# MrTornado24/IDE-3D

Measured on AMD Instinct MI355X. Metric: 512x512 RGB+seg frames/s @96 depth samples (whole job), higher is better.
Workload: dtype f32 (3x3 convs + MLPs: fp32 operands as 3 bf16 pieces, 6 products, f32 accumulate)

## Files before the change

### ide-3d_amd/csrc/modconv.hip

```cpp
#include "common.h"
#include "knobs.h"
#include <stdlib.h>
#include <string.h>
#include <type_traits>

namespace ide3d {

typedef float f32x16 __attribute__((ext_vector_type(16)));

#ifdef IDE3D_MC_TRACE
__device__ unsigned long long g_mc_dbg[256];
#define IDE3D_MC_TS(k) { const unsigned long long now_ = __builtin_readcyclecounter(); mc_acc[k] += now_ - mc_last; mc_last = now_; }
#else
#define IDE3D_MC_TS(k)
#endif

enum { MODE_CONV3 = 0, MODE_CONV1 = 1, MODE_TCONV3 = 2, MODE_TCONV3A = 3, MODE_CONV3S2 = 4 };

template <int MODE> struct ModeCfg;
template <> struct ModeCfg<MODE_CONV3>  { static constexpr int KC = 4, WTAPS = 9, MAXT = 9; };
template <> struct ModeCfg<MODE_CONV1>  { static constexpr int KC = 16, WTAPS = 1, MAXT = 1; };
template <> struct ModeCfg<MODE_CONV3S2> { static constexpr int KC = 4, WTAPS = 9, MAXT = 9; };
template <> struct ModeCfg<MODE_TCONV3> { static constexpr int KC = 4, WTAPS = 9, MAXT = 4; };
template <> struct ModeCfg<MODE_TCONV3A> { static constexpr int KC = 4, WTAPS = 9, MAXT = 9; };
// ... 426 lines not shown
        IDE3D_MC_TS(4)
    }

#ifdef IDE3D_MC_TRACE
    const unsigned long long mc_t1 = __builtin_readcyclecounter();
#endif
    modconv_finish<MODE, TI, PH, PW, NWV, K::NCLS, K::MTW, K::NTW, K::BM, 2 * K::LDS_W>(p, partial, g, acc, s_w, mb, n0, y0, x0, split, cls, wm, wn, l32);
#ifdef IDE3D_MC_TRACE
    if (blockIdx.x == 100 && threadIdx.x == 0) {
        for (int k = 0; k < 6; ++k) g_mc_dbg[k] = mc_acc[k];
        g_mc_dbg[7] = (unsigned long long)(c_end - c_begin);
        g_mc_dbg[8] = mc_prologue;
        g_mc_dbg[9] = __builtin_readcyclecounter() - mc_t1;
    }
#endif
}


typedef unsigned u32x4 __attribute__((ext_vector_type(4)));
typedef unsigned u32x2 __attribute__((ext_vector_type(2)));
typedef __bf16 bf16x8 __attribute__((ext_vector_type(8)));
typedef __bf16 bf16x2 __attribute__((ext_vector_type(2)));
typedef float f32x2 __attribute__((ext_vector_type(2)));

template <int MODE, int BIG, int PH, int PARTS, int WBUF = 2, int NWV_ = 4, int PAIR = 0>
struct SpCfg {
    static_assert(MODE == MODE_CONV3 || MODE == MODE_TCONV3A, "split-bf16 loop: 3x3 and all-class transposed 3x3 only");
    static_assert(BIG == 1 || BIG == 2, "64- or 128-row blocks");
    static_assert(NWV_ == 4 || NWV_ == 8, "4 or 8 waves");
    static constexpr int PW = 16, NWV = NWV_, NT = 64 * NWV;
    static constexpr int BN = PH * PW;
    static_assert(!PAIR || MODE == MODE_TCONV3A, "row-parity pairs exist in the transposed form only");
    static constexpr int NCLS = (MODE == MODE_TCONV3A) ? (PAIR ? 2 : 4) : 1;
    static constexpr int BM = (BIG == 1) ? 128 : 64;
    static constexpr int WM = (BIG == 2 && PH == 32) ? 1 : 2, WN = NWV / WM;
    static constexpr int MTW = BM / 32 / WM, NTW = BN / 32 / WN;
    static_assert(MTW >= 1 && MTW * 32 * WM == BM, "row block must split into 32-row MFMA tiles per wave");
    static_assert(NTW >= 1 && NTW * 32 * WN == BN, "pixel tile must split into 32-pixel MFMA tiles per wave");
    static constexpr int NLOAD = 4;
    static constexpr int KC = 16;
    static constexpr int HALO = (MODE == MODE_TCONV3A) ? 1 : 2;
    static constexpr int HP = PH + HALO, HW = PW + HALO, NSLOT = HP * HW;
    static constexpr int NS = PARTS * (PARTS + 1) / 2;
    static constexpr int W_UNITS = 3 * PARTS * 2 * BM;
    static constexpr int X_UNITS = PARTS * 2 * NSLOT;
    static constexpr int NXR = (NSLOT + 63) / 64;
    static constexpr int LDS_BYTES = 16 * (WBUF * W_UNITS + 2 * X_UNITS);
    static_assert(LDS_BYTES <= 160 * 1024, "LDS of one CU");
};

__host__ __device__ inline int64_t sp_packed_units(int mblocks, int cchunks, int bm, int parts) { return (int64_t)mblocks * cchunks * 9 * parts * 2 * bm; }

__device__ __forceinline__ unsigned pk_bf16(float a, float b) {
    f32x2 v = {a, b};
    return __builtin_bit_cast(unsigned, __builtin_convertvector(v, bf16x2));
}
typedef _Float16 f16x2 __attribute__((ext_vector_type(2)));
typedef _Float16 f16x8 __attribute__((ext_vector_type(8)));
template <int PARTS, int F16 = 0>
__device__ __forceinline__ void split_pair(float a, float b, unsigned (&out)[PARTS]) {
    if constexpr (F16) {
        static_assert(PARTS == 2, "the fp16 split has two pieces");
        const f32x2 v = {a, b};
        const unsigned hi = __builtin_bit_cast(unsigned, __builtin_convertvector(v, f16x2));
        f32x2 r;
        asm("v_fma_mix_f32 %0, %1, -1.0, %2 op_sel_hi:[1,0,0]" : "=v"(r.x) : "v"(hi), "v"(a));
        asm("v_fma_mix_f32 %0, %1, -1.0, %2 op_sel:[1,0,0] op_sel_hi:[1,0,0]" : "=v"(r.y) : "v"(hi), "v"(b));
        out[0] = hi; out[1] = __builtin_bit_cast(unsigned, __builtin_convertvector(r, f16x2));
    } else {
#pragma unroll
    for (int q = 0; q < PARTS; ++q) {
        const unsigned pk = pk_bf16(a, b);
        out[q] = pk;
        if (q + 1 < PARTS) { a -= __uint_as_float(pk << 16); b -= __uint_as_float(pk & 0xffff0000u); }
    }
    }
}
template <int F16>
__device__ __forceinline__ f32x16 sp_mfma(const u32x4& a, const u32x4& b, const f32x16& c) {
    if constexpr (F16) return __builtin_amdgcn_mfma_f32_32x32x16_f16(__builtin_bit_cast(f16x8, a), __builtin_bit_cast(f16x8, b), c, 0, 0, 0);
    else return __builtin_amdgcn_mfma_f32_32x32x16_bf16(__builtin_bit_cast(bf16x8, a), __builtin_bit_cast(bf16x8, b), c, 0, 0, 0);
}
__device__ __forceinline__ void f16_scale(float bound, float& scale, float& unscale) {
    scale = 1.f; unscale = 1.f;
    if (bound > 0.f && bound < __builtin_inff()) {
        int e;
        frexpf(bound, &e);
        e = min(max(15 - e, -126), 126);
        scale = ldexpf(1.f, e); unscale = ldexpf(1.f, -e);
    }
}

__global__ void __launch_bounds__(256)
modconv_row_scale_kernel(const float* __restrict__ w, int cout, int rowlen, int rows_padded, float* __restrict__ scale, float* __restrict__ unscale) {
    const int row = blockIdx.x * 4 + (threadIdx.x >> 6), lane = threadIdx.x & 63;
    if (row >= rows_padded) return;
    float m = 0.f;
    if (row < cout) for (int i = lane; i < rowlen; i += 64) m = fmaxf(m, fabsf(w[(int64_t)row * rowlen + i]));
#pragma unroll
    for (int off = 32; off > 0; off >>= 1) m = fmaxf(m, __shfl_xor(m, off));
    if (lane == 0) { float sc, us; f16_scale(m, sc, us); scale[row] = sc; unscale[row] = us; }
}

template <int PARTS, int F16 = 0>
__global__ void __launch_bounds__(256)
modconv_pack_split_kernel(const float* __restrict__ w, int cout, int cin, int bm, int mblocks, int cchunks, u32x4* __restrict__ out,
                          const float* __restrict__ row_scale = nullptr) {
    const int64_t total = (int64_t)mblocks * cchunks * 9 * 2 * bm;
    const int64_t stride = (int64_t)gridDim.x * blockDim.x;
    for (int64_t i = (int64_t)blockIdx.x * blockDim.x + threadIdx.x; i < total; i += stride) {
        int64_t r = i;
        const int co_l = (int)(r % bm); r /= bm;
        const int kg = (int)(r % 2); r /= 2;
        const int tap = (int)(r % 9); r /= 9;
        const int cc = (int)(r % cchunks); r /= cchunks;
        const int mb = (int)r;
        const int co = mb * bm + co_l;
        const float rs = F16 ? row_scale[co] : 1.f;
        unsigned pk[4][PARTS];
#pragma unroll
        for (int e = 0; e < 4; ++e) {
            const int ci = cc * 16 + kg * 8 + e * 2;
            const float a = (co < cout && ci < cin) ? w[((int64_t)co * cin + ci) * 9 + tap] * rs : 0.f;
            const float b = (co < cout && ci + 1 < cin) ? w[((int64_t)co * cin + ci + 1) * 9 + tap] * rs : 0.f;
            split_pair<PARTS, F16>(a, b, pk[e]);
        }
        const int64_t base = (((int64_t)(mb * cchunks + cc) * 9 + tap) * PARTS * 2 + kg) * bm + co_l;
#pragma unroll
        for (int q = 0; q < PARTS; ++q) {
            const u32x4 v = {pk[0][q], pk[1][q], pk[2][q], pk[3][q]};
            out[base + (int64_t)q * 2 * bm] = v;
        }
    }
}

template <int OFF_BYTES>
__device__ __forceinline__ u32x4 lds_read128_async(unsigned addr) {
    u32x4 v;
    asm volatile("ds_read_b128 %0, %1 offset:%2" : "=v"(v) : "v"(addr), "n"(OFF_BYTES));
    return v;
}
template <int PENDING>
__device__ __forceinline__ void lds_wait128(u32x4& first) { asm volatile("s_waitcnt lgkmcnt(%1)" : "+v"(first) : "n"(PENDING)); }
__device__ __forceinline__ void lds_pin128(u32x4& v) { asm volatile("" : "+v"(v)); }

struct HeadEpi {
    const u32x4* w;
    const float* bias;
    float* y;
    int rows;
    float clamp;
    int store_x;
    int bias_first;
};
template <int PH, int PW, int NWV, int MTW, int NTW, int BM, int MT, int PARTS, int SCRATCH>
__device__ __forceinline__ void split_heads_finish(const ide3d_modconv_params& p, const HeadEpi& he, f32x16 (&acc)[1][MTW][NTW], float* smem,
                                                   int n0, int y0, int x0, int wm, int wn, int lp) {
    constexpr int NT = 64 * NWV, BN = PH * PW, TP = BN + 4, ROWS = MT * 32, CCH = BM / 16, A_UNITS = PARTS * 2 * ROWS;
    static_assert(BM * TP + 2 * BM + ROWS <= SCRATCH, "activation tile + coefficients must fit the loop's LDS");
    const int tid = threadIdx.x, lane = tid & 63, half = lane >> 5, l32 = lane & 31;
    const int wid = __builtin_amdgcn_readfirstlane(tid >> 6);
    const int hw = p.h * p.w_;
    float* const s_t = smem;
    float* const s_dm = smem + BM * TP;
    float* const s_bi = s_dm + BM;
    float* const s_hb = s_bi + BM;
    for (int e = tid; e < BM; e += NT) {
        s_dm[e] = (p.dcoefs && e < p.cout) ? p.dcoefs[(int64_t)n0 * p.cout + e] : 1.f;
        s_bi[e] = (p.bias && e < p.cout) ? p.bias[e] : 0.f;
    }
    for (int e = tid; e < ROWS; e += NT) s_hb[e] = (he.bias && e < he.rows) ? he.bias[e] : 0.f;
    __syncthreads();
    const float e_alpha = (p.act == 3) ? p.alpha : 1.f, e_gain = p.gain;
    const float e_clamp = (p.clamp >= 0.f) ? p.clamp : __builtin_inff();
    const float e_nstr = p.noise ? p.noise_strength : 0.f;
    auto finish = [&](float v, float d, float nz, float bb) {
        v *= d; v += nz; v += bb;
        v = (v > 0.f) ? v : v * e_alpha;
        v *= e_gain;
        return fminf(fmaxf(v, -e_clamp), e_clamp);
    };
#pragma unroll
    for (int j = 0; j < NTW; ++j) {
        const int pix = (wn * NTW + j) * 32 + lp;
        const int gy = y0 + pix / PW, gx = x0 + pix % PW;
        const float nz = (e_nstr != 0.f) ? p.noise[gy * p.w_ + gx] * e_nstr : 0.f;
#pragma unroll
        for (int i = 0; i < MTW; ++i)
#pragma unroll
            for (int r = 0; r < 16; ++r) {
                const int rl = (wm * MTW + i) * 32 + (r & 3) + 8 * (r >> 2) + 4 * half;
                s_t[rl * TP + pix] = finish(acc[0][i][j][r], s_dm[rl], nz, s_bi[rl]);
            }
    }
    __syncthreads();
    typedef float f32x4a __attribute__((ext_vector_type(4)));
    typedef float f32x4u __attribute__((ext_vector_type(4), aligned(4)));
    if (he.store_x) {
        float* const yimg = p.y + (int64_t)n0 * p.cout * hw;
#pragma unroll 4
        for (int e = tid; e < BM * BN / 4; e += NT) {
            const int rl = e / (BN / 4), pix = (e % (BN / 4)) * 4;
            const int gy = y0 + pix / PW, gx = x0 + pix % PW;
            *reinterpret_cast<f32x4u*>(yimg + (int64_t)rl * hw + gy * p.w_ + gx) = *reinterpret_cast<const f32x4a*>(s_t + rl * TP + pix);
        }
    }
    constexpr int NPT = BN / 32;
    constexpr int RG = (MT % 2 == 0 && NPT / NWV < 2) ? 2 : 1, MTH = MT / RG, PG = NWV / RG, NTH = NPT / PG;
    static_assert(MTH * RG == MT && NTH * PG == NPT && NTH >= 1, "head work must split evenly over the waves");
    const int rg = wid / PG, pg = wid % PG;
    const u32x4* __restrict__ wsrc = he.w + (int64_t)n0 * CCH * A_UNITS + half * ROWS + rg * MTH * 32 + l32;
    f32x16 hacc[MTH][NTH];
#pragma unroll
    for (int m = 0; m < MTH; ++m)
#pragma unroll
        for (int g = 0; g < 4; ++g) {
            const f32x4a b4 = *reinterpret_cast<const f32x4a*>(s_hb + (rg * MTH + m) * 32 + 8 * g + 4 * half);
#pragma unroll
            for (int t = 0; t < NTH; ++t)
#pragma unroll
                for (int k = 0; k < 4; ++k) hacc[m][t][4 * g + k] = he.bias_first ? b4[k] : 0.f;
        }
    u32x4 af[2][MTH][PARTS];
    auto fetch_a = [&](int c, int buf) {
#pragma unroll
        for (int m = 0; m < MTH; ++m)
#pragma unroll
            for (int q = 0; q < PARTS; ++q) af[buf][m][q] = wsrc[(int64_t)c * A_UNITS + q * 2 * ROWS + m * 32];
    };
    fetch_a(0, 0);
#pragma unroll
    for (int c = 0; c < CCH; ++c) {
        const int ab = c & 1;
        if (c + 1 < CCH) fetch_a(c + 1, ab ^ 1);
#pragma unroll
        for (int t = 0; t < NTH; ++t) {
            const float* xs = s_t + (c * 16 + 8 * half) * TP + (pg * NTH + t) * 32 + l32;
            u32x4 bfrag[PARTS];
            {
                unsigned pk[4][PARTS];
#pragma unroll
                for (int e = 0; e < 4; ++e) split_pair<PARTS>(xs[(2 * e) * TP], xs[(2 * e + 1) * TP], pk[e]);
#pragma unroll
                for (int q = 0; q < PARTS; ++q) bfrag[q] = u32x4{pk[0][q], pk[1][q], pk[2][q], pk[3][q]};
            }
#pragma unroll
            for (int m = 0; m < MTH; ++m)
#pragma unroll
                for (int qa = 0; qa < PARTS; ++qa)
#pragma unroll
                    for (int qb = 0; qa + qb < PARTS; ++qb)
                        hacc[m][t] = __builtin_amdgcn_mfma_f32_32x32x16_bf16(__builtin_bit_cast(bf16x8, af[ab][m][qa]), __builtin_bit_cast(bf16x8, bfrag[qb]), hacc[m][t], 0, 0, 0);
        }
    }
    const float h_clamp = (he.clamp >= 0.f) ? he.clamp : __builtin_inff();
#pragma unroll
    for (int t = 0; t < NTH; ++t) {
        const int pix = (pg * NTH + t) * 32 + l32;
        const int gy = y0 + pix / PW, gx = x0 + pix % PW;
        float* const o = he.y + (int64_t)n0 * he.rows * hw + gy * p.w_ + gx;
#pragma unroll
        for (int m = 0; m < MTH; ++m)
#pragma unroll
            for (int r = 0; r < 16; ++r) {
                const int row = (rg * MTH + m) * 32 + 8 * (r >> 2) + 4 * half + (r & 3);
                if (row >= he.rows) continue;
                float v = hacc[m][t][r];
                if (he.bias_first) {
                    v = __builtin_amdgcn_fmed3f(v, -h_clamp, h_clamp);
                } else {
                    v *= 1.f; v += 0.f; v += s_hb[row];
                    v = (v > 0.f) ? v : v * 1.f;
                    v = fminf(fmaxf(v, -h_clamp), h_clamp);
                }
                o[(int64_t)row * hw] = v;
            }
    }
    __syncthreads();
}

template <int MODE, int BIG, int PH, int PARTS, int WBUF, int NWV, int F16, int TEAMS = 1, int PAR = -1, int HEAD_MT = 0>
__device__ __forceinline__ void modconv_split_tile(const ide3d_modconv_params& p, const u32x4* __restrict__ wp, float* __restrict__ partial,
                                                   const ConvGeom& g, unsigned char* smem, int mb, int tl, int grp, int split, int tiles_x,
                                                   const float* __restrict__ row_unscale, float* wg_scratch = nullptr, const HeadEpi* he = nullptr) {
    using K = SpCfg<MODE, BIG, PH, PARTS, WBUF, NWV, (PAR >= 0)>;
    static_assert(!F16 || PARTS == 2, "f16x3 = two fp16 pieces per operand");
    static_assert(PAR < 0 || (MODE == MODE_TCONV3A && WBUF == 2 && TEAMS == 1), "row-parity pairs: transposed form, two weight buffers, one team");
    constexpr int NST = (PAR < 0) ? 3 : (PAR == 0 ? 2 : 1);
    auto kys = [](int i) constexpr { return (PAR < 0) ? i : (PAR == 0 ? 2 * i : 1); };
    static_assert(TEAMS == 1 || (TEAMS == 2 && NWV == 4), "two teams of four waves, or one team");
    constexpr int PW = K::PW;
    const int tid = (TEAMS == 2) ? (int)(threadIdx.x & 255u) : (int)threadIdx.x, lane = tid & 63;
    const int wid = __builtin_amdgcn_readfirstlane(tid >> 6);
    const int wm = wid / K::WN, wn = wid % K::WN;
    const int half = lane >> 5, l32 = lane & 31;
    const int lp = ((((l32 >> 2) ^ (l32 >> 3) ^ (l32 >> 4)) & 1) << 4) | (l32 & 15);
    const int txi = tl % tiles_x, tyi = tl / tiles_x;
    const int y0 = tyi * PH, x0 = txi * PW;
    const int n0 = grp;
    u32x4* const s_w = reinterpret_cast<u32x4*>(smem);
    u32x4* const s_x = s_w + WBUF * K::W_UNITS;

    f32x16 acc[K::NCLS][K::MTW][K::NTW];
#pragma unroll
    for (int q = 0; q < K::NCLS; ++q)
#pragma unroll
        for (int i = 0; i < K::MTW; ++i)
#pragma unroll
            for (int j = 0; j < K::NTW; ++j)
#pragma unroll
                for (int r = 0; r < 16; ++r) acc[q][i][j][r] = 0.f;

    const int hw = p.h * p.w_;
    int x_src[K::NXR];
#pragma unroll
    for (int r = 0; r < K::NXR; ++r) {
        const int sidx = lane + 64 * r;
        const int ry = sidx / K::HW, rx = sidx % K::HW;
        const int yy = y0 - 1 + ry, xx = x0 - 1 + rx;
        x_src[r] = (sidx < K::NSLOT && yy >= 0 && yy < p.h && xx >= 0 && xx < p.w_) ? yy * p.w_ + xx : -1;
    }
    const float* __restrict__ ximg = p.x + (int64_t)n0 * p.cin * hw;
    float xreg[K::NXR][4];
    float sty[4];
    float xs = 1.f, xus = 1.f;
    if constexpr (F16) {
        float mm = p.styles ? 0.f : 1.f;
        if (p.styles) for (int ci = lane; ci < p.cin; ci += 64) mm = fmaxf(mm, fabsf(p.styles[(int64_t)n0 * p.cin + ci]));
        float xm = (lane < IDE3D_AMAX_SLOTS) ? p.x_amax[(int64_t)n0 * IDE3D_AMAX_FLOATS + lane * IDE3D_AMAX_STRIDE] : 0.f;
#pragma unroll
        for (int off = 32; off > 0; off >>= 1) { mm = fmaxf(mm, __shfl_xor(mm, off)); xm = fmaxf(xm, __shfl_xor(xm, off)); }
        f16_scale(mm * xm, xs, xus);
    }
    const bool stages_patch = (NWV == 4) || wid < 4;
    auto fetch_patch = [&](int c) {
        if (!stages_patch) return;
        const int ci0 = c * K::KC + wid * 4;
#pragma unroll
        for (int k = 0; k < 4; ++k) {
            const int ci = min(ci0 + k, p.cin - 1);
            sty[k] = (ci0 + k < p.cin) ? (p.styles ? p.styles[(int64_t)n0 * p.cin + ci] : 1.f) : 0.f;
#pragma unroll
            for (int r = 0; r < K::NXR; ++r) xreg[r][k] = ximg[(int64_t)ci * hw + max(x_src[r], 0)];
        }
    };
    auto commit_patch = [&](int buf) {
        if (!stages_patch) return;
        unsigned char* const dst = reinterpret_cast<unsigned char*>(s_x + buf * K::X_UNITS) + ((wid >> 1) * K::NSLOT) * 16 + (wid & 1) * 8;
        const float sc[4] = {F16 ? sty[0] * xs : sty[0], F16 ? sty[1] * xs : sty[1], F16 ? sty[2] * xs : sty[2], F16 ? sty[3] * xs : sty[3]};
#pragma unroll
        for (int r = 0; r < K::NXR; ++r) {
            const int sidx = lane + 64 * r;
            const bool live = x_src[r] >= 0;
            unsigned lo[PARTS], hi[PARTS];
            split_pair<PARTS, F16>(live ? xreg[r][0] * sc[0] : 0.f, live ? xreg[r][1] * sc[1] : 0.f, lo);
            split_pair<PARTS, F16>(live ? xreg[r][2] * sc[2] : 0.f, live ? xreg[r][3] * sc[3] : 0.f, hi);
            if (sidx < K::NSLOT) {
#pragma unroll
                for (int q = 0; q < PARTS; ++q) {
                    const u32x2 v = {lo[q], hi[q]};
                    *reinterpret_cast<u32x2*>(dst + (q * 2 * K::NSLOT + sidx) * 16) = v;
                }
            }
        }
    };
    const u32x4* __restrict__ wsrc = wp + (int64_t)mb * g.cchunks * 3 * K::W_UNITS;
    constexpr int W_PIECES = K::W_UNITS / 64;
    static_assert(K::W_UNITS % 64 == 0, "weight stage is a whole number of 1 KB pieces");
    constexpr int W_COL = (W_PIECES + 3) / 4;
    constexpr int W_EARLY = (NWV == 8) ? (W_COL * 5 + 8) / 9 : W_COL;
    auto fetch_weights = [&](int stage, int buf, bool late = false) {
        const u32x4* src = wsrc + (int64_t)stage * K::W_UNITS;
        if (NWV == 4 && late) return;
        if (NWV == 8 && (late != (wid < 4))) return;
        const int m0 = late ? W_EARLY : 0, m1 = late ? W_COL : W_EARLY;
        for (int m = m0; m < m1; ++m) {
            const int i = (wid & 3) + 4 * m;
            if (i < W_PIECES)
                __builtin_amdgcn_global_load_lds((const __attribute__((address_space(1))) void*)(src + i * 64 + lane),
                                                 (__attribute__((address_space(3))) void*)(s_w + buf * K::W_UNITS + i * 64), 16, 0, 0);
        }
    };

    const unsigned a_base0 = (unsigned)(size_t)(s_w + half * K::BM + wm * K::MTW * 32 + l32);
    unsigned b_base0[K::NTW];
#pragma unroll
    for (int j = 0; j < K::NTW; ++j) {
        const int pix = (wn * K::NTW + j) * 32 + lp;
        b_base0[j] = (unsigned)(size_t)(s_x + half * K::NSLOT + (pix / PW) * K::HW + (pix % PW));
    }

    const int c_begin = split * g.chunks_per_split;
    const int c_end = min(c_begin + g.chunks_per_split, g.cchunks);
#ifdef IDE3D_MC_TRACE
    unsigned long long mc_acc[6] = {0, 0, 0, 0, 0, 0}, mc_last = 0;
    const unsigned long long mc_t0 = __builtin_readcyclecounter();
#endif
    if (c_begin < c_end) {
        if (WBUF == 2) { fetch_weights(c_begin * 3 + kys(0), 0); if (NWV == 8) fetch_weights(c_begin * 3 + kys(0), 0, true); }
        fetch_patch(c_begin);
        commit_patch(0);
    }
    asm volatile("s_waitcnt vmcnt(0)" ::: "memory");
    __syncthreads();
    int wbuf = 0;
#ifdef IDE3D_MC_TRACE
    mc_last = __builtin_readcyclecounter();
    const unsigned long long mc_prologue = mc_last - mc_t0;
#endif
    for (int c = c_begin; c < c_end; ++c) {
        const int xbuf = (c - c_begin) & 1;
        const bool more = c + 1 < c_end;
        static_for<NST>([&](auto sii) {
            constexpr int SI = decltype(sii)::value, KY = kys(SI);
            constexpr bool LAST = (SI == NST - 1), MID = (SI == (NST == 3 ? 1 : 0));
            const int next_stage = LAST ? (c + 1) * 3 + kys(0) : c * 3 + kys(LAST ? 0 : SI + 1);
            IDE3D_MC_TS(0)
            if constexpr (WBUF == 2) {
                if (!LAST || more) fetch_weights(next_stage, wbuf ^ 1);
                if (MID && more) fetch_patch(c + 1);
            } else {
                fetch_weights(c * 3 + KY, 0);
                if (MID && more) fetch_patch(c + 1);
                asm volatile("s_waitcnt vmcnt(0)" ::: "memory");
                __syncthreads();
            }
            IDE3D_MC_TS(1)
            const unsigned a_base = a_base0 + ((WBUF == 2) ? wbuf * (K::W_UNITS * 16) : 0);
            unsigned b_base[K::NTW];
#pragma unroll
            for (int j = 0; j < K::NTW; ++j) b_base[j] = b_base0[j] + xbuf * (K::X_UNITS * 16);
            constexpr int GRP = K::MTW + K::NTW, NGRP = 3 * PARTS;
            constexpr int SP_AHEAD = 1;
            constexpr int NBUF = (PARTS == 2 && SP_AHEAD > 1) ? 3 : 2;
            constexpr int AHEAD_CAP = 15 / GRP - 1, AHEAD_SAFE = (NBUF - 1) * PARTS - 1;
            constexpr int AHEAD = (SP_AHEAD < AHEAD_CAP ? SP_AHEAD : AHEAD_CAP) < AHEAD_SAFE ? (SP_AHEAD < AHEAD_CAP ? SP_AHEAD : AHEAD_CAP) : AHEAD_SAFE;
            static_assert(AHEAD >= 1 && (AHEAD + 1) * GRP <= 15, "lgkmcnt is a 4-bit counter");
            constexpr bool B_REUSE = (MODE == MODE_TCONV3A) && NBUF == 2;
            u32x4 av[NBUF][K::MTW][PARTS], bv[NBUF][K::NTW][PARTS];
            auto issue = [&](auto ss) {
                constexpr int S = decltype(ss)::value, KX = S / PARTS, Q = S % PARTS, B = KX % NBUF, T = KY * 3 + KX;
                constexpr int BS = B_REUSE ? (KX == 2 ? 1 : 0) : B;
                static_for<K::MTW>([&](auto ii) {
                    constexpr int I = decltype(ii)::value;
                    av[B][I][Q] = lds_read128_async<(((KX * PARTS + Q) * 2) * K::BM + I * 32) * 16>(a_base);
                });
                if constexpr (!(B_REUSE && KX == 1))
                static_for<K::NTW>([&](auto jj) {
                    constexpr int J = decltype(jj)::value;
                    bv[BS][J][Q] = lds_read128_async<(Q * 2 * K::NSLOT + tap_patch_offset<MODE, K::HW>(T)) * 16>(b_base[J]);
                });
            };
            static_for<AHEAD>([&](auto ss) { issue(ss); });
            static_for<NGRP>([&](auto ss) {
                constexpr int S = decltype(ss)::value, KX = S / PARTS, Q = S % PARTS, B = KX % NBUF, QC = (PAR >= 0) ? (KX & 1) : tap_class<MODE>(KY * 3 + KX);
                constexpr int BS = B_REUSE ? (KX == 2 ? 1 : 0) : B;
                if constexpr (S + AHEAD < NGRP) issue(std::integral_constant<int, S + AHEAD>{});
                constexpr int PENDING = [] { int n = 0; for (int s2 = S + 1; s2 <= S + AHEAD && s2 < NGRP; ++s2) n += K::MTW + ((B_REUSE && s2 / PARTS == 1) ? 0 : K::NTW); return n; }();
                lds_wait128<PENDING>(av[B][0][Q]);
#pragma unroll
                for (int i = 0; i < K::MTW; ++i) lds_pin128(av[B][i][Q]);
                if constexpr (!(B_REUSE && KX == 1)) {
#pragma unroll
                for (int j = 0; j < K::NTW; ++j) lds_pin128(bv[BS][j][Q]);
                }
#pragma unroll
                for (int qa = 0; qa <= Q; ++qa)
#pragma unroll
                    for (int qb = 0; qb <= Q; ++qb) {
                        if ((qa == Q || qb == Q) && qa + qb < PARTS) {
#pragma unroll
                            for (int i = 0; i < K::MTW; ++i)
#pragma unroll
                                for (int j = 0; j < K::NTW; ++j)
                                    acc[QC][i][j] = sp_mfma<F16>(av[B][i][qa], bv[BS][j][qb], acc[QC][i][j]);
                        }
                    }
            });
            IDE3D_MC_TS(2)
            if (LAST && more) commit_patch(xbuf ^ 1);
            if constexpr (WBUF == 2 && NWV == 8) { if (!LAST || more) fetch_weights(next_stage, wbuf ^ 1, true); }
            IDE3D_MC_TS(3)
            if (WBUF == 2) asm volatile("s_waitcnt vmcnt(0)" ::: "memory");
            IDE3D_MC_TS(4)
            __syncthreads();
            IDE3D_MC_TS(5)
            wbuf ^= 1;
        });
    }
#ifdef IDE3D_MC_TRACE
    const unsigned long long mc_t1 = __builtin_readcyclecounter();
#endif
    if constexpr (HEAD_MT > 0) {
        static_assert(MODE == MODE_CONV3 && TEAMS == 1 && !F16 && K::NCLS == 1, "fused heads: 3x3 split-bf16 layers");
        split_heads_finish<PH, PW, K::NWV, K::MTW, K::NTW, K::BM, HEAD_MT, PARTS, K::LDS_BYTES / 4>(p, *he, acc, reinterpret_cast<float*>(smem), n0, y0, x0, wm, wn, lp);
    } else
    modconv_finish<MODE, 1, PH, PW, K::NWV, K::NCLS, K::MTW, K::NTW, K::BM, K::LDS_BYTES / 4, PAR>(p, partial, g, acc, reinterpret_cast<float*>(smem), mb, n0, y0, x0, split, 0, wm, wn, lp,
                                                                                                F16 ? row_unscale : nullptr, xus, (TEAMS == 2) ? tid : -1, wg_scratch);
#ifdef IDE3D_MC_TRACE
    if (blockIdx.x == 100 && (threadIdx.x == 0 || threadIdx.x == 256)) {
        const int o = threadIdx.x ? 16 : 0;
        for (int k = 0; k < 6; ++k) g_mc_dbg[o + k] = mc_acc[k];
        g_mc_dbg[o + 7] = (unsigned long long)(c_end - c_begin) * 3;
        g_mc_dbg[o + 8] = mc_prologue;
        g_mc_dbg[o + 9] = __builtin_readcyclecounter() - mc_t1;
    }
#endif
}



constexpr int head_waves(int mt) { return mt == 1 ? 16 : 8; }
template <int PARTS, int MT>
struct HeadCfg {
    static constexpr int ROWS = MT * 32;
    static constexpr int A_UNITS = PARTS * 2 * ROWS;
    static constexpr int NWV = head_waves(MT);
    static constexpr int BN = 32 * NWV;
};
__host__ __device__ inline int64_t head_packed_units(int n, int cchunks, int parts, int mt) { return (int64_t)n * cchunks * parts * 2 * mt * 32; }

template <int PARTS>
__global__ void __launch_bounds__(256)
head_pack_split_kernel(const float* __restrict__ w, int64_t w_batch_stride, int n, int cout, int cin, int rows, int cchunks, u32x4* __restrict__ out) {
    const int64_t total = (int64_t)n * cchunks * 2 * rows;
    const int64_t stride = (int64_t)gridDim.x * blockDim.x;
    for (int64_t i = (int64_t)blockIdx.x * blockDim.x + threadIdx.x; i < total; i += stride) {
        int64_t r = i;
        const int row = (int)(r % rows); r /= rows;
        const int kg = (int)(r % 2); r /= 2;
        const int cc = (int)(r % cchunks); r /= cchunks;
        const int nb = (int)r;
        unsigned pk[4][PARTS];
#pragma unroll
        for (int e = 0; e < 4; ++e) {
            const int ci = cc * 16 + kg * 8 + e * 2;
            const float a = (row < cout && ci < cin) ? w[nb * w_batch_stride + (int64_t)row * cin + ci] : 0.f;
            const float b = (row < cout && ci + 1 < cin) ? w[nb * w_batch_stride + (int64_t)row * cin + ci + 1] : 0.f;
            split_pair<PARTS>(a, b, pk[e]);
        }
        const int64_t base = (((int64_t)nb * cchunks + cc) * PARTS * 2 + kg) * rows + row;
#pragma unroll
        for (int q = 0; q < PARTS; ++q) {
            const u32x4 v = {pk[0][q], pk[1][q], pk[2][q], pk[3][q]};
            out[base + (int64_t)q * 2 * rows] = v;
        }
    }
}

template <int PARTS, int MT>
__global__ void __launch_bounds__(64 * head_waves(MT), head_waves(MT) / 4)
head_split_kernel(ide3d_modconv_params p, const u32x4* __restrict__ wp, int cchunks, int tiles_per_image) {
    using K = HeadCfg<PARTS, MT>;
    if constexpr (K::NWV == 16) asm volatile("" ::: "v127"); else asm volatile("" ::: "v255");
    constexpr int S_MIN = K::NWV * 32 * 40 / 4 + 2 * K::ROWS / 4 + 16;
    constexpr int S_UNITS = (2 * K::A_UNITS > S_MIN) ? 2 * K::A_UNITS : S_MIN;
    __shared__ __attribute__((aligned(16))) u32x4 s_a[S_UNITS];
    const int tid = threadIdx.x, lane = tid & 63, half = lane >> 5, l32 = lane & 31;
    const int wid = __builtin_amdgcn_readfirstlane(tid >> 6);
    const int bid = xcd_remap(blockIdx.x, gridDim.x);
    const int n0 = bid / tiles_per_image, tile = bid % tiles_per_image;
    const int hw = p.h * p.w_;
    const int pix = tile * K::BN + wid * 32 + l32;
    const int pix_c = min(pix, hw - 1);
    const float* __restrict__ xl = p.x + (int64_t)n0 * p.cin * hw + (int64_t)(8 * half) * hw + pix_c;
    const u32x4* __restrict__ wsrc = wp + (int64_t)n0 * cchunks * K::A_UNITS;

    f32x16 acc[1][MT][1];
#pragma unroll
    for (int m = 0; m < MT; ++m)
#pragma unroll
        for (int r = 0; r < 16; ++r) acc[0][m][0][r] = 0.f;

    constexpr int A_PIECES = K::A_UNITS / 64;
    static_assert(K::A_UNITS % 64 == 0, "whole 1 KB pieces");
    auto fetch_a = [&](int c, int buf) {
        for (int i = wid; i < A_PIECES; i += K::NWV)
            __builtin_amdgcn_global_load_lds((const __attribute__((address_space(1))) void*)(wsrc + (int64_t)c * K::A_UNITS + i * 64 + lane),
                                             (__attribute__((address_space(3))) void*)(s_a + buf * K::A_UNITS + i * 64), 16, 0, 0);
    };
    float xr[3][8];
    auto fetch_b = [&](int c, auto slot_tag) {
        constexpr int SLOT = decltype(slot_tag)::value;
#pragma unroll
        for (int e = 0; e < 8; ++e) {
            const int ch = c * 16 + 8 * half + e;
            const float v = xl[(int64_t)(min(ch, p.cin - 1) - 8 * half) * hw];
            xr[SLOT][e] = (ch < p.cin) ? v : 0.f;
        }
    };
    using S0 = std::integral_constant<int, 0>; using S1 = std::integral_constant<int, 1>; using S2 = std::integral_constant<int, 2>;
    fetch_a(0, 0); fetch_b(0, S0{});
    if (cchunks > 1) fetch_b(1, S1{});
    auto chunk = [&](int c, auto slot_tag) {
        constexpr int SLOT = decltype(slot_tag)::value, NSLOT = (SLOT + 2) % 3;
        if (c + 1 < cchunks) asm volatile("s_waitcnt vmcnt(8)" ::: "memory"); else asm volatile("s_waitcnt vmcnt(0)" ::: "memory");
        __syncthreads();
        if (c + 1 < cchunks) fetch_a(c + 1, (c + 1) & 1);
        if (c + 2 < cchunks) fetch_b(c + 2, std::integral_constant<int, NSLOT>{});
        u32x4 bfrag[PARTS];
        {
            unsigned pk[4][PARTS];
#pragma unroll
            for (int e = 0; e < 4; ++e) split_pair<PARTS>(xr[SLOT][2 * e], xr[SLOT][2 * e + 1], pk[e]);
#pragma unroll
            for (int q = 0; q < PARTS; ++q) bfrag[q] = u32x4{pk[0][q], pk[1][q], pk[2][q], pk[3][q]};
        }
        const u32x4* sa = s_a + (c & 1) * K::A_UNITS + half * K::ROWS + l32;
#pragma unroll
        for (int m = 0; m < MT; ++m) {
            u32x4 af[PARTS];
#pragma unroll
            for (int q = 0; q < PARTS; ++q) af[q] = sa[q * 2 * K::ROWS + m * 32];
#pragma unroll
            for (int qa = 0; qa < PARTS; ++qa)
#pragma unroll
                for (int qb = 0; qa + qb < PARTS; ++qb)
                    acc[0][m][0] = __builtin_amdgcn_mfma_f32_32x32x16_bf16(__builtin_bit_cast(bf16x8, af[qa]), __builtin_bit_cast(bf16x8, bfrag[qb]), acc[0][m][0], 0, 0, 0);
        }
    };
    for (int c = 0; c < cchunks; c += 3) {
        chunk(c, S0{});
        if (c + 1 < cchunks) chunk(c + 1, S1{});
        if (c + 2 < cchunks) chunk(c + 2, S2{});
    }
    __syncthreads();
    ide3d_modconv_params pf = p;
    pf.h = 1; pf.w_ = hw;
    ConvGeom g{};
    g.oh = 1; g.ow = hw; g.split_k = 1;
    modconv_finish<MODE_CONV1, 1, 1, K::BN, K::NWV, 1, MT, 1, K::ROWS, S_UNITS * 4>(pf, nullptr, g, acc, reinterpret_cast<float*>(s_a), 0, n0, 0, tile * K::BN, 0, 0, 0, wid, l32);
}


template <class T>
__device__ __forceinline__ T* uniform_ptr(T* ptr) {
    const uint64_t v = reinterpret_cast<uint64_t>(ptr);
    const unsigned lo = __builtin_amdgcn_readfirstlane((unsigned)v), hi = __builtin_amdgcn_readfirstlane((unsigned)(v >> 32));
    return reinterpret_cast<T*>(((uint64_t)hi << 32) | lo);
}
template <int PARTS, int MT, int NCH>
__global__ void __launch_bounds__(512, 2)
head_resident_kernel(ide3d_modconv_params p, const u32x4* __restrict__ wp, int wgs_per_image, int tiles32) {
    using K = HeadCfg<PARTS, MT>;
    asm volatile("" ::: "v255");
    constexpr int NWV = 8, NBUF = (MT == 1) ? 2 : 1;
    __shared__ __attribute__((aligned(16))) u32x4 s_a[NCH * K::A_UNITS + K::ROWS / 4 + 4];
    float* const s_bi = reinterpret_cast<float*>(s_a + NCH * K::A_UNITS);
// ... 174 lines not shown

constexpr int STRIP_CO = 8, STRIP_WAVES = 16;
__global__ void __launch_bounds__(256)
tconv_strip_pack_kernel(const float* __restrict__ w, int cout, int cin, int cout_pad, float* __restrict__ ws) {
    const int64_t total = (int64_t)cin * 6 * cout_pad;
    for (int64_t i = (int64_t)blockIdx.x * 256 + threadIdx.x; i < total; i += (int64_t)gridDim.x * 256) {
        const int co = (int)(i % cout_pad); const int64_t r = i / cout_pad;
        const int t = (int)(r % 6), ci = (int)(r / 6);
        const int tap = t < 3 ? 6 + t : (t - 3) * 3 + 2;
        ws[i] = co < cout ? w[((int64_t)co * cin + ci) * 9 + tap] : 0.f;
    }
}
__global__ void __launch_bounds__(256)
tconv_strip_gather_kernel(const float* __restrict__ x, int rows, int h, int w_, float* __restrict__ xs) {
    const int len = w_ + h;
    for (int64_t i = (int64_t)blockIdx.x * 256 + threadIdx.x; i < (int64_t)rows * len; i += (int64_t)gridDim.x * 256) {
        const int64_t r = i / len; const int e = (int)(i - r * len);
        xs[i] = e < w_ ? x[r * h * w_ + (int64_t)(h - 1) * w_ + e] : x[r * h * w_ + (int64_t)(e - w_) * w_ + (w_ - 1)];
    }
}
__global__ void __launch_bounds__(64 * STRIP_WAVES, 4)
tconv_strip_kernel(ide3d_modconv_params p, const float* __restrict__ ws, const float* __restrict__ xs, int cout_pad, int oh, int ow, int64_t pitch,
                   int nb_re, int nb_ro, int nb_ce) {
    __shared__ float s_red[STRIP_WAVES][STRIP_CO][64];
    __shared__ float s_am[STRIP_WAVES];
    const int h = p.h, w_ = p.w_;
    const int lane = threadIdx.x & 63, q = __builtin_amdgcn_readfirstlane((int)(threadIdx.x >> 6));
    int b = (int)blockIdx.x, kind = 0;
    if (b >= nb_re) { b -= nb_re; kind = 1; if (b >= nb_ro) { b -= nb_ro; kind = 2; if (b >= nb_ce) { b -= nb_ce; kind = 3; } } }
    const bool is_row = kind < 2, odd = kind & 1;
    const int a = b * 64 + lane;
    const int t = 2 * a + (odd ? 1 : 0);
    const bool live = t < (is_row ? ow : oh - 1);
    const int co0 = (int)blockIdx.y * STRIP_CO, n = (int)blockIdx.z;
    const int len = is_row ? w_ : h;
    const bool ok_a = live && a < len, ok_b = live && !odd && a >= 1;
    const int64_t xs_pitch = (int64_t)w_ + h;
    const float* __restrict__ xn = xs + (int64_t)n * p.cin * xs_pitch;
    const int64_t off_a = (is_row ? 0 : w_) + min(a, len - 1), off_b = (is_row ? 0 : w_) + min(max(a - 1, 0), len - 1);
    const float* __restrict__ wt = ws + (is_row ? 0 : 3) * (int64_t)cout_pad + co0;
    constexpr int STRIP_CH = 8 * STRIP_WAVES, PER_WAVE = STRIP_CH / STRIP_WAVES, WPC = 3 * STRIP_CO;
    static_assert(PER_WAVE * WPC == 3 * 64, "three weight loads per lane and chunk");
    __shared__ __attribute__((aligned(16))) float s_wt[STRIP_WAVES][PER_WAVE * WPC];
    float acc[STRIP_CO];
#pragma unroll
    for (int j = 0; j < STRIP_CO; ++j) acc[j] = 0.f;
    for (int c0 = 0; c0 < p.cin; c0 += STRIP_CH) {
        float xa[PER_WAVE], xb[PER_WAVE], scv[PER_WAVE], wreg[3];
#pragma unroll
        for (int k = 0; k < PER_WAVE; ++k) {
            const int ci = min(c0 + q + k * STRIP_WAVES, p.cin - 1);
            xa[k] = xn[(int64_t)ci * xs_pitch + off_a];
            xb[k] = odd ? 0.f : xn[(int64_t)ci * xs_pitch + off_b];
            scv[k] = p.styles ? p.styles[(int64_t)n * p.cin + ci] : 1.f;
        }
#pragma unroll
        for (int r = 0; r < 3; ++r) {
            const int e = lane + 64 * r, k = e / WPC, rem = e - k * WPC, tp = rem / STRIP_CO, jj = rem - tp * STRIP_CO;
            const int ci = c0 + q + k * STRIP_WAVES;
            wreg[r] = (ci < p.cin) ? wt[((int64_t)ci * 6 + tp) * cout_pad + jj] : 0.f;
        }
        __builtin_amdgcn_wave_barrier();
#pragma unroll
        for (int r = 0; r < 3; ++r) s_wt[q][lane + 64 * r] = wreg[r];
        __builtin_amdgcn_fence(__ATOMIC_RELEASE, "wavefront");
        __builtin_amdgcn_wave_barrier();
        __builtin_amdgcn_fence(__ATOMIC_ACQUIRE, "wavefront");
#pragma unroll
        for (int k = 0; k < PER_WAVE; ++k) {
            const float va = ok_a ? xa[k] * scv[k] : 0.f;
            const float4* wv = reinterpret_cast<const float4*>(&s_wt[q][k * WPC]);
            if (odd) {
                const float4 b0 = wv[2], b1 = wv[3];
                const float w1[STRIP_CO] = {b0.x, b0.y, b0.z, b0.w, b1.x, b1.y, b1.z, b1.w};
#pragma unroll
                for (int j = 0; j < STRIP_CO; ++j) acc[j] = fmaf(va, w1[j], acc[j]);
            } else {
                const float vb = ok_b ? xb[k] * scv[k] : 0.f;
                const float4 a0 = wv[0], a1 = wv[1], c0v = wv[4], c1v = wv[5];
                const float w0[STRIP_CO] = {a0.x, a0.y, a0.z, a0.w, a1.x, a1.y, a1.z, a1.w};
                const float w2[STRIP_CO] = {c0v.x, c0v.y, c0v.z, c0v.w, c1v.x, c1v.y, c1v.z, c1v.w};
#pragma unroll
                for (int j = 0; j < STRIP_CO; ++j) { acc[j] = fmaf(va, w0[j], acc[j]); acc[j] = fmaf(vb, w2[j], acc[j]); }
            }
        }
    }
#pragma unroll
    for (int j = 0; j < STRIP_CO; ++j) s_red[q][j][lane] = acc[j];
    __syncthreads();
    float am = 0.f;
    {
        static_assert(STRIP_CO <= STRIP_WAVES, "wave q < STRIP_CO finishes output channel co0 + q");
        float v = 0.f;
        const int qc = min(q, STRIP_CO - 1);
#pragma unroll
        for (int k = 0; k < STRIP_WAVES; ++k) v += s_red[k][qc][lane];
        const int co = co0 + q;
        if (live && q < STRIP_CO && co < p.cout) {
            v *= p.dcoefs ? p.dcoefs[(int64_t)n * p.cout + co] : 1.f;
            const int oy = is_row ? oh - 1 : t, ox = is_row ? t : ow - 1;
            p.y[((int64_t)n * p.cout + co) * ((int64_t)oh * pitch) + (int64_t)oy * pitch + ox] = v;
            amax_acc(am, v);
        }
    }
    if (p.y_amax) amax_raise_block(p.y_amax, n, am, s_am);
}

struct BlockId { int mb, tile, grp, split; };
__device__ __forceinline__ BlockId decode_block(const ConvGeom& g) {
    int bid = xcd_remap(blockIdx.x, gridDim.x);
    BlockId b;
    b.mb = bid % g.mblocks; bid /= g.mblocks;
    b.tile = bid % g.tile_base[4]; bid /= g.tile_base[4];
    b.grp = bid % g.img_groups; bid /= g.img_groups;
    b.split = bid;
    return b;
}

template <int MODE, int BIG, int TI, int PH, int PW, int NWV = 4, int KCO = 0>
__global__ void __launch_bounds__(64 * NWV, NWV == 8 ? 2
                                  : (McCfg<MODE, BIG, TI, PH, PW, NWV, KCO>::NCLS * McCfg<MODE, BIG, TI, PH, PW, NWV, KCO>::MTW * McCfg<MODE, BIG, TI, PH, PW, NWV, KCO>::NTW > 8) ? 1
                                  : (TI * PH * PW <= 128 && MODE != MODE_CONV3S2 && KCO == 0) ? 3 : 2)
modconv_kernel(ide3d_modconv_params p, const float* __restrict__ wp, float* __restrict__ partial, ConvGeom g) {
    using K = McCfg<MODE, BIG, TI, PH, PW, NWV, KCO>;
    __shared__ __attribute__((aligned(16))) float s_w[2 * K::LDS_W];
    __shared__ __attribute__((aligned(16))) float s_x[2 * K::LDS_X];
    const BlockId b = decode_block(g);
    int cls = 0;
    if (MODE == MODE_TCONV3) { cls = (b.tile >= g.tile_base[1]) + (b.tile >= g.tile_base[2]) + (b.tile >= g.tile_base[3]); }
    modconv_tile<MODE, BIG, TI, PH, PW, NWV, KCO>(p, wp, partial, g, s_w, s_x, b.mb, b.tile - g.tile_base[cls], b.grp, b.split, cls, g.tiles_x[cls]);
}


#ifdef IDE3D_SP_SHARED_SIMD
constexpr bool kSpExclusive = false;
#else
constexpr bool kSpExclusive = true;
#endif
template <int MODE, int BIG, int PH, int PARTS, int WBUF, int NWV>
constexpr int sp_waves_per_simd() {
    using K = SpCfg<MODE, BIG, PH, PARTS, WBUF, NWV>;
    return (NWV == 8) ? 2 : (!kSpExclusive && K::LDS_BYTES <= 80 * 1024 && (WBUF == 1 || K::NCLS * K::MTW * K::NTW <= 8)) ? 2 : 1;
}
template <int MODE, int BIG, int PH, int PARTS, int WBUF = 2, int NWV = 4, int F16 = 0>
__global__ void __launch_bounds__(64 * NWV, (sp_waves_per_simd<MODE, BIG, PH, PARTS, WBUF, NWV>()))
modconv_split_kernel(ide3d_modconv_params p, const u32x4* __restrict__ wp, float* __restrict__ partial, ConvGeom g, const float* __restrict__ row_unscale) {
    using K = SpCfg<MODE, BIG, PH, PARTS, WBUF, NWV>;
    if constexpr (kSpExclusive) { if constexpr (NWV == 8) asm volatile("" ::: "v255"); else asm volatile("" ::: "v255", "a255"); }
    __shared__ __attribute__((aligned(16))) unsigned char sp_smem[K::LDS_BYTES];
    const BlockId b = decode_block(g);
    modconv_split_tile<MODE, BIG, PH, PARTS, WBUF, NWV, F16>(p, wp, partial, g, sp_smem, b.mb, b.tile, b.grp, b.split, g.tiles_x[0], row_unscale);
}

template <int BIG, int PH, int HEAD_MT>
__global__ void __launch_bounds__(512, 2)
modconv_split_heads_kernel(ide3d_modconv_params p, const u32x4* __restrict__ wp, ConvGeom g, HeadEpi he) {
    using K = SpCfg<MODE_CONV3, BIG, PH, 3, 2, 8>;
    if constexpr (kSpExclusive) asm volatile("" ::: "v255");
    __shared__ __attribute__((aligned(16))) unsigned char sp_smem[K::LDS_BYTES];
    const BlockId b = decode_block(g);
    modconv_split_tile<MODE_CONV3, BIG, PH, 3, 2, 8, 0, 1, -1, HEAD_MT>(p, wp, nullptr, g, sp_smem, b.mb, b.tile, b.grp, b.split, g.tiles_x[0], nullptr, nullptr, &he);
}

template <int BIG, int PH, int PARTS, int F16 = 0>
__global__ void __launch_bounds__(512, 2)
modconv_split_pair_kernel(ide3d_modconv_params p, const u32x4* __restrict__ wp, float* __restrict__ partial, ConvGeom g, const float* __restrict__ row_unscale) {
    using K = SpCfg<MODE_TCONV3A, BIG, PH, PARTS, 2, 8, 1>;
    if constexpr (kSpExclusive) asm volatile("" ::: "v255");
    __shared__ __attribute__((aligned(16))) unsigned char sp_smem[K::LDS_BYTES];
    const int half_grid = (int)(gridDim.x >> 1);
    const int par = __builtin_amdgcn_readfirstlane((int)blockIdx.x >= half_grid ? 1 : 0);
    int bid = xcd_remap((int)blockIdx.x - par * half_grid, half_grid);
    BlockId b;
    b.mb = bid % g.mblocks; bid /= g.mblocks;
    b.tile = bid % g.tile_base[4]; bid /= g.tile_base[4];
    b.grp = bid % g.img_groups; bid /= g.img_groups;
    b.split = bid;
    if (par == 0) modconv_split_tile<MODE_TCONV3A, BIG, PH, PARTS, 2, 8, F16, 1, 0>(p, wp, partial, g, sp_smem, b.mb, b.tile, b.grp, b.split, g.tiles_x[0], row_unscale);
    else          modconv_split_tile<MODE_TCONV3A, BIG, PH, PARTS, 2, 8, F16, 1, 1>(p, wp, partial, g, sp_smem, b.mb, b.tile, b.grp, b.split, g.tiles_x[0], row_unscale);
}

template <int MODE, int BIG, int PH, int PARTS, int WBUF, int F16>
__global__ void __launch_bounds__(512, 2)
modconv_split_teams_kernel(ide3d_modconv_params p, const u32x4* __restrict__ wp, float* __restrict__ partial, ConvGeom g, const float* __restrict__ row_unscale) {
    using K = SpCfg<MODE, BIG, PH, PARTS, WBUF, 4>;
    static_assert(2 * K::LDS_BYTES <= 160 * 1024, "both teams' LDS must fit");
    asm volatile("" ::: "v255");
    __shared__ __attribute__((aligned(16))) unsigned char sp_smem[2 * K::LDS_BYTES];
    const int team = (int)(threadIdx.x >> 8);
    int bid = xcd_remap(blockIdx.x, gridDim.x);
    const int mpairs = g.mblocks >> 1;
    BlockId b;
    b.mb = 2 * (bid % mpairs) + team; bid /= mpairs;
    b.tile = bid % g.tile_base[4]; bid /= g.tile_base[4];
    b.grp = bid % g.img_groups; bid /= g.img_groups;
    b.split = bid;
    modconv_split_tile<MODE, BIG, PH, PARTS, WBUF, 4, F16, 2>(p, wp, partial, g, sp_smem + team * K::LDS_BYTES, b.mb, b.tile, b.grp, b.split, g.tiles_x[0], row_unscale,
                                                              reinterpret_cast<float*>(sp_smem));
}

__global__ void __launch_bounds__(256)
modconv_epilogue_kernel(ide3d_modconv_params p, const float* __restrict__ partial, int split_k, int oh, int ow) {
    const int64_t per = (int64_t)p.n * p.cout * oh * ow;
    const int64_t stride = (int64_t)gridDim.x * blockDim.x;
    int am_n = -1; float am = 0.f;
    __shared__ unsigned s_am[64];
    const bool am_lds = p.y_amax && p.n <= 64;
    if (p.y_amax) { if (threadIdx.x < 64) s_am[threadIdx.x] = 0u; __syncthreads(); }
    const int hw = oh * ow;
    if (p.y_pitch <= 0 && (hw & 3) == 0) {
        typedef float f32x4v __attribute__((ext_vector_type(4)));
        const int64_t per4 = per >> 2;
        for (int64_t q = (int64_t)blockIdx.x * blockDim.x + threadIdx.x; q < per4; q += stride) {
            const int64_t i = q << 2;
            f32x4v v = {0.f, 0.f, 0.f, 0.f};
            int s = 0;
            for (; s + 4 <= split_k; s += 4) {
                f32x4v t[4];
#pragma unroll
                for (int k = 0; k < 4; ++k) t[k] = *reinterpret_cast<const f32x4v*>(partial + (int64_t)(s + k) * per + i);
#pragma unroll
                for (int k = 0; k < 4; ++k) v += t[k];
            }
            for (; s < split_k; ++s) v += *reinterpret_cast<const f32x4v*>(partial + (int64_t)s * per + i);
            const int pix = (int)(i % hw);
            const int co = (int)((i / hw) % p.cout);
            const int n = (int)(i / ((int64_t)hw * p.cout));
            const float d = p.dcoefs ? p.dcoefs[(int64_t)n * p.cout + co] : 1.f, bb = p.bias ? p.bias[co] : 0.f;
#pragma unroll
            for (int e = 0; e < 4; ++e) {
                float x = v[e];
                if (p.dcoefs) x *= d;
                if (p.noise) x += p.noise[pix + e] * p.noise_strength;
                if (p.bias) x += bb;
                if (p.act == 3) x = (x > 0.f) ? x : x * p.alpha;
                x *= p.gain;
                if (p.clamp >= 0.f) x = fminf(fmaxf(x, -p.clamp), p.clamp);
                v[e] = x;
            }
            *reinterpret_cast<f32x4v*>(p.y + i) = v;
            if (p.y_amax) {
                if (n != am_n) { if (am_n >= 0) { if (am_lds) amax_lds_flush(s_am, am_n, am); else amax_commit(p.y_amax, am_n, am, false); } am_n = n; am = 0.f; }
                amax_acc(am, v[0]); amax_acc(am, v[1]); amax_acc(am, v[2]); amax_acc(am, v[3]);
            }
        }
    } else
    for (int64_t i = (int64_t)blockIdx.x * blockDim.x + threadIdx.x; i < per; i += stride) {
        float v = 0.f;
        int s = 0;
        for (; s + 8 <= split_k; s += 8) {
            float t[8];
#pragma unroll
            for (int k = 0; k < 8; ++k) t[k] = partial[(int64_t)(s + k) * per + i];
#pragma unroll
            for (int k = 0; k < 8; ++k) v += t[k];
        }
        if (s + 4 <= split_k) {
            float t[4];
#pragma unroll
            for (int k = 0; k < 4; ++k) t[k] = partial[(int64_t)(s + k) * per + i];
#pragma unroll
            for (int k = 0; k < 4; ++k) v += t[k];
            s += 4;
        }
        for (; s < split_k; ++s) v += partial[(int64_t)s * per + i];
        const int pix = (int)(i % ((int64_t)oh * ow));
        const int co = (int)((i / ((int64_t)oh * ow)) % p.cout);
        const int n = (int)(i / ((int64_t)oh * ow * p.cout));
        if (p.dcoefs) v *= p.dcoefs[(int64_t)n * p.cout + co];
        if (p.noise) v += p.noise[pix] * p.noise_strength;
        if (p.bias) v += p.bias[co];
        if (p.act == 3) v = (v > 0.f) ? v : v * p.alpha;
        v *= p.gain;
        if (p.clamp >= 0.f) v = fminf(fmaxf(v, -p.clamp), p.clamp);
        if (p.y_pitch > 0) p.y[(i / ow) * p.y_pitch + (i % ow)] = v; else p.y[i] = v;
        if (p.y_amax) {
            if (n != am_n) { if (am_n >= 0) { if (am_lds) amax_lds_flush(s_am, am_n, am); else amax_commit(p.y_amax, am_n, am, false); } am_n = n; am = 0.f; }
            amax_acc(am, v);
        }
    }
    if (p.y_amax) {
        if (am_n >= 0) { if (am_lds) amax_lds_flush(s_am, am_n, am); else amax_commit(p.y_amax, am_n, am, false); }
        if (am_lds) amax_lds_commit(p.y_amax, s_am, p.n);
    }
}


struct ConvPlan {
    int mode, big, tile;
    int bm, kc, taps, mblocks, cchunks, oh, ow;
    int parts;
    int f16;
    int pair;
    int strip;
    int64_t strip_off, strip_floats;
    int64_t packed_floats, aux_floats, partial_floats;
    ConvGeom g;
};

struct McEnv { bool no_flat, no_allcls; int tile, debug, ta_rows; };
static const McEnv& mc_env() {
    static const McEnv e = {knobs().mc_no_flat, knobs().mc_no_allcls, knobs().mc_tile, knobs().mc_debug, knobs().mc_ta_rows};
    return e;
}

struct PlanKnobs { bool ta_bm64, head_bm128, ta_kc8, no_smallmap, ta_old, sp_oldplan, no_ph32, no_w8split, no_one_round; int sp_modes; };
static const PlanKnobs& plan_knobs() {
    const Knobs& e = knobs();
    static const PlanKnobs k = {e.ta_bm64, e.head_bm128, e.ta_kc8, e.no_smallmap, e.ta_old, e.sp_oldplan, e.no_ph32, e.no_w8split, e.no_one_round, e.sp_modes};
    return k;
}

static ide3d_modconv_params flatten_pointwise(const ide3d_modconv_params& in) {
    ide3d_modconv_params p = in;
// ... 268 lines not shown
}
static bool head_resident_applies(const ide3d_modconv_params& p) {
    const bool no_resident = ide3d::knobs().head_no_resident;
    const int mt = p.cout <= 32 ? 1 : 6, cchunks = ide3d::cdiv(p.cin, 16);
    const int hw = p.h * p.w_, wgs_img = ide3d::kNumCU / p.n, tiles32 = hw / 32;
    return !no_resident && ide3d::kSpExclusive && p.cin % 16 == 0 && hw % 32 == 0 && wgs_img >= 1 && p.y_pitch == 0 &&
           ((mt == 1 && (cchunks == 4 || cchunks == 8)) || (mt == 6 && cchunks == 8)) && tiles32 >= 2 * wgs_img * 8;
}

static int check_modconv(const ide3d_modconv_params& p) {
    using namespace ide3d;
    IDE3D_CHECK_ARG(p.n > 0 && p.cin > 0 && p.cout > 0 && p.h > 0 && p.w_ > 0, "modconv2d: bad shape");
    IDE3D_CHECK_ARG(p.k == 1 || p.k == 3, "modconv2d: kernel size must be 1 or 3 (got %d)", p.k);
    IDE3D_CHECK_ARG(p.mode == 0 || ((p.mode == 1 || p.mode == 2) && p.k == 3),
                    "modconv2d: mode must be 0 (conv), 1 (3x3 stride-2 conv, no padding) or 2 (3x3 transposed, stride 2)");
    IDE3D_CHECK_ARG(p.mode != 1 || (p.h >= 3 && p.w_ >= 3), "modconv2d: stride-2 convolution needs an input of at least 3x3");
    IDE3D_CHECK_ARG((int64_t)p.n * p.cin * p.h * p.w_ < 0x7fffffffLL, "modconv2d: input too large for 32-bit indexing");
    return IDE3D_OK;
}

extern "C" int64_t ide3d_modconv_workspace_bytes(int32_t n, int32_t cin, int32_t cout, int32_t h, int32_t w, int32_t k, int32_t mode,
                                                 int32_t per_image_weights) {
    using namespace ide3d;
    ide3d_modconv_params p{};
    p.n = n; p.cin = cin; p.cout = cout; p.h = h; p.w_ = w; p.k = k; p.mode = mode; p.w_batch_stride = per_image_weights ? 1 : 0;
    if (check_modconv(p) != IDE3D_OK) return -1;
    p.x = nullptr;
    int64_t packed = 0, part = 0;
    static const float dummy = 0.f;
    for (int epi = 0; epi < 2; ++epi) {
        ide3d_modconv_params q0 = p;
        q0.act = 1; q0.gain = 1.f; q0.clamp = -1.f;
        if (epi == 1) { q0.noise = &dummy; q0.bias = &dummy; q0.noise_strength = 1.f; q0.act = 3; q0.alpha = 0.2f; q0.gain = 1.41421356f; }
        for (int arith : {1, 3, 6, 16}) {
            ConvPlan pl; plan_conv(q0, pl, arith);
            ConvPlan pf; plan_conv(flatten_pointwise(q0), pf, arith);
            for (const ConvPlan* q : {&pl, &pf}) {
                if (q->packed_floats + q->aux_floats > packed) packed = q->packed_floats + q->aux_floats;
                if (q->partial_floats > part) part = q->partial_floats;
            }
        }
    }
    int64_t bytes = (packed + part) * (int64_t)sizeof(float);
    if (per_image_weights && k == 1) {
        const int64_t hb = head_packed_units(n, cdiv(cin, 16), 3, cout <= 32 ? 1 : 6) * 16;
        if (hb > bytes) bytes = hb;
    }
    return bytes;
}

static void pack_split_weights(const ide3d_modconv_params& p, const ide3d::ConvPlan& pl, float* wp, hipStream_t st) {
    using namespace ide3d;
    const int64_t items = (int64_t)pl.mblocks * pl.cchunks * 9 * 2 * pl.bm;
    if (pl.f16) {
        float* const rs = wp + pl.packed_floats;
        const int rows = pl.mblocks * pl.bm;
        hipLaunchKernelGGL(modconv_row_scale_kernel, dim3(cdiv(rows, 4)), dim3(256), 0, st, p.w, p.cout, p.cin * 9, rows, rs, rs + rows);
        hipLaunchKernelGGL((modconv_pack_split_kernel<2, 1>), dim3(stream_grid(items, 256)), dim3(256), 0, st, p.w, p.cout, p.cin, pl.bm, pl.mblocks, pl.cchunks, reinterpret_cast<u32x4*>(wp), rs);
    }
    else if (pl.parts == 2) hipLaunchKernelGGL(modconv_pack_split_kernel<2>, dim3(stream_grid(items, 256)), dim3(256), 0, st, p.w, p.cout, p.cin, pl.bm, pl.mblocks, pl.cchunks, reinterpret_cast<u32x4*>(wp), nullptr);
    else               hipLaunchKernelGGL(modconv_pack_split_kernel<3>, dim3(stream_grid(items, 256)), dim3(256), 0, st, p.w, p.cout, p.cin, pl.bm, pl.mblocks, pl.cchunks, reinterpret_cast<u32x4*>(wp), nullptr);
}

extern "C" int ide3d_modconv2d(const ide3d_modconv_params* pp, void* stream) {
    using namespace ide3d;
    IDE3D_CHECK_ARG(pp != nullptr, "modconv2d: null params");
    const ide3d_modconv_params p = flatten_pointwise(*pp);
    IDE3D_CHECK_ARG(p.x && p.w && p.y && p.workspace, "modconv2d: null tensor / workspace pointer");
    int rc = check_modconv(p);
    if (rc) return rc;
    IDE3D_CHECK_ARG(p.act == 1 || p.act == 3, "modconv2d: act must be linear (1) or lrelu (3)");
    IDE3D_CHECK_ARG(p.y_pitch == 0 || (p.mode == 2 && p.y_pitch >= 2 * p.w_ + 1), "modconv2d: y_pitch is the row pitch of a transposed convolution's output (>= 2 w + 1), or 0");
    hipStream_t st_head = (hipStream_t)stream;
    {
        const int64_t hw = (int64_t)p.h * p.w_;
        if (head_small_applies(p)) {
            if (hw <= 64) hipLaunchKernelGGL((head_small_kernel<64, 32>), dim3(cdiv(p.cout, HS_RB), 1, p.n), dim3(HS_THREADS), 0, st_head, p, (int)hw);
            else          hipLaunchKernelGGL((head_small_kernel<256, 8>), dim3(cdiv(p.cout, HS_RB), cdiv((int)hw, 256), p.n), dim3(HS_THREADS), 0, st_head, p, (int)hw);
            IDE3D_CHECK_LAUNCH("modconv2d (small-map heads)");
            return IDE3D_OK;
        }
    }
    if (head_split_applies(p, resolve_arith(p.arith))) {
        const int parts = resolve_arith(p.arith) == 3 ? 2 : 3, mt = p.cout <= 32 ? 1 : 6, cchunks = cdiv(p.cin, 16);
        IDE3D_CHECK_ARG(p.workspace_bytes >= head_packed_units(p.n, cchunks, parts, mt) * 16, "modconv2d: workspace too small for the packed head weights");
        u32x4* wu = reinterpret_cast<u32x4*>(p.workspace);
        const int64_t items = (int64_t)p.n * cchunks * 2 * mt * 32;
        const int tiles = cdiv(p.h * p.w_, 32 * head_waves(mt));
        const int hw_h = p.h * p.w_, wgs_img = kNumCU / p.n, tiles32 = hw_h / 32;
        const bool resident = head_resident_applies(p);
#define IDE3D_HEAD_RES(P, M, C) IDE3D_EXCL_LAUNCH((head_resident_kernel<P, M, C>), dim3(p.n * wgs_img), 512, 0, st_head, p, wu, wgs_img, tiles32)
#define IDE3D_HEAD(P, M) do { \
            hipLaunchKernelGGL(head_pack_split_kernel<P>, dim3(stream_grid(items, 256)), dim3(256), 0, st_head, p.w, p.w_batch_stride, p.n, p.cout, p.cin, M * 32, cchunks, wu); \
            if (resident) { if (M == 6) IDE3D_HEAD_RES(P, 6, 8); else if (cchunks == 4) IDE3D_HEAD_RES(P, 1, 4); else IDE3D_HEAD_RES(P, 1, 8); } \
            else IDE3D_EXCL_LAUNCH((head_split_kernel<P, M>), dim3(p.n * tiles), 64 * head_waves(M), 0, st_head, p, wu, cchunks, tiles); } while (0)
        if (parts == 2) { if (mt == 1) IDE3D_HEAD(2, 1); else IDE3D_HEAD(2, 6); }
        else            { if (mt == 1) IDE3D_HEAD(3, 1); else IDE3D_HEAD(3, 6); }
#undef IDE3D_HEAD
#undef IDE3D_HEAD_RES
        IDE3D_CHECK_LAUNCH("modconv2d (split-bf16 heads)");
        return IDE3D_OK;
    }
    int arith_eff = resolve_arith(p.arith);
    if (arith_eff == 16 && !p.x_amax) arith_eff = 6;
    ConvPlan pl; plan_conv(p, pl, arith_eff);
    IDE3D_CHECK_ARG(p.workspace_bytes >= (pl.packed_floats + pl.aux_floats + pl.partial_floats) * (int64_t)sizeof(float),
                    "modconv2d: workspace too small (need %lld bytes)", (long long)((pl.packed_floats + pl.aux_floats + pl.partial_floats) * sizeof(float)));
    hipStream_t st = (hipStream_t)stream;
    float* wp = p.workspace;
    float* partial = p.workspace + pl.packed_floats + pl.aux_floats;
    if (pl.parts) {
        if (!p.weights_packed) pack_split_weights(p, pl, wp, st);
#define IDE3D_SP_DISPATCH(M) \
        do { if (pl.big == 1) { if (pl.f16) launch_split<M, 1, 2, 1>(p, pl, wp, partial, st); else if (pl.parts == 2) launch_split<M, 1, 2>(p, pl, wp, partial, st); else launch_split<M, 1, 3>(p, pl, wp, partial, st); } \
             else             { if (pl.f16) launch_split<M, 2, 2, 1>(p, pl, wp, partial, st); else if (pl.parts == 2) launch_split<M, 2, 2>(p, pl, wp, partial, st); else launch_split<M, 2, 3>(p, pl, wp, partial, st); } } while (0)
        if (pl.mode == MODE_CONV3) IDE3D_SP_DISPATCH(MODE_CONV3); else IDE3D_SP_DISPATCH(MODE_TCONV3A);
#undef IDE3D_SP_DISPATCH
    } else {
    if (!p.weights_packed) {
        hipLaunchKernelGGL(modconv_pack_kernel, dim3(stream_grid(pl.packed_floats, 256)), dim3(256), 0, st,
                           p.w, p.w_batch_stride, p.w_batch_stride ? p.n : 1, p.cout, p.cin, pl.taps, pl.bm, pl.kc, pl.mblocks, pl.cchunks, wp);
    }
#define IDE3D_MC_DISPATCH(M) \
    do { if (pl.big == 1) launch_tiles<M, 1>(p, pl, wp, partial, st); else if (pl.big == 2) launch_tiles<M, 2>(p, pl, wp, partial, st); \
         else launch_tiles<M, 0>(p, pl, wp, partial, st); } while (0)
    if (pl.mode == MODE_CONV3)       IDE3D_MC_DISPATCH(MODE_CONV3);
    else if (pl.mode == MODE_CONV1)  IDE3D_MC_DISPATCH(MODE_CONV1);
    else if (pl.mode == MODE_CONV3S2) IDE3D_MC_DISPATCH(MODE_CONV3S2);
    else if (pl.mode == MODE_TCONV3A) IDE3D_MC_DISPATCH(MODE_TCONV3A);
    else                             IDE3D_MC_DISPATCH(MODE_TCONV3);
#undef IDE3D_MC_DISPATCH
    }
    if (pl.g.split_k > 1) {
        const int64_t per = (int64_t)p.n * p.cout * pl.oh * pl.ow;
        hipLaunchKernelGGL(modconv_epilogue_kernel, dim3(stream_grid((p.y_pitch <= 0 && ((pl.oh * pl.ow) & 3) == 0) ? per / 4 : per, 256)), dim3(256), 0, st, p, partial, pl.g.split_k, pl.oh, pl.ow);
    }
    if (pl.mode == MODE_TCONV3A && !p.weights_packed) {
        hipLaunchKernelGGL(tconv_strip_pack_kernel, dim3(stream_grid(pl.strip_floats, 256)), dim3(256), 0, st, p.w, p.cout, p.cin, cdiv(p.cout, STRIP_CO) * STRIP_CO,
                           wp + pl.packed_floats + pl.strip_off);
    }
    if (pl.strip) {
        const int cout_pad = cdiv(p.cout, STRIP_CO) * STRIP_CO;
        float* const wstrip = wp + pl.packed_floats + pl.strip_off;
        const int nb_re = cdiv(p.w_ + 1, 64), nb_ro = cdiv(p.w_, 64), nb_ce = cdiv(p.h, 64), nb_co = cdiv(p.h, 64);
        float* const xs = wstrip + pl.strip_floats;
        hipLaunchKernelGGL(tconv_strip_gather_kernel, dim3(stream_grid((int64_t)p.n * p.cin * (p.h + p.w_), 256)), dim3(256), 0, st, p.x, p.n * p.cin, p.h, p.w_, xs);
        hipLaunchKernelGGL(tconv_strip_kernel, dim3(nb_re + nb_ro + nb_ce + nb_co, cout_pad / STRIP_CO, p.n), dim3(64 * STRIP_WAVES), 0, st, p, wstrip, xs, cout_pad,
                           pl.oh, pl.ow, (int64_t)(p.y_pitch > 0 ? p.y_pitch : pl.ow), nb_re, nb_ro, nb_ce);
    }
    IDE3D_CHECK_LAUNCH("modconv2d");
    return IDE3D_OK;
}

extern "C" int ide3d_modconv2d_heads(const ide3d_modconv_params* pp, const ide3d_modconv_head_epilogue* hp, void* stream) {
    using namespace ide3d;
    IDE3D_CHECK_ARG(pp != nullptr && hp != nullptr, "modconv2d_heads: null params");
    const ide3d_modconv_params& p = *pp;
    const ide3d_modconv_head_epilogue& h = *hp;
    IDE3D_CHECK_ARG(p.x && p.w && p.workspace && (p.y || h.no_activation_output) && h.w && h.y && h.workspace, "modconv2d_heads: null tensor / workspace pointer");
    int rc = check_modconv(p);
    if (rc) return rc;
    IDE3D_CHECK_ARG(p.act == 1 || p.act == 3, "modconv2d_heads: act must be linear (1) or lrelu (3)");
    IDE3D_CHECK_ARG(h.rows > 0, "modconv2d_heads: bad head rows");
    auto no_kernel = [](const char* why) { set_error("modconv2d_heads: %s", why); return IDE3D_ENOKERNEL; };
    if (knob_live("IDE3D_MODCONV_NO_HEAD_FUSION")) return no_kernel("IDE3D_MODCONV_NO_HEAD_FUSION is set");
    if (p.k != 3 || p.mode != 0 || p.w_batch_stride != 0 || p.y_amax || p.y_pitch != 0) return no_kernel("not a shared-weight 3x3 layer without side outputs");
    int arith = resolve_arith(p.arith);
    if (arith == 16 && !p.x_amax) arith = 6;
    if (arith != 6) return no_kernel("the fused form exists for bf16x6 only");
    ConvPlan pl; plan_conv(p, pl, arith);
    if (pl.parts != 3 || pl.f16 || pl.mode != MODE_CONV3 || pl.pair || pl.g.split_k != 1 || pl.g.mblocks != 1 || pl.bm != p.cout || TIv[pl.tile] != 1)
        return no_kernel("the layer's plan does not hold all channels of a tile in one workgroup");
    const bool tile16 = pl.big == 1 && p.cout == 128 && pl.tile != 0 && pl.tile != 4 && pl.tile != 6 && pl.tile != 12 && sp_form(pl).waves == 8;
    const bool tile32 = pl.big == 2 && p.cout == 64 && pl.tile == 12;
    const int ph = tile32 ? 32 : 16;
    if (!(tile16 || tile32) || p.h % ph != 0 || p.w_ % 16 != 0) return no_kernel("no fused instance for this tile");
    ide3d_modconv_params q{};
    q.x = p.y; q.w = h.w; q.bias = h.bias; q.y = h.y;
    q.n = p.n; q.cin = p.cout; q.cout = h.rows; q.h = p.h; q.w_ = p.w_; q.k = 1; q.mode = 0;
    q.act = 1; q.alpha = 0.f; q.gain = 1.f; q.clamp = h.clamp; q.w_batch_stride = (int64_t)h.rows * p.cout; q.arith = p.arith;
    const int mt = h.rows <= 32 ? 1 : 6, hcc = p.cout / 16;
    if (head_small_applies(q) || !head_split_applies(q, resolve_arith(q.arith)) || resolve_arith(q.arith) == 3 || (mt == 6 && !tile16))
        return no_kernel("the heads do not take the split-bf16 path");
    IDE3D_CHECK_ARG(p.workspace_bytes >= (pl.packed_floats + pl.aux_floats) * (int64_t)sizeof(float), "modconv2d_heads: workspace too small");
    IDE3D_CHECK_ARG(h.workspace_bytes >= head_packed_units(p.n, hcc, 3, mt) * 16, "modconv2d_heads: head workspace too small");
    hipStream_t st = (hipStream_t)stream;
    if (!p.weights_packed) pack_split_weights(p, pl, p.workspace, st);
    u32x4* const hw_packed = reinterpret_cast<u32x4*>(h.workspace);
    const int64_t items = (int64_t)p.n * hcc * 2 * mt * 32;
    hipLaunchKernelGGL(head_pack_split_kernel<3>, dim3(stream_grid(items, 256)), dim3(256), 0, st, h.w, q.w_batch_stride, p.n, h.rows, p.cout, mt * 32, hcc, hw_packed);
    HeadEpi e;
    e.w = hw_packed; e.bias = h.bias; e.y = h.y; e.rows = h.rows; e.clamp = h.clamp; e.store_x = !h.no_activation_output;
    e.bias_first = head_resident_applies(q) ? 1 : 0;
    const ConvGeom& g = pl.g;
    const unsigned nblocks = (unsigned)((int64_t)g.mblocks * g.tile_base[4] * g.img_groups * g.split_k);
    const u32x4* wu = reinterpret_cast<const u32x4*>(p.workspace);
    if (tile32) IDE3D_EXCL_LAUNCH((modconv_split_heads_kernel<2, 32, 1>), dim3(nblocks), 512, 0, st, p, wu, g, e);
    else if (mt == 1) IDE3D_EXCL_LAUNCH((modconv_split_heads_kernel<1, 16, 1>), dim3(nblocks), 512, 0, st, p, wu, g, e);
    else IDE3D_EXCL_LAUNCH((modconv_split_heads_kernel<1, 16, 6>), dim3(nblocks), 512, 0, st, p, wu, g, e);
    IDE3D_CHECK_LAUNCH("modconv2d_heads");
    return IDE3D_OK;
}

extern "C" int ide3d_modconv_plan(const ide3d_modconv_params* pp, ide3d_modconv_plan_info* out) {
    using namespace ide3d;
    IDE3D_CHECK_ARG(pp != nullptr && out != nullptr, "modconv_plan: null argument");
    const ide3d_modconv_params p = flatten_pointwise(*pp);
    int rc = check_modconv(p);
    if (rc) return rc;
    *out = ide3d_modconv_plan_info{};
    const int arith = resolve_arith(p.arith);
    if (head_small_applies(p)) {
        const int hw = p.h * p.w_;
        out->kind = IDE3D_PLAN_HEAD_SMALL; out->tile_h = 1; out->tile_w = hw <= 64 ? 64 : 256; out->rows = HS_RB; out->waves = HS_THREADS / 64; out->split_k = 1;
        out->workgroups = (int64_t)cdiv(p.cout, HS_RB) * (hw <= 64 ? 1 : cdiv(hw, 256)) * p.n;
        return IDE3D_OK;
    }
    if (head_split_applies(p, arith)) {
        const int mt = p.cout <= 32 ? 1 : 6;
        out->rows = mt * 32; out->parts = arith == 3 ? 2 : 3; out->split_k = 1; out->tile_h = 1;
        if (head_resident_applies(p)) { out->kind = IDE3D_PLAN_HEAD_RESIDENT; out->tile_w = 32; out->waves = 8; out->workgroups = (int64_t)p.n * (kNumCU / p.n); }
        else { out->kind = IDE3D_PLAN_HEAD_SPLIT; out->waves = head_waves(mt); out->tile_w = 32 * out->waves; out->workgroups = (int64_t)p.n * cdiv(p.h * p.w_, out->tile_w); }
        return IDE3D_OK;
    }
    int arith_eff = arith;
    if (arith_eff == 16 && !p.x_amax) arith_eff = 6;
    ConvPlan pl; plan_conv(p, pl, arith_eff);
    const int64_t blocks = (int64_t)pl.g.mblocks * pl.g.tile_base[4] * pl.g.img_groups * pl.g.split_k * (pl.pair ? 2 : 1);
    out->tile_h = PHv[pl.tile]; out->tile_w = PWv[pl.tile]; out->images_per_tile = TIv[pl.tile];
    out->rows = pl.bm; out->parts = pl.parts; out->f16 = pl.f16; out->split_k = pl.g.split_k; out->strip = pl.strip;
    out->transposed_all_class = (pl.mode == MODE_TCONV3A);
    if (pl.parts) {
        const SpForm f = sp_form(pl);
        out->kind = f.teams ? IDE3D_PLAN_SPLIT_TEAMS : IDE3D_PLAN_SPLIT; out->waves = f.teams ? 8 : f.waves; out->workgroups = f.teams ? blocks / 2 : blocks;
    } else {
        out->kind = IDE3D_PLAN_FP32; out->waves = (pl.tile == 8 || pl.tile == 9) ? 8 : 4; out->workgroups = blocks;
    }
    return IDE3D_OK;
}

extern "C" int ide3d_set_conv_arithmetic(int32_t arith) {
    IDE3D_CHECK_ARG(arith == 0 || arith == 1 || arith == 3 || arith == 6 || arith == 16,
                    "set_conv_arithmetic: 0 (environment default), 1 (fp32), 3 (bf16x3), 6 (bf16x6) or 16 (f16x3)");
    ide3d::g_conv_arith = arith;
    return IDE3D_OK;
}
extern "C" int32_t ide3d_get_conv_arithmetic(void) { return ide3d::conv_arith_default(); }

#ifdef IDE3D_MC_TRACE
extern "C" int ide3d_debug_mc(unsigned long long* host) {
    return (int)hipMemcpyFromSymbol(host, HIP_SYMBOL(ide3d::g_mc_dbg), sizeof(unsigned long long) * 256);
}
#endif

namespace ide3d {
const char* modconv_build_flags() {
    return ""
#ifdef IDE3D_SP_SHARED_SIMD
        "!IDE3D_SP_SHARED_SIMD "
#endif
#ifdef IDE3D_MC_TRACE
        "IDE3D_MC_TRACE "
#endif
        ;
}
}
```

### ide-3d_amd/torch_utils/hip_plugin.py

```python

import ctypes
import math
import os
import threading
import weakref

import torch

_LIB_ENV = 'IDE3D_HIP_LIB'
_ABI_VERSION = 8
AMAX_SLOTS, AMAX_STRIDE = 32, 64
AMAX_FLOATS = AMAX_SLOTS * AMAX_STRIDE

_DTYPE_CODE = {torch.float32: 0, torch.float16: 1, torch.bfloat16: 2, torch.float64: 3}

_lock = threading.Lock()
_lib = None

CALLS = {}


def lib_path():
    env = os.environ.get(_LIB_ENV)
    if env:
        return env
    here = os.path.dirname(os.path.abspath(__file__))
    return os.path.join(os.path.dirname(here), 'lib', 'libide3d_hip.so')


class _UpfirdnParams(ctypes.Structure):
    _fields_ = [
        ('x', ctypes.c_void_p), ('f', ctypes.c_void_p), ('y', ctypes.c_void_p),
        ('dtype', ctypes.c_int32),
        ('n', ctypes.c_int32), ('c', ctypes.c_int32), ('in_h', ctypes.c_int32), ('in_w', ctypes.c_int32),
        ('out_h', ctypes.c_int32), ('out_w', ctypes.c_int32),
        ('x_stride', ctypes.c_int64 * 4), ('y_stride', ctypes.c_int64 * 4),
        ('f_h', ctypes.c_int32), ('f_w', ctypes.c_int32),
        ('f_stride', ctypes.c_int64 * 2),
        ('up_x', ctypes.c_int32), ('up_y', ctypes.c_int32), ('down_x', ctypes.c_int32), ('down_y', ctypes.c_int32),
        ('pad_x0', ctypes.c_int32), ('pad_y0', ctypes.c_int32),
        ('flip', ctypes.c_int32), ('gain', ctypes.c_float), ('x_row_floats', ctypes.c_int32),
    ]


def _row_floats_readable(x):
    if x.ndim != 4 or any(st <= 0 for st in x.stride()):
        return 0
    last_row = x.storage_offset() + sum((x.shape[i] - 1) * x.stride(i) for i in range(3))
    total = x.untyped_storage().nbytes() // x.element_size()
    return int(max(0, min(total - last_row, 2 ** 31 - 1)))


class _UpfirdnEpilogue(ctypes.Structure):
    _fields_ = [
        ('add', ctypes.c_void_p), ('add_stride', ctypes.c_int64 * 4),
        ('noise', ctypes.c_void_p), ('noise_strength', ctypes.c_float),
        ('bias', ctypes.c_void_p),
        ('fused_act', ctypes.c_int32), ('act', ctypes.c_int32),
        ('alpha', ctypes.c_float), ('act_gain', ctypes.c_float), ('clamp', ctypes.c_float),
        ('y_amax', ctypes.c_void_p),
    ]


class _FlreluParams(ctypes.Structure):
    _fields_ = [
        ('x', ctypes.c_void_p), ('y', ctypes.c_void_p), ('b', ctypes.c_void_p), ('s', ctypes.c_void_p),
        ('fu', ctypes.c_void_p), ('fd', ctypes.c_void_p),
        ('dtype', ctypes.c_int32),
        ('n', ctypes.c_int32), ('c', ctypes.c_int32), ('in_h', ctypes.c_int32), ('in_w', ctypes.c_int32),
        ('out_h', ctypes.c_int32), ('out_w', ctypes.c_int32),
        ('x_stride', ctypes.c_int64 * 4), ('y_stride', ctypes.c_int64 * 4),
        ('fu_w', ctypes.c_int32), ('fu_h', ctypes.c_int32), ('fd_w', ctypes.c_int32), ('fd_h', ctypes.c_int32),
        ('fu_stride', ctypes.c_int64 * 2), ('fd_stride', ctypes.c_int64 * 2),
        ('up', ctypes.c_int32), ('down', ctypes.c_int32),
        ('pad_x0', ctypes.c_int32), ('pad_y0', ctypes.c_int32),
        ('s_w_bytes', ctypes.c_int32), ('s_h', ctypes.c_int32),
        ('s_ofs_x', ctypes.c_int32), ('s_ofs_y', ctypes.c_int32),
        ('sw_limit', ctypes.c_int32), ('sign_mode', ctypes.c_int32),
        ('flip', ctypes.c_int32),
        ('gain', ctypes.c_float), ('slope', ctypes.c_float), ('clamp', ctypes.c_float),
    ]


class _Lattice(ctypes.Structure):
    _fields_ = [('n', ctypes.c_int32), ('voxel_size', ctypes.c_float), ('corner', ctypes.c_float * 3), ('scale', ctypes.c_float)]


class _RenderParams(ctypes.Structure):
    _fields_ = [
        ('rays_d_cam', ctypes.c_void_p), ('z_lin', ctypes.c_void_p), ('cam2world', ctypes.c_void_p),
        ('jitter', ctypes.c_void_p), ('sigma_noise', ctypes.c_void_p),
        ('tex_planes', ctypes.c_void_p), ('geo_planes', ctypes.c_void_p),
        ('tex_stride', ctypes.c_int64 * 4), ('geo_stride', ctypes.c_int64 * 4),
        ('geo_w0', ctypes.c_void_p), ('geo_b0', ctypes.c_void_p), ('geo_w1', ctypes.c_void_p), ('geo_b1', ctypes.c_void_p),
        ('tex_w0', ctypes.c_void_p), ('tex_b0', ctypes.c_void_p), ('tex_w1', ctypes.c_void_p), ('tex_b1', ctypes.c_void_p),
        ('n', ctypes.c_int32), ('rays_per_img', ctypes.c_int32), ('steps', ctypes.c_int32),
        ('C', ctypes.c_int32), ('H', ctypes.c_int32), ('W', ctypes.c_int32),
        ('hidden', ctypes.c_int32), ('feat_ch', ctypes.c_int32), ('seg_ch', ctypes.c_int32),
        ('clamp_mode', ctypes.c_int32), ('last_back', ctypes.c_int32), ('white_back', ctypes.c_int32),
        ('max_depth', ctypes.c_float),
        ('out_feat', ctypes.c_void_p), ('out_depth', ctypes.c_void_p), ('out_wsum', ctypes.c_void_p),
    ]


class _ModconvParams(ctypes.Structure):
    _fields_ = [
        ('x', ctypes.c_void_p), ('w', ctypes.c_void_p), ('styles', ctypes.c_void_p), ('dcoefs', ctypes.c_void_p),
        ('noise', ctypes.c_void_p), ('bias', ctypes.c_void_p), ('y', ctypes.c_void_p),
        ('n', ctypes.c_int32), ('cin', ctypes.c_int32), ('cout', ctypes.c_int32),
        ('h', ctypes.c_int32), ('w_', ctypes.c_int32), ('k', ctypes.c_int32),
        ('noise_strength', ctypes.c_float),
        ('act', ctypes.c_int32), ('alpha', ctypes.c_float), ('gain', ctypes.c_float), ('clamp', ctypes.c_float),
        ('mode', ctypes.c_int32), ('weights_packed', ctypes.c_int32),
        ('workspace', ctypes.c_void_p), ('workspace_bytes', ctypes.c_int64),
        ('w_batch_stride', ctypes.c_int64), ('arith', ctypes.c_int32),
        ('x_amax', ctypes.c_void_p), ('y_amax', ctypes.c_void_p), ('y_pitch', ctypes.c_int32),
    ]


class _ModconvHeadEpilogue(ctypes.Structure):
    _fields_ = [
        ('w', ctypes.c_void_p), ('bias', ctypes.c_void_p), ('y', ctypes.c_void_p),
        ('rows', ctypes.c_int32), ('clamp', ctypes.c_float), ('no_activation_output', ctypes.c_int32),
        ('workspace', ctypes.c_void_p), ('workspace_bytes', ctypes.c_int64),
    ]


class _ModconvPlanInfo(ctypes.Structure):
    _fields_ = [
        ('kind', ctypes.c_int32), ('tile_h', ctypes.c_int32), ('tile_w', ctypes.c_int32), ('images_per_tile', ctypes.c_int32),
        ('rows', ctypes.c_int32), ('waves', ctypes.c_int32), ('parts', ctypes.c_int32), ('f16', ctypes.c_int32),
        ('split_k', ctypes.c_int32), ('strip', ctypes.c_int32), ('transposed_all_class', ctypes.c_int32), ('reserved', ctypes.c_int32),
        ('workgroups', ctypes.c_int64),
    ]


PLAN_KINDS = ('fp32', 'split', 'split_teams', 'head_split', 'head_resident', 'head_small')

STYLE_BATCH_MAX = 24


class _StyleJob(ctypes.Structure):
    _fields_ = [
        ('w', ctypes.c_void_p), ('w_stride', ctypes.c_int64),
        ('affine_w', ctypes.c_void_p), ('affine_b', ctypes.c_void_p),
        ('wsq_t', ctypes.c_void_p),
        ('cin', ctypes.c_int32), ('cout', ctypes.c_int32),
        ('affine_gain', ctypes.c_float), ('bias_gain', ctypes.c_float),
        ('styles', ctypes.c_void_p), ('dcoefs', ctypes.c_void_p),
    ]


class _FoldJob(ctypes.Structure):
    _fields_ = [
        ('w', ctypes.c_void_p), ('w_stride', ctypes.c_int64),
        ('cin', ctypes.c_int32), ('affine_gain', ctypes.c_float),
        ('a0', ctypes.c_void_p), ('b0', ctypes.c_void_p), ('w0', ctypes.c_void_p), ('cout0', ctypes.c_int32), ('gain0', ctypes.c_float),
        ('a1', ctypes.c_void_p), ('b1', ctypes.c_void_p), ('w1', ctypes.c_void_p), ('cout1', ctypes.c_int32), ('gain1', ctypes.c_float),
        ('out', ctypes.c_void_p),
    ]


LOWRES_MAX_LAYERS, LOWRES_MAX_HEADS = 8, 4


class _LowresLayer(ctypes.Structure):
    _fields_ = [('weight', ctypes.c_void_p), ('styles', ctypes.c_void_p), ('dcoefs', ctypes.c_void_p), ('noise', ctypes.c_void_p), ('bias', ctypes.c_void_p),
                ('act_gain', ctypes.c_float), ('clamp', ctypes.c_float), ('up', ctypes.c_int32), ('head', ctypes.c_int32),
                ('weights_packed', ctypes.c_int32), ('reserved', ctypes.c_int32)]


class _LowresHead(ctypes.Structure):
    _fields_ = [('w', ctypes.c_void_p), ('bias', ctypes.c_void_p), ('skip', ctypes.c_void_p), ('clamp', ctypes.c_float), ('O', ctypes.c_int32)]


class _LowresParams(ctypes.Structure):
    _fields_ = [('x0', ctypes.c_void_p), ('x0_batch_stride', ctypes.c_int64), ('fir', ctypes.c_void_p), ('x_out', ctypes.c_void_p),
                ('workspace', ctypes.c_void_p), ('workspace_bytes', ctypes.c_int64),
                ('n', ctypes.c_int32), ('C', ctypes.c_int32), ('res0', ctypes.c_int32), ('nlayers', ctypes.c_int32), ('nheads', ctypes.c_int32),
                ('arith', ctypes.c_int32), ('persistent', ctypes.c_int32), ('reserved', ctypes.c_int32),
                ('layers', _LowresLayer * LOWRES_MAX_LAYERS), ('heads', _LowresHead * LOWRES_MAX_HEADS)]


class _MappingParams(ctypes.Structure):
    _fields_ = [
        ('z', ctypes.c_void_p), ('c', ctypes.c_void_p), ('embed_w', ctypes.c_void_p), ('embed_b', ctypes.c_void_p),
        ('fc_w', ctypes.c_void_p * 16), ('fc_b', ctypes.c_void_p * 16), ('fc_out', ctypes.c_int32 * 16),
        ('w_avg', ctypes.c_void_p), ('ws', ctypes.c_void_p),
        ('workspace', ctypes.c_void_p), ('workspace_bytes', ctypes.c_int64),
        ('n', ctypes.c_int32), ('z_dim', ctypes.c_int32), ('c_dim', ctypes.c_int32), ('embed', ctypes.c_int32),
        ('layers', ctypes.c_int32), ('num_ws', ctypes.c_int32),
        ('embed_weight_gain', ctypes.c_float), ('embed_bias_gain', ctypes.c_float), ('lr_multiplier', ctypes.c_float),
        ('alpha', ctypes.c_float), ('act_gain', ctypes.c_float), ('truncation_psi', ctypes.c_float),
        ('truncation_cutoff', ctypes.c_int32),
    ]


def _hip_runtimes_mapped():
    paths = set()
    try:
        with open('/proc/self/maps') as f:
            for line in f:
                if 'libamdhip64' in line:
                    paths.add(line.split()[-1])
    except OSError:
        pass
    return paths


def load():
    global _lib
    if _lib is not None:
        return _lib
    with _lock:
        if _lib is not None:
            return _lib
        path = lib_path()
        if not os.path.isfile(path):
            raise RuntimeError(
                f'libide3d_hip.so not found at {path}. Build it with `python -c "import __graft_entry__ as g; g.build()"` '
                f'or `make -C ide-3d_amd/csrc`, or point ${_LIB_ENV} at it. There is no CPU/eager fallback for CUDA tensors.')
        torch.cuda.is_available()
        try:
            lib = ctypes.CDLL(path, mode=ctypes.RTLD_LOCAL)
        except OSError as e:
            raise RuntimeError(f'failed to load {path}: {e}') from e
        rts = _hip_runtimes_mapped()
        if len(rts) > 1:
            raise RuntimeError(f'two HIP runtimes mapped in one process ({sorted(rts)}); import torch before loading the plugin')
        vp, i32, i64, f32 = ctypes.c_void_p, ctypes.c_int32, ctypes.c_int64, ctypes.c_float
        lib.ide3d_last_error.restype = ctypes.c_char_p
        lib.ide3d_last_error.argtypes = []
        lib.ide3d_abi_version.restype = ctypes.c_int
        lib.ide3d_build_arch.restype = ctypes.c_char_p
        if lib.ide3d_abi_version() != _ABI_VERSION:
            raise RuntimeError(f'{path}: ABI version {lib.ide3d_abi_version()} != expected {_ABI_VERSION}; rebuild')
        lib.ide3d_build_flags.restype = ctypes.c_char_p
        lib.ide3d_build_flags.argtypes = []
        flags = lib.ide3d_build_flags().decode('ascii', 'replace').split()
        unsafe = [f for f in flags if f.startswith('!')]
        if unsafe and os.environ.get('IDE3D_ALLOW_EXPERIMENT_BUILD') != '1':
            raise RuntimeError(f'{path} was built with experiment knobs that change results or drop a safety property ({" ".join(unsafe)}); '
                               'rebuild without EXTRA=..., or set IDE3D_ALLOW_EXPERIMENT_BUILD=1 for timing experiments')
        protos = {
            'ide3d_bias_act': [vp, vp, vp, vp, vp, vp, ctypes.c_int, ctypes.c_int, ctypes.c_int, f32, f32, f32, i64, i64, i64, vp],
            'ide3d_upfirdn2d': [ctypes.POINTER(_UpfirdnParams), vp],
            'ide3d_upfirdn2d_ex': [ctypes.POINTER(_UpfirdnParams), ctypes.POINTER(_UpfirdnEpilogue), vp],
            'ide3d_filtered_lrelu': [ctypes.POINTER(_FlreluParams), vp],
            'ide3d_filtered_lrelu_act': [vp, vp, ctypes.c_int, i32, i32, i32, i32, ctypes.POINTER(i64 * 4),
                                         i32, i32, i32, i32, f32, f32, f32, ctypes.c_int, vp],
            'ide3d_triplane_sample': [vp, ctypes.POINTER(i64 * 4), i32, i32, i32, i32, vp, i64, vp, vp],
            'ide3d_triplane_sample_rays': [vp, ctypes.POINTER(i64 * 4), i32, i32, i32, i32, vp, i64, vp, i32, i32, i32, vp],
            'ide3d_triplane_taps': [i32, i32, vp, i64, vp, vp],
            'ide3d_triplane_sample_backward': [vp, vp, ctypes.POINTER(i64 * 4), i32, i32, i32, i32, vp, i64,
                                               vp, ctypes.POINTER(i64 * 4), vp, vp],
            'ide3d_composite': [vp, vp, vp, vp, i64, i32, i32, ctypes.c_int, ctypes.c_int, ctypes.c_int, f32,
                                ctypes.c_int, vp, vp, vp, vp],
            'ide3d_sample_pdf': [vp, vp, vp, i64, i64, i32, i32, f32, vp, vp],
            'ide3d_render_rays': [ctypes.POINTER(_RenderParams), vp],
            'ide3d_sample_voxel': [ctypes.POINTER(_RenderParams), vp, i64, vp, vp, ctypes.c_int, vp],
            'ide3d_lattice_points': [ctypes.POINTER(_Lattice), i64, i64, vp, vp],
            'ide3d_density_lattice': [ctypes.POINTER(_RenderParams), ctypes.POINTER(_Lattice), i64, i64, vp, vp],
            'ide3d_modconv2d': [ctypes.POINTER(_ModconvParams), vp],
            'ide3d_modconv2d_heads': [ctypes.POINTER(_ModconvParams), ctypes.POINTER(_ModconvHeadEpilogue), vp],
            'ide3d_modconv_plan': [ctypes.POINTER(_ModconvParams), ctypes.POINTER(_ModconvPlanInfo)],
            'ide3d_modconv_workspace_bytes': [i32, i32, i32, i32, i32, i32, i32, i32],
            'ide3d_set_conv_arithmetic': [i32],
            'ide3d_get_conv_arithmetic': [],
            'ide3d_frame_u8': [vp, vp, vp, i32, i32, i32, i32, vp, vp],
            'ide3d_sphere_points': [vp, vp, i32, ctypes.c_float, i32, vp, vp, vp],
            'ide3d_cam2world': [vp, vp, vp, i32, i32, vp, vp],
            'ide3d_style_demod': [vp, i64, vp, vp, vp, i32, i32, i32, i32, f32, f32, vp, vp, vp],
            'ide3d_fold_heads': [vp, i64, i32, i32, i32, f32, vp, vp, vp, i32, f32, vp, vp, vp, i32, f32, vp, vp],
            'ide3d_style_demod_batch': [ctypes.POINTER(_StyleJob), i32, i32, i32, vp],
            'ide3d_fold_heads_batch': [ctypes.POINTER(_FoldJob), i32, i32, i32, vp],
            'ide3d_mapping': [ctypes.POINTER(_MappingParams), vp],
            'ide3d_mapping_workspace_bytes': [],
            'ide3d_mapping_supported': [],
            'ide3d_skip_upsample_add_cl': [vp, ctypes.POINTER(i64 * 4), vp, ctypes.POINTER(i64 * 4), i32, i32, i32, i32, vp, vp],
            'ide3d_bilinear_up2_split': [vp, i32, i32, i32, i32, ctypes.POINTER(vp * 3), ctypes.POINTER(i32 * 3), ctypes.POINTER(i32 * 3), ctypes.POINTER(ctypes.c_int64 * 3), vp],
            'ide3d_lowres_layers_supported': [i32, i32, i32, ctypes.POINTER(i32), i32, i32],
            'ide3d_lowres_workspace_bytes': [ctypes.POINTER(_LowresParams)],
            'ide3d_lowres_group': [ctypes.POINTER(_LowresParams), vp],
        }
        for name, argtypes in protos.items():
            fn = getattr(lib, name)
            fn.restype = ctypes.c_int64 if name.endswith('_bytes') else ctypes.c_int
            fn.argtypes = argtypes
        _lib = lib
        return _lib


EXPORTED_SYMBOLS = (
    'ide3d_last_error', 'ide3d_abi_version', 'ide3d_build_arch', 'ide3d_build_flags', 'ide3d_exclusive_violations', 'ide3d_exclusive_violation_text', 'ide3d_bias_act', 'ide3d_upfirdn2d', 'ide3d_upfirdn2d_ex',
    'ide3d_filtered_lrelu', 'ide3d_filtered_lrelu_act', 'ide3d_triplane_sample', 'ide3d_triplane_sample_rays', 'ide3d_triplane_taps',
    'ide3d_triplane_sample_backward', 'ide3d_composite', 'ide3d_sample_pdf', 'ide3d_render_rays', 'ide3d_sample_voxel',
    'ide3d_lattice_points', 'ide3d_density_lattice',
    'ide3d_modconv2d', 'ide3d_modconv2d_heads', 'ide3d_modconv_workspace_bytes', 'ide3d_modconv_plan', 'ide3d_set_conv_arithmetic', 'ide3d_get_conv_arithmetic', 'ide3d_frame_u8', 'ide3d_sphere_points', 'ide3d_cam2world', 'ide3d_style_demod', 'ide3d_fold_heads',
    'ide3d_style_demod_batch', 'ide3d_fold_heads_batch',
    'ide3d_skip_upsample_add_cl', 'ide3d_bilinear_up2_split', 'ide3d_mapping', 'ide3d_mapping_workspace_bytes', 'ide3d_mapping_supported',
    'ide3d_lowres_layers_supported', 'ide3d_lowres_workspace_bytes', 'ide3d_lowres_group',
)


def exclusive_violations():
    lib = load()
    lib.ide3d_exclusive_violations.restype = ctypes.c_int
    lib.ide3d_exclusive_violation_text.restype = ctypes.c_char_p
    return int(lib.ide3d_exclusive_violations()), lib.ide3d_exclusive_violation_text().decode('utf-8', 'replace')


def _check(rc, what):
    if rc == 0:
        CALLS[what] = CALLS.get(what, 0) + 1
    if rc != 0:
        msg = load().ide3d_last_error().decode('utf-8', 'replace')
        raise RuntimeError(f'{what} failed (code {rc}): {msg}')


_raw_stream = getattr(torch._C, '_cuda_getCurrentRawStream', None)


def _stream_handle(device):
    if _raw_stream is not None:
        return _raw_stream(device.index if device.index is not None else torch.cuda.current_device())
    return torch.cuda.current_stream(device).cuda_stream


def _stream(t):
    return ctypes.c_void_p(_stream_handle(t.device))


_private_streams = {}


def _hip_runtime():
    paths = _hip_runtimes_mapped()
    if len(paths) != 1:
        raise RuntimeError(f'expected exactly one HIP runtime mapped in this process, found {sorted(paths)}')
    rt = ctypes.CDLL(next(iter(paths)))
    rt.hipStreamCreateWithFlags.argtypes = [ctypes.POINTER(ctypes.c_void_p), ctypes.c_uint]
    rt.hipStreamCreateWithFlags.restype = ctypes.c_int
    return rt


def private_stream(device, purpose):
    device = torch.device(device)
    idx = device.index if device.index is not None else torch.cuda.current_device()
    key = (idx, purpose)
    st = _private_streams.get(key)
    if st is None:
        with _lock:
            st = _private_streams.get(key)
            if st is None:
                torch.cuda.init()
                h = ctypes.c_void_p()
                with torch.cuda.device(idx):
                    rc = _hip_runtime().hipStreamCreateWithFlags(ctypes.byref(h), 1)
                if rc != 0 or not h.value:
                    raise RuntimeError(f'hipStreamCreateWithFlags failed ({rc})')
                st = _private_streams[key] = torch.cuda.ExternalStream(h.value, device=torch.device('cuda', idx))
    return st


capture_lock = threading.RLock()


class _NoGuard:
    def __enter__(self):
        return self

    def __exit__(self, *exc):
        return False


_NO_GUARD = _NoGuard()


def _dev_guard(device):
    if device is None:
        return _NO_GUARD
    idx = device.index if isinstance(device, torch.device) else device
    if idx is None or idx == torch.cuda.current_device():
        return _NO_GUARD
    return torch.cuda.device(idx)


_scope = threading.local()
_scope_finalizers = {}


def _drop_owner(domain):
    _scope_finalizers.pop(domain, None)
    for cache in (ModconvPlugin._ws, MappingPlugin._ws, LowresPlugin._ws):
        for k in [k for k in cache if domain in k]:
            del cache[k]


class workspace_scope:

    def __init__(self, owner):
        self.domain = ('owner', id(owner))
        if self.domain not in _scope_finalizers:
            _scope_finalizers[self.domain] = weakref.finalize(owner, _drop_owner, self.domain)

    def __enter__(self):
        self.prev = getattr(_scope, 'domain', None)
        _scope.domain = self.domain
        return self

    def __exit__(self, *exc):
        _scope.domain = self.prev
        return False


def _ws_domain(device):
    dom = getattr(_scope, 'domain', None)
    return dom if dom is not None else ('stream', _stream_handle(device))


def _ptr(t):
    return ctypes.c_void_p(t.data_ptr()) if (t is not None and t.numel() > 0) else ctypes.c_void_p(0)


def _i64x4(vals):
    return (ctypes.c_int64 * 4)(*[int(v) for v in vals])


def _require(cond, msg):
    if not cond:
        raise RuntimeError(msg)


def _dense(t):
    return t.is_contiguous() or (t.ndim == 4 and t.is_contiguous(memory_format=torch.channels_last))



class BiasActPlugin:

    @staticmethod
    def bias_act(x, b, xref, yref, dy, grad, dim, act, alpha, gain, clamp):
        _require(x.is_cuda, 'x must reside on CUDA device')
        for name, t in (('b', b), ('xref', xref), ('yref', yref), ('dy', dy)):
            if t.numel():
                _require(t.device == x.device, f'{name} must reside on the same device as x')
                _require(t.dtype == x.dtype, f'{name} must have the same dtype as x')
        _require(x.dtype in _DTYPE_CODE, 'x must be float16, bfloat16, float32 or float64')
        _require(b.numel() == 0 or (b.ndim == 1 and 0 <= dim < x.ndim and b.shape[0] == x.shape[dim]),
                 'b must be a vector matching dimension `dim` of x')
        _require(b.numel() == 0 or b.is_contiguous(), 'b must be contiguous')
# ... 341 lines not shown
        p.rays_per_img, p.steps = rays_d_cam.shape[0], z_lin.shape[0]
        keep = [rays_d_cam, z_lin, cam2world]
        if jitter is not None:
            jitter = jitter.contiguous(); keep.append(jitter); p.jitter = jitter.data_ptr()
        if sigma_noise is not None:
            sigma_noise = sigma_noise.contiguous(); keep.append(sigma_noise); p.sigma_noise = sigma_noise.data_ptr()
        p.clamp_mode, p.last_back, p.white_back = int(clamp_mode), int(bool(last_back)), int(bool(white_back))
        p.max_depth = float(max_depth or 0.0)
        n, R = p.n, p.rays_per_img
        feat = torch.empty([n, p.feat_ch + p.seg_ch, R], dtype=torch.float32, device=dev)
        depth = torch.empty([n, R], dtype=torch.float32, device=dev)
        wsum = torch.empty([n, R], dtype=torch.float32, device=dev)
        p.out_feat, p.out_depth, p.out_wsum = feat.data_ptr(), depth.data_ptr(), wsum.data_ptr()
        with _dev_guard(dev):
            rc = load().ide3d_render_rays(ctypes.byref(p), _stream(tex_planes))
        if rc == -2:
            return None
        _check(rc, 'render_rays')
        return feat, depth, wsum

    @staticmethod
    def sample_voxel(tex_planes, geo_planes, mlp, pts, sigma_only=False):
        dev = tex_planes.device
        pts = pts.contiguous()
        _require(pts.is_cuda and pts.dtype == torch.float32 and pts.ndim == 3 and pts.shape[2] == 3, 'pts must be [n, m, 3] float32')
        p = _RenderParams()
        VolumeRenderPlugin._fill_render_params(p, tex_planes, geo_planes, mlp)
        n, m = pts.shape[0], pts.shape[1]
        _require(n == p.n, 'pts batch must match the tri-plane batch')
        width = p.feat_ch + p.seg_ch + 1
        out = None if sigma_only else torch.empty([n * m, width], dtype=torch.float32, device=dev)
        sig = torch.empty([n * m], dtype=torch.float32, device=dev) if sigma_only else None
        if m:
            with _dev_guard(dev):
                rc = load().ide3d_sample_voxel(ctypes.byref(p), _ptr(pts), m, _ptr(out), _ptr(sig), int(sigma_only), _stream(pts))
            if rc == -2:
                return None
            _check(rc, 'sample_voxel')
        return sig if sigma_only else out


    @staticmethod
    def _lattice(n, voxel_size, corner, scale):
        lat = _Lattice()
        lat.n, lat.voxel_size, lat.scale = int(n), float(voxel_size), float(scale)
        for i in range(3):
            lat.corner[i] = float(corner[i])
        return lat

    @staticmethod
    def lattice_points(n, voxel_size, corner, scale, first, count, device):
        device = torch.device(device)
        _require(device.type == 'cuda', 'lattice_points: CUDA device required')
        pts = torch.empty([count, 3], dtype=torch.float32, device=device)
        lat = VolumeRenderPlugin._lattice(n, voxel_size, corner, scale)
        with _dev_guard(device):
            rc = load().ide3d_lattice_points(ctypes.byref(lat), int(first), int(count), _ptr(pts), _stream(pts))
        _check(rc, 'lattice_points')
        return pts

    @staticmethod
    def density_lattice(tex_planes, geo_planes, mlp, n, voxel_size, corner, scale, first, count):
        p = _RenderParams()
        VolumeRenderPlugin._fill_render_params(p, tex_planes, geo_planes, mlp)
        lat = VolumeRenderPlugin._lattice(n, voxel_size, corner, scale)
        sig = torch.empty([p.n * int(count)], dtype=torch.float32, device=tex_planes.device)
        if count:
            with _dev_guard(tex_planes.device):
                rc = load().ide3d_density_lattice(ctypes.byref(p), ctypes.byref(lat), int(first), int(count), _ptr(sig), _stream(tex_planes))
            if rc == -2:
                return None
            _check(rc, 'density_lattice')
        return sig


class ModconvPlugin:
    _ws = {}
    _heads_declined = set()

    @staticmethod
    def _workspace(lib, x, w, n, cin, cout, h, wd, k, mode, per_image, arith):
        key = (0 if per_image else w.data_ptr(), tuple(w.shape), n, h, wd, mode, x.device.index, _ws_domain(x.device), arith)
        ent = ModconvPlugin._ws.get(key)
        if ent is None:
            nbytes = lib.ide3d_modconv_workspace_bytes(n, cin, cout, h, wd, k, mode, int(per_image))
            _require(nbytes >= 0, 'modconv2d: unsupported configuration')
            if len(ModconvPlugin._ws) > 1024:
                for k_dead in [k_ for k_, e_ in ModconvPlugin._ws.items() if e_[2] is not None and e_[2]() is None]:
                    del ModconvPlugin._ws[k_dead]
            ent = [torch.empty([max(nbytes // 4, 1)], dtype=torch.float32, device=x.device), None, None]
            ModconvPlugin._ws[key] = ent
        return ent

    @staticmethod
    def _params(lib, x, w, y, styles, dcoefs, noise, noise_strength, bias, act, alpha, gain, clamp, mode, arith, x_amax, y_amax):
        n, cin, h, wd = x.shape
        per_image = (w.ndim == 5)
        cout, _, k, _ = w.shape[-4:]
        ent = ModconvPlugin._workspace(lib, x, w, n, cin, cout, h, wd, k, mode, per_image, arith)
        p = _ModconvParams()
        p.x, p.w, p.y = x.data_ptr(), w.data_ptr(), (y.data_ptr() if y is not None else None)
        keep = []
        for name, t in (('styles', styles), ('dcoefs', dcoefs), ('noise', noise), ('bias', bias)):
            if t is not None:
                t = t.contiguous(); keep.append(t)
                _require(t.is_cuda and t.dtype == torch.float32, f'modconv2d: {name} must be float32 on GPU')
                _require(t.device == x.device, f'modconv2d: {name} must reside on the same device as x')
                setattr(p, name, t.data_ptr())
        p.n, p.cin, p.cout, p.h, p.w_, p.k = n, cin, cout, h, wd, k
        p.noise_strength = float(noise_strength)
        p.act, p.alpha, p.gain, p.clamp = int(act), float(alpha), float(gain), float(clamp)
        p.mode = mode
        p.weights_packed = int((not per_image) and ent[2] is not None and ent[2]() is w and ent[1] == w._version)
        p.w_batch_stride = (cout * cin * k * k) if per_image else 0
        p.arith = arith
        for name, t in (('x_amax', x_amax), ('y_amax', y_amax)):
            if t is not None:
                _require(t.is_cuda and t.device == x.device and t.dtype == torch.float32 and tuple(t.shape) == (n, AMAX_FLOATS) and t.is_contiguous(),
                         f'modconv2d: {name} must be a contiguous float32 [n, AMAX_FLOATS] tensor on the device of x')
                setattr(p, name, t.data_ptr())
        p.workspace, p.workspace_bytes = ent[0].data_ptr(), ent[0].numel() * 4
        return p, ent, keep

    @staticmethod
    def modconv2d(x, w, styles, dcoefs, noise, noise_strength, bias, act, alpha, gain, clamp, mode=0, arith=0, x_amax=None, y_amax=None, pad_rows=False):
        for t in (x, w):
            _require(t.is_cuda and t.dtype == torch.float32 and t.is_contiguous(), 'modconv2d: contiguous float32 CUDA tensors required')
        _require(w.device == x.device, 'modconv2d: w must reside on the same device as x')
        n, cin, h, wd = x.shape
        per_image = (w.ndim == 5)
        if per_image:
            _require(w.shape[0] == n and styles is None, 'modconv2d: per-image weights need w.shape[0] == batch and styles=None')
        cout, cin2, k, k2 = w.shape[-4:]
        _require(cin == cin2 and k == k2 and k in (1, 3), 'modconv2d: weight must be [cout, cin, k, k] with k in {1, 3}')
        _require(mode in (0, 1, 2), 'modconv2d: mode must be 0, 1 or 2')
        _require(mode != 1 or (k == 3 and h >= 3 and wd >= 3), 'modconv2d: mode 1 is a 3x3 stride-2 convolution on an input of at least 3x3')
        oh, ow = (2 * h + 1, 2 * wd + 1) if mode == 2 else (((h - 3) // 2 + 1, (wd - 3) // 2 + 1) if mode == 1 else (h, wd))
        pitch = (ow + 3) // 4 * 4 if (pad_rows and mode == 2) else ow
        y = torch.empty([n, cout, oh, pitch], dtype=torch.float32, device=x.device)
        lib = load()
        arith = int(arith) or int(lib.ide3d_get_conv_arithmetic())
        if arith == 16 and x_amax is None:
            arith = 6
        p, ent, keep = ModconvPlugin._params(lib, x, w, y, styles, dcoefs, noise, noise_strength, bias, act, alpha, gain, clamp, mode, arith, x_amax, y_amax)
        p.y_pitch = pitch if pitch != ow else 0
        with _dev_guard(x.device):
            rc = lib.ide3d_modconv2d(ctypes.byref(p), _stream(x))
        _check(rc, 'modconv2d')
        ent[1], ent[2] = (None, None) if per_image else (w._version, weakref.ref(w))
        return y if pitch == ow else y[..., :ow]

    @staticmethod
    def modconv2d_heads(x, w, styles, dcoefs, noise, noise_strength, bias, act, alpha, gain, clamp, head_w, head_bias, head_clamp,
                        want_x=True, arith=0):
        for t in (x, w, head_w):
            _require(t.is_cuda and t.dtype == torch.float32 and t.is_contiguous(), 'modconv2d_heads: contiguous float32 CUDA tensors required')
        n, cin, h, wd = x.shape
        cout = w.shape[0]
        _require(w.ndim == 4 and tuple(w.shape[1:]) == (cin, 3, 3), 'modconv2d_heads: w must be [cout, cin, 3, 3]')
        _require(head_w.ndim == 5 and head_w.shape[0] == n and head_w.shape[2] == cout and tuple(head_w.shape[3:]) == (1, 1),
                 'modconv2d_heads: head_w must be [n, rows, cout, 1, 1]')
        lib = load()
        arith = int(arith) or int(lib.ide3d_get_conv_arithmetic())
        if arith == 16:
            arith = 6
        rows = head_w.shape[1]
        shape_key = (n, cin, cout, h, wd, rows, arith)
        knob_off = 'IDE3D_MODCONV_NO_HEAD_FUSION' in os.environ
        if knob_off or shape_key in ModconvPlugin._heads_declined:
            return None
        y = torch.empty([n, cout, h, wd], dtype=torch.float32, device=x.device) if want_x else None
        heads = torch.empty([n, rows, h, wd], dtype=torch.float32, device=x.device)
        p, ent, keep = ModconvPlugin._params(lib, x, w, y, styles, dcoefs, noise, noise_strength, bias, act, alpha, gain, clamp, 0, arith, None, None)
        hent = ModconvPlugin._workspace(lib, heads, head_w, n, cout, rows, h, wd, 1, 0, True, arith)
        e = _ModconvHeadEpilogue()
        e.w, e.y, e.rows, e.clamp, e.no_activation_output = head_w.data_ptr(), heads.data_ptr(), rows, float(head_clamp), int(not want_x)
        if head_bias is not None:
            head_bias = head_bias.contiguous()
            _require(head_bias.is_cuda and head_bias.dtype == torch.float32 and head_bias.numel() == rows, 'modconv2d_heads: head_bias must be float32 [rows] on GPU')
            e.bias = head_bias.data_ptr()
        e.workspace, e.workspace_bytes = hent[0].data_ptr(), hent[0].numel() * 4
        with _dev_guard(x.device):
            rc = lib.ide3d_modconv2d_heads(ctypes.byref(p), ctypes.byref(e), _stream(x))
        if rc == -2:
            ModconvPlugin._heads_declined.add(shape_key)
            return None
        _check(rc, 'modconv2d_heads')
        ent[1], ent[2] = w._version, weakref.ref(w)
        return y, heads


def modconv_plan(n, cin, cout, h, w, k=3, mode=0, per_image=False, arith=0, epilogue='conv', x_amax=False):
    p = _ModconvParams()
    p.n, p.cin, p.cout, p.h, p.w_, p.k, p.mode = n, cin, cout, h, w, k, mode
    p.arith = int(arith)
    p.w_batch_stride = cout * cin * k * k if per_image else 0
    dummy = 256
    p.x = p.w = p.y = dummy
    if not per_image:
        p.styles = p.dcoefs = dummy
    if epilogue == 'conv':
        p.noise, p.bias, p.noise_strength, p.act, p.alpha, p.gain, p.clamp = dummy, dummy, 1.0, 3, 0.2, math.sqrt(2.0), -1.0
    elif epilogue == 'plain':
        p.act, p.gain, p.clamp = 1, 1.0, -1.0
    elif epilogue == 'head':
        p.bias, p.act, p.gain, p.clamp = dummy, 1, 1.0, 256.0
    else:
        raise ValueError(epilogue)
    if x_amax:
        p.x_amax = dummy
    info = _ModconvPlanInfo()
    rc = load().ide3d_modconv_plan(ctypes.byref(p), ctypes.byref(info))
    if rc != 0:
        raise RuntimeError(f'modconv_plan failed (code {rc}): ' + load().ide3d_last_error().decode('utf-8', 'replace'))
    out = {name: getattr(info, name) for name, _ in _ModconvPlanInfo._fields_ if name != 'reserved'}
    out['kind'] = PLAN_KINDS[info.kind]
    return out


_ARITH_NAMES = {'fp32': 1, 'bf16x3': 3, 'bf16x6': 6, 'f16x3': 16, 'default': 0}


def conv_arithmetic(name=None):
    lib = load()
    if name is not None:
        _require(name in _ARITH_NAMES, f'conv_arithmetic: one of {sorted(_ARITH_NAMES)}')
        _check(lib.ide3d_set_conv_arithmetic(_ARITH_NAMES[name]), 'set_conv_arithmetic')
    code = int(lib.ide3d_get_conv_arithmetic())
    return {1: 'fp32', 3: 'bf16x3', 6: 'bf16x6', 16: 'f16x3'}[code]


class StylePlugin:
    @staticmethod
    def style_demod(w, affine_w, affine_b, affine_gain, bias_gain, wsq_t=None):
        _require(w.is_cuda and w.dtype == torch.float32 and w.ndim == 2 and w.stride(1) == 1, 'style_demod: w must be float32 [n, wdim] with unit inner stride')
        n, wdim = w.shape
        cin = affine_w.shape[0]
        _require(affine_w.is_contiguous() and affine_w.dtype == torch.float32 and affine_w.shape[1] == wdim, 'style_demod: bad affine weight')
        for name, t in (('affine_w', affine_w), ('affine_b', affine_b), ('wsq_t', wsq_t)):
            _require(t is None or t.device == w.device, f'style_demod: {name} must reside on the same device as w')
        styles = torch.empty([n, cin], dtype=torch.float32, device=w.device)
        dcoefs = None
        cout = 0
        if wsq_t is not None:
            _require(wsq_t.is_contiguous() and wsq_t.shape[0] == cin, 'style_demod: wsq_t must be contiguous [cin, cout]')
            cout = wsq_t.shape[1]
            dcoefs = torch.empty([n, cout], dtype=torch.float32, device=w.device)
        with _dev_guard(w.device):
            rc = load().ide3d_style_demod(_ptr(w), w.stride(0), _ptr(affine_w), _ptr(affine_b), _ptr(wsq_t), n, cin, cout, wdim,
                                          float(affine_gain), float(bias_gain), _ptr(styles), _ptr(dcoefs), _stream(w))
        _check(rc, 'style_demod')
        return styles, dcoefs

    @staticmethod
    def fold_heads(w, affine_gain, a0, b0, w0, gain0, a1, b1, w1, gain1):
        _require(w.is_cuda and w.dtype == torch.float32 and w.ndim == 2 and w.stride(1) == 1, 'fold_heads: w must be float32 [n, wdim]')
        n, wdim = w.shape
        cout0, cin = w0.shape[0], w0.shape[1]
        cout1 = w1.shape[0]
        for t in (a0, b0, w0, a1, b1, w1):
            _require(t.is_cuda and t.dtype == torch.float32 and t.is_contiguous(), 'fold_heads: contiguous float32 CUDA tensors required')
            _require(t.device == w.device, 'fold_heads: all tensors must reside on the same device as w')
        out = torch.empty([n, cout0 + cout1, cin, 1, 1], dtype=torch.float32, device=w.device)
        with _dev_guard(w.device):
            rc = load().ide3d_fold_heads(_ptr(w), w.stride(0), n, cin, wdim, float(affine_gain), _ptr(a0), _ptr(b0), _ptr(w0), cout0, float(gain0),
                                         _ptr(a1), _ptr(b1), _ptr(w1), cout1, float(gain1), _ptr(out), _stream(w))
        _check(rc, 'fold_heads')
        return out

    @staticmethod
    def style_demod_batch(jobs):
        if not jobs:
            return []
        w0 = jobs[0][0]
        n, wdim = w0.shape
        if n > 8:
            return None
        dev = w0.device
        tot_s = sum(j[1].shape[0] for j in jobs)
        tot_d = sum(j[5].shape[1] for j in jobs if j[5] is not None)
        sbuf = torch.empty([n * tot_s], dtype=torch.float32, device=dev)
        dbuf = torch.empty([max(n * tot_d, 1)], dtype=torch.float32, device=dev)
        arr = (_StyleJob * len(jobs))()
        outs, so, do = [], 0, 0
        for k, (w, aw, ab, again, bgain, wsq_t) in enumerate(jobs):
            _require(w.is_cuda and w.dtype == torch.float32 and w.ndim == 2 and w.stride(1) == 1 and tuple(w.shape) == (n, wdim) and w.device == dev,
                     'style_demod_batch: every w must be float32 [n, wdim] with unit inner stride on one device')
            cin = aw.shape[0]
            _require(aw.is_contiguous() and aw.shape[1] == wdim and aw.dtype == torch.float32 and aw.device == dev, 'style_demod_batch: affine weight must be contiguous float32 [cin, wdim]')
            _require(ab is None or (ab.is_contiguous() and ab.numel() == cin and ab.device == dev), 'style_demod_batch: affine bias must be contiguous [cin]')
            styles = sbuf[so:so + n * cin].view(n, cin); so += n * cin
            dco, cout = None, 0
            if wsq_t is not None:
                _require(wsq_t.is_contiguous() and wsq_t.shape[0] == cin and wsq_t.device == dev, 'style_demod_batch: wsq_t must be contiguous [cin, cout]')
                cout = wsq_t.shape[1]
                dco = dbuf[do:do + n * cout].view(n, cout); do += n * cout
            j = arr[k]
            j.w, j.w_stride = w.data_ptr(), w.stride(0)
            j.affine_w, j.affine_b = aw.data_ptr(), (ab.data_ptr() if ab is not None else None)
            j.wsq_t = wsq_t.data_ptr() if wsq_t is not None else None
            j.cin, j.cout, j.affine_gain, j.bias_gain = cin, cout, float(again), float(bgain)
            j.styles, j.dcoefs = styles.data_ptr(), (dco.data_ptr() if dco is not None else None)
            outs.append((styles, dco))
        lib = load()
        with _dev_guard(dev):
            for k0 in range(0, len(jobs), STYLE_BATCH_MAX):
                cnt = min(STYLE_BATCH_MAX, len(jobs) - k0)
                rc = lib.ide3d_style_demod_batch(ctypes.cast(ctypes.byref(arr, k0 * ctypes.sizeof(_StyleJob)), ctypes.POINTER(_StyleJob)),
                                                 cnt, n, wdim, _stream(w0))
                _check(rc, 'style_demod_batch')
        return outs

    @staticmethod
    def fold_heads_batch(jobs):
        if not jobs:
            return []
        w_0 = jobs[0][0]
        n, wdim = w_0.shape
        dev = w_0.device
        sizes = [(j[4].shape[0] + j[8].shape[0]) * j[4].shape[1] for j in jobs]
        buf = torch.empty([n * sum(sizes)], dtype=torch.float32, device=dev)
        arr = (_FoldJob * len(jobs))()
        outs, off = [], 0
        for k, (w, again, a0, b0, w0, g0, a1, b1, w1, g1) in enumerate(jobs):
            _require(w.is_cuda and w.dtype == torch.float32 and w.ndim == 2 and w.stride(1) == 1 and tuple(w.shape) == (n, wdim) and w.device == dev,
                     'fold_heads_batch: every w must be float32 [n, wdim] with unit inner stride on one device')
            for t in (a0, b0, w0, a1, b1, w1):
                _require(t.is_cuda and t.dtype == torch.float32 and t.is_contiguous() and t.device == dev, 'fold_heads_batch: contiguous float32 CUDA tensors required')
            cout0, cin = w0.shape[0], w0.shape[1]
            cout1 = w1.shape[0]
            _require(w1.shape[1] == cin and a0.shape == (cin, wdim) and a1.shape == (cin, wdim), 'fold_heads_batch: head shapes do not agree')
            out = buf[off:off + n * sizes[k]].view(n, cout0 + cout1, cin, 1, 1); off += n * sizes[k]
            j = arr[k]
            j.w, j.w_stride, j.cin, j.affine_gain = w.data_ptr(), w.stride(0), cin, float(again)
            j.a0, j.b0, j.w0, j.cout0, j.gain0 = a0.data_ptr(), b0.data_ptr(), w0.data_ptr(), cout0, float(g0)
            j.a1, j.b1, j.w1, j.cout1, j.gain1 = a1.data_ptr(), b1.data_ptr(), w1.data_ptr(), cout1, float(g1)
            j.out = out.data_ptr()
            outs.append(out)
        lib = load()
        with _dev_guard(dev):
# ... 270 lines not shown
```

### ide-3d_amd/training/graph_cache.py

```python

import collections
import contextlib
import os
import threading
import warnings
import weakref

import torch

_tls = threading.local()
_caches = weakref.WeakKeyDictionary()
_pools = {}

STATS = collections.Counter()


_PASS_ENV = ('IDE3D_NO_SKIP_MERGE', 'IDE3D_NO_STYLE_PREFETCH', 'IDE3D_NO_STYLE_BATCH', 'IDE3D_GATHER_PC', 'IDE3D_NO_LOWRES_GROUP', 'IDE3D_LOWRES_PERSISTENT')


def _env_int(name, default):
    try:
        return int(os.environ.get(name, default))
    except ValueError:
        return default


def enabled():
    return os.environ.get('IDE3D_AUTO_GRAPH', '1') != '0' and not getattr(_tls, 'off', 0)


@contextlib.contextmanager
def disabled():
    _tls.off = getattr(_tls, 'off', 0) + 1
    try:
        yield
    finally:
        _tls.off -= 1


def reset(module=None):
    if module is None:
        for c in list(_caches.values()):
            c.clear()
    elif module in _caches:
        _caches[module].clear()


def stats(module):
    c = _caches.get(module)
    return {'graphs': 0 if c is None else len(c.entries), 'seen': 0 if c is None else len(c.seen)}


def tree_stamp(root):
    acc = []
    push = acc.append
    requires_grad = False
    hooked = False
    stack = [root]
    while stack:
        m = stack.pop()
        if m._forward_hooks or m._forward_pre_hooks:
            hooked = True
        for p in m._parameters.values():
            if p is not None:
                push(p._version); push(p.data_ptr())
                if p.requires_grad:
                    requires_grad = True
        for b in m._buffers.values():
            if b is not None:
                push(b._version); push(b.data_ptr())
        for sub in m._modules.values():
            if sub is not None:
                stack.append(sub)
    return hash(tuple(acc)), requires_grad, hooked


def _global_hooks():
    mod = torch.nn.modules.module
    return bool(getattr(mod, '_global_forward_hooks', None)) or bool(getattr(mod, '_global_forward_pre_hooks', None))


class _Captured:
    __slots__ = ('graph', 'ws', 'c', 'jitter', 'jitter_given', 'out', 'planes', 'tensors', 'aliases', 'versions', '__weakref__')

    def untouched(self):
        v = 0
        for t in self.tensors:
            v += t._version
        return v == self.versions


class _ModuleGraphs:
    def __init__(self):
        self.entries = collections.OrderedDict()
        self.seen = {}
        self.stamp = None
        self.evictions = 0
        self.lock = threading.RLock()

    def clear(self):
        if self.entries:
            torch.cuda.synchronize(next(iter(self.entries.values())).ws.device)
        self.entries.clear()
        self.seen.clear()
        self.evictions = 0


def _out_tensors(out):
    if isinstance(out, dict):
        return list(out.values())
    return list(out) if isinstance(out, (tuple, list)) else [out]


def _fresh(out, caller_planes):
    memo = {}

    def cp(t):
        if not torch.is_tensor(t):
            return t
        base = t._base
        if (base is not None and base.ndim >= 2 and base.is_contiguous() and t.ndim == base.ndim and t.stride() == base.stride()
                and t.shape[0] == base.shape[0] and t.shape[2:] == base.shape[2:]):
            nb = memo.get(id(base))
            if nb is None:
                nb = memo[id(base)] = base.clone()
            off = (t.data_ptr() - base.data_ptr()) // (base.stride(1) * base.element_size())
            return nb[:, off:off + t.shape[1]]
        return t.clone()

    if isinstance(out, dict):
        res = {}
        for k, v in out.items():
            if k == 'planes':
                res[k] = caller_planes if caller_planes is not None else tuple(cp(p) for p in v)
            else:
                res[k] = cp(v)
        return res
    if isinstance(out, (tuple, list)):
        return type(out)(cp(t) for t in out)
    return cp(out)


def run(module, impl, ws, c, render_params, noise_mode, flags, force_fp32, ray_jitter, cached_planes, extra_kwargs, kind='synthesis'):
    why = _ineligible(module, ws, c, render_params, noise_mode, ray_jitter, cached_planes, extra_kwargs)
    if why is not None:
        STATS['ineligible:' + why] += 1
        return impl(ws, c, ray_jitter, cached_planes)

    from torch_utils import hip_plugin
    from training import networks
    cache = _caches.get(module)
    if cache is None:
        cache = _caches.setdefault(module, _ModuleGraphs())
    with cache.lock:
        return _run_locked(cache, module, impl, ws, c, render_params, noise_mode, flags, force_fp32, ray_jitter, cached_planes, kind)


def _run_locked(cache, module, impl, ws, c, render_params, noise_mode, flags, force_fp32, ray_jitter, cached_planes, kind):
    from torch_utils import hip_plugin
    from training import networks
    sp = module.spec
    n = ws.shape[0]
    steps = render_params.get('num_steps') or sp.num_steps
    jit_kind = 'none' if ray_jitter is False else ('draw' if ray_jitter is None else 'given')
    planes_key = None
    if cached_planes is not None:
        planes_key = tuple((p.data_ptr(), tuple(p.shape), p.stride()) for p in cached_planes)
    dev = ws.device
    sig = (kind, n, tuple(ws.shape[1:]), None if c is None else (tuple(c.shape), c.dtype), noise_mode, flags, bool(force_fp32), jit_kind, planes_key,
           render_params.get('fov'), steps, render_params.get('ray_start'), render_params.get('ray_end'),
           hip_plugin.conv_arithmetic(), networks.use_hip_modconv, torch.is_grad_enabled(), dev.index, hip_plugin._stream_handle(dev),
           bool(getattr(module, 'style_prefetch', True)),
           module.training, tuple(ch.training for ch in module.children()), tuple(os.environ.get(k) for k in _PASS_ENV))

    def current(stamp, requires_grad, hooked):
        if hooked or _global_hooks():
            return 'forward hook'
        if torch.is_grad_enabled() and (requires_grad or ws.requires_grad):
            return 'autograd'
        if cache.stamp != stamp:
            return 'parameters changed'
        return None

    ent = cache.entries.get(sig)
    replayable = not (torch.is_grad_enabled() and ws.requires_grad) and not module._forward_hooks and not module._forward_pre_hooks and not _global_hooks()
    if ent is not None and replayable and ent.untouched():
        cache.entries.move_to_end(sig)
        gen = torch.cuda.default_generators[dev.index if dev.index is not None else torch.cuda.current_device()]
        offset = gen.get_offset() if (ent.jitter is not None and not ent.jitter_given) else None
        out = _replay(ent, ws, c, ray_jitter, cached_planes)
        why = current(*tree_stamp(module))
        if why is None:
            STATS['replay'] += 1
            return out
        del out
        if offset is not None:
            gen.set_offset(offset)
        STATS['replay_discarded'] += 1

    stamp, requires_grad, hooked = tree_stamp(module)
    if cache.stamp != stamp:
        cache.clear()
        cache.stamp = stamp
    why = current(stamp, requires_grad, hooked)
    if why is not None:
        STATS['ineligible:' + why] += 1
        return impl(ws, c, ray_jitter, cached_planes)

    seen = cache.seen.get(sig, 0)
    if seen < _env_int('IDE3D_AUTO_GRAPH_AFTER', 1) << min(cache.evictions, 6):
        if len(cache.seen) > 256:
            cache.seen.clear()
        cache.seen[sig] = seen + 1
        STATS['eager'] += 1
        return impl(ws, c, ray_jitter, cached_planes)
    try:
        with hip_plugin.capture_lock:
            ent = _capture(module, impl, ws, c, ray_jitter, cached_planes, steps, sig)
    except Exception as e:
        warnings.warn(f'ide3d graph_cache: capture of G.synthesis failed ({type(e).__name__}: {e}); this call signature stays eager')
        cache.seen[sig] = -(1 << 60)
        STATS['capture_failed'] += 1
        return impl(ws, c, ray_jitter, cached_planes)
    cache.entries[sig] = ent
    cache.seen.pop(sig, None)
    while len(cache.entries) > max(1, _env_int('IDE3D_AUTO_GRAPH_MAX', 6)):
        torch.cuda.synchronize(ws.device)
        cache.entries.popitem(last=False)
        cache.evictions += 1
    STATS['capture'] += 1
    STATS['replay'] += 1
    return _replay(ent, ws, c, ray_jitter, cached_planes)


def _replay(ent, ws, c, ray_jitter, cached_planes):
    with torch.no_grad():
        ent.ws.copy_(ws, non_blocking=True)
        if ent.c is not None:
            ent.c.copy_(c, non_blocking=True)
        if ent.jitter is not None:
            if ent.jitter_given:
                ent.jitter.copy_(ray_jitter, non_blocking=True)
            else:
                ent.jitter.uniform_()
    ent.graph.replay()
    return _fresh(ent.out, cached_planes)


def _ineligible(module, ws, c, render_params, noise_mode, ray_jitter, cached_planes, extra_kwargs):
    if not enabled() or not getattr(module, 'auto_graph', True):
        return 'switched off'
    if not (torch.is_tensor(ws) and ws.is_cuda and ws.ndim == 3 and (c is None or (torch.is_tensor(c) and c.device == ws.device and c.ndim == 2))):
        return 'not device tensors'
    if ws.device.index is not None and ws.device.index != torch.cuda.current_device():
        return 'tensors on a device that is not the current one'
    if torch.cuda.is_current_stream_capturing():
        return 'capture in progress'
    if noise_mode not in ('const', 'none'):
        return 'random noise'
    if extra_kwargs:
        return 'unknown keyword arguments'
    sp = module.spec
    if render_params.get('nerf_noise') or render_params.get('importance_u') is not None:
        return 'device draws inside the pass'
    hier = render_params.get('hierarchical')
    if hier or (hier is None and sp.hierarchical):
        return 'hierarchical pass'
    for k in ('fov', 'num_steps', 'ray_start', 'ray_end'):
        v = render_params.get(k)
        if v is not None and not isinstance(v, (int, float)):
            return 'non-scalar render parameter'
    if ray_jitter is not None and ray_jitter is not False:
        steps = render_params.get('num_steps') or sp.num_steps
        if not (torch.is_tensor(ray_jitter) and ray_jitter.device == ws.device
# ... 50 lines not shown
```

### ide-3d_amd/training/networks.py

```python

import math
import weakref

import numpy as np
import torch

from dnnlib import util
from torch_utils import custom_ops
from torch_utils import misc
from torch_utils import persistence
from torch_utils.ops import bias_act
from torch_utils.ops import conv2d_resample
from torch_utils.ops import fma
from torch_utils.ops import upfirdn2d

_modconv_plugin = None

use_hip_modconv = True


def _upfirdn_plugin():
    upfirdn2d._init()
    return upfirdn2d._plugin

# ... 245 lines not shown
        _wscale_cache[id(weight)] = ent
    return ent[2]


def _scaled_const_noise(noise_const, noise_strength):
    if torch.is_grad_enabled() and (noise_strength.requires_grad or noise_const.requires_grad):
        return noise_const * noise_strength
    ent = _noise_cache.get(id(noise_const))
    if (ent is None or ent[0]() is not noise_const or ent[1]() is not noise_strength
            or ent[2] != (_stamp(noise_const), _stamp(noise_strength))):
        _evict_dead(_noise_cache)
        ent = (weakref.ref(noise_const), weakref.ref(noise_strength), (_stamp(noise_const), _stamp(noise_strength)),
               (noise_const * noise_strength).detach())
        _noise_cache[id(noise_const)] = ent
    return ent[3]
_eps_cache = {}


def _eps_like(t):
    k = (t.device, t.dtype)
    if k not in _eps_cache:
        _eps_cache[k] = torch.full([1], 1e-8, device=t.device, dtype=t.dtype)
    return _eps_cache[k]


@misc.profiled_function
def modulated_conv2d(
    x,
    weight,
    styles,
    noise           = None,
    up              = 1,
    down            = 1,
    padding         = 0,
    resample_filter = None,
    demodulate      = True,
    flip_weight     = True,
    fused_modconv   = True,
    mode            = '2d',
    **unused,
):
    assert mode == '2d', 'only 2-D modulated convolutions are part of the render path'
    batch_size = x.shape[0]
    cout, cin, kh, kw = weight.shape

    if (use_hip_modconv and up == 1 and down == 1 and kh == kw and kh in (1, 3) and padding == kh // 2 and flip_weight
            and _inference_on_gpu(x, weight, styles) and _modconv_init()):
        dcoefs = _demod_coefs(weight, styles) if demodulate else None
        y = _modconv_plugin.modconv2d(x.contiguous(), weight.contiguous(), styles.contiguous(), dcoefs,
                                      None, 0.0, None, 1, 0.0, 1.0, -1.0)
        if noise is not None:
            y = y.add_(noise)
        return y

    if x.dtype == torch.float16 and demodulate:
        weight = weight * (1 / np.sqrt(cin * kh * kw) / weight.norm(float('inf'), dim=[1, 2, 3], keepdim=True))
        styles = styles / styles.norm(float('inf'), dim=1, keepdim=True)

    if not fused_modconv:
        dcoefs = _demod_coefs(weight, styles) if demodulate else None
        x = x * styles.to(x.dtype).reshape(batch_size, -1, 1, 1)
        x = conv2d_resample.conv2d_resample(x=x, w=weight.to(x.dtype), f=resample_filter, up=up, down=down,
                                            padding=padding, flip_weight=flip_weight)
        if demodulate and noise is not None:
            x = fma.fma(x, dcoefs.to(x.dtype).reshape(batch_size, -1, 1, 1), noise.to(x.dtype))
        elif demodulate:
            x = x * dcoefs.to(x.dtype).reshape(batch_size, -1, 1, 1)
        elif noise is not None:
            x = x.add_(noise.to(x.dtype))
        return x

    w = weight.unsqueeze(0) * styles.reshape(batch_size, 1, -1, 1, 1)
    if demodulate:
        dcoefs = (w.square().sum(dim=[2, 3, 4]) + 1e-8).rsqrt()
        w = w * dcoefs.reshape(batch_size, -1, 1, 1, 1)
    with misc.suppress_tracer_warnings():
        batch_size = int(batch_size)
    x = x.reshape(1, -1, *x.shape[2:])
    w = w.reshape(-1, cin, kh, kw)
    x = conv2d_resample.conv2d_resample(x=x, w=w.to(x.dtype), f=resample_filter, up=up, down=down, padding=padding,
                                        groups=batch_size, flip_weight=flip_weight)
    x = x.reshape(batch_size, -1, *x.shape[2:])
    if noise is not None:
        x = x.add_(noise)
    return x


def _modconv_bias_act(x, weight, styles, demodulate, noise2d, noise_strength, bias, act, gain, clamp, dcoefs=None):
    cout, cin, kh, kw = weight.shape
    if not (use_hip_modconv and kh == kw and kh in (1, 3) and act in ('linear', 'lrelu')
            and _inference_on_gpu(x, weight, styles, bias) and _modconv_init()):
        return None
    spec = bias_act.activation_funcs[act]
    if demodulate and dcoefs is None:
        dcoefs = _demod_coefs(weight, styles)
    amax = _amax_wanted(x) if kh == 3 else None
    xc = x.contiguous()
    return _with_amax(_modconv_plugin.modconv2d(
        xc, weight.contiguous(), styles.contiguous(), dcoefs, noise2d, noise_strength, bias,
        spec.cuda_idx, spec.def_alpha, gain, -1.0 if clamp is None else clamp,
        x_amax=(_amax_of(x) if xc is x else None), y_amax=amax), amax)


def _folded_head_weights(torgb, toseg, w):
    if not (w.ndim == 2 and w.stride(1) == 1 and torgb.weight.shape[2] == 1 and _inference_on_gpu(w, torgb.weight, toseg.weight)
            and _style_init()):
        return None
    return _style_plugin.fold_heads(w, torgb.affine.weight_gain,
                                    torgb.affine.weight, torgb.affine.bias, torgb.weight.reshape(torgb.weight.shape[0], -1), torgb.weight_gain,
                                    toseg.affine.weight, toseg.affine.bias, toseg.weight.reshape(toseg.weight.shape[0], -1), toseg.weight_gain)


def _adjacent_views(a, b):
    if a is None or b is None or a._base is None or a._base is not b._base:
        return None
    t = a._base
    if (t.ndim != 4 or a.ndim != 4 or b.ndim != 4 or not t.is_contiguous() or t.shape[1] != a.shape[1] + b.shape[1]
            or a.shape[0] != t.shape[0] or a.shape[2:] != t.shape[2:] or b.shape[0] != t.shape[0] or b.shape[2:] != t.shape[2:]
            or a.stride() != t.stride() or b.stride() != t.stride()
            or a.data_ptr() != t.data_ptr() or b.data_ptr() != t.data_ptr() + a.shape[1] * t.stride(1) * t.element_size()):
        return None
    return t


def _dual_head_weights(torgb, toseg, w):
    wcat = _take_prefetched(torgb, w) if _prefetch_table() else None
    if wcat is None:
        wcat = _folded_head_weights(torgb, toseg, w)
    if wcat is None:
        s_rgb = torgb.affine(w) * torgb.weight_gain
        s_seg = toseg.affine(w) * toseg.weight_gain
        wr = torgb.weight[None, :, :, 0, 0] * s_rgb[:, None, :]
        ws = toseg.weight[None, :, :, 0, 0] * s_seg[:, None, :]
        wcat = torch.cat([wr, ws], dim=1)[:, :, :, None, None].contiguous()
    return wcat


def _dual_head(x, torgb, toseg, w, wcat=None):
    if not (use_hip_modconv and torgb.weight.shape[2] == 1 and torgb.conv_clamp == toseg.conv_clamp
            and _inference_on_gpu(x, w, torgb.weight, toseg.weight) and _modconv_init()):
        return None
    n = x.shape[0]
    if w.shape[0] != n:
        return None
    if wcat is None:
        wcat = _dual_head_weights(torgb, toseg, w)
    bias = _cat_cached(torgb.bias, toseg.bias)
    clamp = -1.0 if torgb.conv_clamp is None else torgb.conv_clamp
    y = _modconv_plugin.modconv2d(x.contiguous(), wcat, None, None, None, 0.0, bias, 1, 0.0, 1.0, clamp)
    co = torgb.weight.shape[0]
    return y[:, :co], y[:, co:]


def _conv1_dual_head(block, x, w1, w_shared, want_x, noise_mode='random', gain=1, input_noise=None, **unused):
    c1, tr, ts = block.conv1, block.torgb, block.toseg
    if not (use_hip_modconv and type(c1) is SynthesisLayer and c1.up == 1 and c1.padding == 1 and c1.weight.shape[2:] == (3, 3)
            and c1.activation in ('linear', 'lrelu') and tr.weight.shape[2] == 1 and tr.conv_clamp == ts.conv_clamp
            and x.ndim == 4 and x.shape[0] == w1.shape[0] == w_shared.shape[0]
            and _inference_on_gpu(x, w1, w_shared, c1.weight, c1.bias, tr.weight, ts.weight)
            and not _hooked(block, c1, tr, ts) and _modconv_init()):
        return None
    from torch_utils import hip_plugin
    if hip_plugin.conv_arithmetic() != 'bf16x6':
        return None
    noise = None
    if c1.use_noise and noise_mode != 'none':
        if input_noise is not None or noise_mode != 'const' or tuple(c1.noise_const.shape) != tuple(x.shape[2:]):
            return None
        noise = _scaled_const_noise(c1.noise_const, c1.noise_strength)
    styles, dcoefs = _styles_and_dcoefs(c1.affine, w1, c1.weight, True)
    if dcoefs is None:
        dcoefs = _demod_coefs(c1.weight, styles)
    spec = bias_act.activation_funcs[c1.activation]
    act_gain = c1.act_gain * gain
    act_clamp = c1.conv_clamp * gain if c1.conv_clamp is not None else None
    bias = c1.bias.to(x.dtype)
    wcat = _dual_head_weights(tr, ts, w_shared)
    hbias = _cat_cached(tr.bias, ts.bias)
    hclamp = -1.0 if tr.conv_clamp is None else tr.conv_clamp
    xc = x.contiguous()
    out = _modconv_plugin.modconv2d_heads(xc, c1.weight.contiguous(), styles.contiguous(), dcoefs, noise, 1.0, bias,
                                          spec.cuda_idx, spec.def_alpha, act_gain, -1.0 if act_clamp is None else act_clamp,
                                          wcat, hbias, hclamp, want_x=want_x)
    if out is None:
        x = _modconv_bias_act(x, c1.weight, styles, True, noise, 1.0, bias, c1.activation, act_gain, act_clamp, dcoefs=dcoefs)
        return x, _dual_head(x, tr, ts, w_shared, wcat=wcat)
    x, y = out
    co = tr.weight.shape[0]
    return x, (y[:, :co], y[:, co:])


_lowres_plugin = None


def _lowres_init():
    global _lowres_plugin
    if _lowres_plugin is None:
        _lowres_plugin = custom_ops.get_plugin(module_name='lowres_plugin', sources=['lowres.hip'])
    return True


def _hooked(*modules):
    from torch.nn.modules import module as _m
    if _m._global_forward_hooks or _m._global_forward_pre_hooks:
        return True
    return any(m._forward_hooks or m._forward_pre_hooks for m in modules)


def lowres_group_forward(blocks, ws_per_block, noise_mode='const', force_fp32=False, **other_kwargs):
    if os.environ.get('IDE3D_NO_LOWRES_GROUP') or not use_hip_modconv or other_kwargs or noise_mode not in ('const', 'none'):
        return None
    if not blocks or len(blocks) != len(ws_per_block):
        return None
    b0 = blocks[0]
    ws0 = ws_per_block[0]
    if not (torch.is_tensor(ws0) and ws0.is_cuda and ws0.dtype == torch.float32) or (torch.is_grad_enabled() and ws0.requires_grad):
        return None
    if b0.in_channels != 0 or b0.use_single_layer or not hasattr(b0, 'const') or not _inference_on_gpu(b0.const, b0.conv1.weight):
        return None
    from torch_utils import hip_plugin
    if hip_plugin.conv_arithmetic() not in ('bf16x6', 'bf16x3'):
        return None
    C, n = b0.out_channels, ws0.shape[0]
    if C % 32 != 0 or n > 8:
        return None
    cand = []
    for bi, blk in enumerate(blocks):
        ok = (blk.architecture == 'skip' and not blk.use_single_layer and blk.out_channels == C and (bi == 0 or blk.in_channels == C)
              and not (blk.use_fp16 and not force_fp32) and not getattr(blk, 'skip_channels_last', False)
              and blk.torgb.conv_clamp == blk.toseg.conv_clamp and blk.torgb.weight.shape[2] == 1 and blk._filter_is_1331()
              and blk.resolution == b0.resolution << bi
              and not _hooked(blk, blk.conv1, blk.torgb, blk.toseg, *([blk.conv0] if bi else [])))
        if not ok:
            break
        for name in (('conv1',) if bi == 0 else ('conv0', 'conv1')):
            lay = getattr(blk, name)
            if not (lay.activation == 'lrelu' and lay.weight.shape == (C, C, 3, 3) and lay.padding == 1 and lay.up == (2 if name == 'conv0' else 1)
                    and _inference_on_gpu(ws0, lay.weight, lay.bias) and lay.weight.is_contiguous()
                    and (not lay.use_noise or noise_mode == 'none' or lay.noise_const.shape[-1] == blk.resolution)):
                ok = False
                break
            cand.append((bi, name, lay))
        if not ok:
            cand = [c for c in cand if c[0] < bi]
            break
    if not cand or not _lowres_init():
        return None
    ups = [lay.up for _, _, lay in cand]
    fit = _lowres_plugin.layers_supported(n, C, b0.resolution, ups)
    if fit < 1:
        return None
    cand = cand[:fit]
    last_bi, last_name, _ = cand[-1]
    resume = last_name == 'conv0'
    nheads = last_bi if resume else last_bi + 1
    if nheads > hip_plugin.LOWRES_MAX_HEADS or (nheads == 0):
        return None
    layers, heads = [], []
    for bi, name, lay in cand:
        blk, wsb = blocks[bi], ws_per_block[bi]
        w = wsb[:, (0 if (bi == 0 or name == 'conv0') else 1)]
        styles, dcoefs = _styles_and_dcoefs(lay.affine, w, lay.weight, True)
        noise = None
        if lay.use_noise and noise_mode == 'const':
            noise = _scaled_const_noise(lay.noise_const, lay.noise_strength)
        layers.append(dict(weight=lay.weight, styles=styles, dcoefs=dcoefs, noise=noise, bias=lay.bias, act_gain=lay.act_gain,
                           clamp=(-1.0 if lay.conv_clamp is None else lay.conv_clamp), up=lay.up,
                           head=(bi if (name == 'conv1' and bi < nheads) else -1)))
    for bi in range(nheads):
        blk, wsb = blocks[bi], ws_per_block[bi]
        w = wsb[:, blk.num_conv]
        wcat = _take_prefetched(blk.torgb, w) if _prefetch_table() else None
        if wcat is None:
            wcat = _folded_head_weights(blk.torgb, blk.toseg, w)
        if wcat is None:
            return None
        heads.append(dict(w=wcat, bias=_cat_cached(blk.torgb.bias, blk.toseg.bias), clamp=(-1.0 if blk.torgb.conv_clamp is None else blk.torgb.conv_clamp)))
    x, skips = _lowres_plugin.group(b0.const.detach(), layers, heads, b0.resample_filter)
    co = blocks[0].torgb.weight.shape[0]
    skip = skips[-1]
    return x, skip[:, :co], skip[:, co:], nheads, resume


@persistence.persistent_class
class FullyConnectedLayer(torch.nn.Module):

    def __init__(self, in_features, out_features, bias=True, activation='linear', lr_multiplier=1, bias_init=0):
        super().__init__()
        self.activation = activation
        self.weight = torch.nn.Parameter(torch.randn([out_features, in_features]) / lr_multiplier)
        self.bias = torch.nn.Parameter(torch.full([out_features], np.float32(bias_init))) if bias else None
        self.weight_gain = lr_multiplier / np.sqrt(in_features)
        self.bias_gain = lr_multiplier

    def effective(self, dtype=torch.float32):
        w = self.weight.to(dtype) * self.weight_gain
        b = self.bias
        if b is not None:
            b = b.to(dtype)
            if self.bias_gain != 1:
                b = b * self.bias_gain
        return w, b

    def forward(self, x):
        if _inference_on_gpu(x, self.weight, self.bias):
            w = _scaled_weight(self.weight, self.weight_gain)
            b = None if self.bias is None else (_scaled_weight(self.bias, self.bias_gain) if self.bias_gain != 1 else self.bias)
        else:
            w, b = self.effective(x.dtype)
        if self.activation == 'linear' and b is not None:
            return torch.addmm(b.unsqueeze(0), x, w.t())
        x = x.matmul(w.t())
        return bias_act.bias_act(x, b, act=self.activation)


@persistence.persistent_class
class Conv2dLayer(torch.nn.Module):

    def __init__(self, in_channels, out_channels, kernel_size, bias=True, activation='linear', up=1, down=1,
                 resample_filter=[1, 3, 3, 1], conv_clamp=None, channels_last=False, trainable=True, **unused):
        super().__init__()
        self.activation = activation
        self.up = up
        self.down = down
        self.conv_clamp = conv_clamp
        self.register_buffer('resample_filter', upfirdn2d.setup_filter(resample_filter))
        self.padding = kernel_size // 2
        self.weight_gain = 1 / np.sqrt(in_channels * (kernel_size ** 2))
        self.act_gain = bias_act.activation_funcs[activation].def_gain
        memory_format = torch.channels_last if channels_last else torch.contiguous_format
        weight = torch.randn([out_channels, in_channels, kernel_size, kernel_size]).to(memory_format=memory_format)
        bias = torch.zeros([out_channels]) if bias else None
        if trainable:
            self.weight = torch.nn.Parameter(weight)
            self.bias = torch.nn.Parameter(bias) if bias is not None else None
        else:
            self.register_buffer('weight', weight)
            if bias is not None:
                self.register_buffer('bias', bias)
            else:
                self.bias = None

# ... 135 lines not shown

    def __init__(self, in_channels, out_channels, w_dim, resolution, kernel_size=3, up=1, use_noise=True,
                 activation='lrelu', resample_filter=[1, 3, 3, 1], conv_clamp=None, channels_last=False, **unused_kwargs):
        super().__init__()
        self.resolution = resolution
        self.up = up
        self.use_noise = use_noise
        self.activation = activation
        self.conv_clamp = conv_clamp
        self.register_buffer('resample_filter', upfirdn2d.setup_filter(resample_filter))
        self.padding = kernel_size // 2
        self.act_gain = bias_act.activation_funcs[activation].def_gain
        self.affine = FullyConnectedLayer(w_dim, in_channels, bias_init=1)
        memory_format = torch.channels_last if channels_last else torch.contiguous_format
        self.weight = torch.nn.Parameter(torch.randn([out_channels, in_channels, kernel_size, kernel_size]).to(memory_format=memory_format))
        if use_noise:
            self.register_buffer('noise_const', torch.randn([resolution, resolution]))
            self.noise_strength = torch.nn.Parameter(torch.zeros([]))
        self.bias = torch.nn.Parameter(torch.zeros([out_channels]))

    def forward(self, x, w, noise_mode='random', fused_modconv=True, gain=1, input_noise=None, **unused_kwargs):
        assert noise_mode in ['random', 'const', 'none']
        styles, dcoefs_pre = _styles_and_dcoefs(self.affine, w, self.weight, True)
        if styles.size(0) < x.size(0):
            dcoefs_pre = None
            assert x.size(0) % styles.size(0) == 0
            styles = styles.repeat_interleave(x.size(0) // styles.size(0), dim=0)

        noise = None
        const_noise = False
        if self.use_noise:
            if input_noise is not None:
                noise = input_noise * self.noise_strength
            elif noise_mode == 'random':
                noise = torch.randn([x.shape[0], 1, self.up * x.shape[2], self.up * x.shape[3]], device=x.device) * self.noise_strength
            elif noise_mode == 'const':
                const_noise = self.noise_const.shape[-1] >= self.up * x.shape[3]
                noise = _scaled_const_noise(self.noise_const, self.noise_strength)
                if not const_noise:
                    noise = noise.repeat(1, self.up * x.shape[3] // noise.shape[-1])

        act_gain = self.act_gain * gain
        act_clamp = self.conv_clamp * gain if self.conv_clamp is not None else None

        if (self.up == 2 and use_hip_modconv and self.weight.shape[2] == 3 and self.padding == 1
                and _inference_on_gpu(x, self.weight, styles, self.bias) and _modconv_init()):
            dcoefs = dcoefs_pre if dcoefs_pre is not None else _demod_coefs(self.weight, styles)
            xc = x.contiguous()
            y = _modconv_plugin.modconv2d(xc, self.weight.contiguous(), styles.contiguous(), dcoefs,
                                          None, 0.0, None, 1, 0.0, 1.0, -1.0, mode=2, x_amax=(_amax_of(x) if xc is x else None), pad_rows=True)
            spec = bias_act.activation_funcs[self.activation]
            if self.activation in ('linear', 'lrelu') and (noise is None or (noise.ndim == 2 and noise.shape == (2 * x.shape[2], 2 * x.shape[3]))):
                amax = _amax_wanted(y)
                return _with_amax(_upfirdn_plugin().upfirdn2d_ex(y, self.resample_filter, 1, 1, 1, 1, 1, 1, 1, 1, False, 4.0,
                                                                 noise=noise, noise_strength=1.0, bias=self.bias, act=spec.cuda_idx,
                                                                 alpha=spec.def_alpha, act_gain=act_gain,
                                                                 clamp=(-1.0 if act_clamp is None else act_clamp), y_amax=amax), amax)
            y = upfirdn2d.upfirdn2d(y, self.resample_filter, padding=[1, 1, 1, 1], gain=4)
            if noise is not None:
                y = y.add_(noise)
            return bias_act.bias_act(y, self.bias.to(x.dtype), act=self.activation, gain=act_gain, clamp=act_clamp)
        if self.up == 1:
            if noise is None or (const_noise and input_noise is None and noise.shape == x.shape[2:]):
                y = _modconv_bias_act(x, self.weight, styles, True, noise, 1.0,
                                      self.bias.to(x.dtype), self.activation, act_gain, act_clamp, dcoefs=dcoefs_pre)
                if y is not None:
                    return y
        x = modulated_conv2d(x=x, weight=self.weight, styles=styles, noise=noise, up=self.up, padding=self.padding,
                             resample_filter=(self.resample_filter if self.up > 1 else None), flip_weight=(self.up == 1),
                             fused_modconv=(fused_modconv and not _inference_on_gpu(x, self.weight, styles)))
        return bias_act.bias_act(x, self.bias.to(x.dtype), act=self.activation, gain=act_gain, clamp=act_clamp)


@persistence.persistent_class
class ToRGBLayer(torch.nn.Module):

    def __init__(self, in_channels, out_channels, w_dim, kernel_size=1, conv_clamp=None, channels_last=False, **unused):
        super().__init__()
        self.conv_clamp = conv_clamp
        self.affine = FullyConnectedLayer(w_dim, in_channels, bias_init=1)
        memory_format = torch.channels_last if channels_last else torch.contiguous_format
        self.weight = torch.nn.Parameter(torch.randn([out_channels, in_channels, kernel_size, kernel_size]).to(memory_format=memory_format))
        self.bias = torch.nn.Parameter(torch.zeros([out_channels]))
        self.weight_gain = 1 / np.sqrt(in_channels * (kernel_size ** 2))

    def forward(self, x, w, fused_modconv=True):
        styles = self.affine(w) * self.weight_gain
        if x.size(0) > styles.size(0):
            assert x.size(0) % styles.size(0) == 0
            styles = styles.repeat_interleave(x.size(0) // styles.size(0), dim=0)
        y = _modconv_bias_act(x, self.weight, styles, False, None, 0.0, self.bias.to(x.dtype), 'linear', 1.0, self.conv_clamp)
        if y is not None:
            return y
        x = modulated_conv2d(x=x, weight=self.weight, styles=styles, demodulate=False, fused_modconv=fused_modconv)
        return bias_act.bias_act(x, self.bias.to(x.dtype), clamp=self.conv_clamp)


@persistence.persistent_class
class SegSynthesisBlock(torch.nn.Module):

    def __init__(self, in_channels, out_channels, w_dim, resolution, img_channels, seg_channels, is_last,
                 architecture='skip', resample_filter=[1, 3, 3, 1], conv_clamp=None, use_fp16=False,
                 fp16_channels_last=False, use_single_layer=False, disable_upsample=False, **layer_kwargs):
        assert architecture in ['orig', 'skip']
        super().__init__()
        self.in_channels, self.out_channels = in_channels, out_channels
        self.w_dim, self.resolution = w_dim, resolution
        self.img_channels, self.seg_channels = img_channels, seg_channels
        self.is_last, self.architecture = is_last, architecture
        self.use_fp16 = use_fp16
        self.channels_last = (use_fp16 and fp16_channels_last)
        self.use_single_layer = use_single_layer
        self.register_buffer('resample_filter', upfirdn2d.setup_filter(resample_filter))
        self.num_conv = self.num_torgb = self.num_toseg = 0
        layer_name = layer_kwargs.pop('layer_name', 'training.networks.SynthesisLayer')

        if in_channels == 0:
            self.const = torch.nn.Parameter(torch.randn([out_channels, resolution, resolution]))
        else:
            self.conv0 = util.construct_class_by_name(
                class_name=layer_name, in_channels=in_channels, out_channels=out_channels, w_dim=w_dim,
                resolution=resolution, up=(1 if disable_upsample else 2), resample_filter=resample_filter,
                conv_clamp=conv_clamp, channels_last=self.channels_last, **layer_kwargs)
            self.num_conv += 1
        if not use_single_layer:
            self.conv1 = util.construct_class_by_name(
                class_name=layer_name, in_channels=out_channels, out_channels=out_channels, w_dim=w_dim,
                resolution=resolution, conv_clamp=conv_clamp, channels_last=self.channels_last, **layer_kwargs)
            self.num_conv += 1
        if is_last or architecture == 'skip':
            self.torgb = ToRGBLayer(out_channels, img_channels, w_dim=w_dim, conv_clamp=conv_clamp, channels_last=self.channels_last)
            self.num_torgb += 1
            self.toseg = ToRGBLayer(out_channels, seg_channels, w_dim=w_dim, conv_clamp=conv_clamp, channels_last=self.channels_last)
            self.num_toseg += 1

    def _merge_skip(self, skip, x):
        if skip is None:
            return None
        if skip.size(-1) * 2 == x.size(-1):
            return upfirdn2d.upsample2d(skip, self.resample_filter)
        if skip.size(-1) == x.size(-1):
            return skip
        raise NotImplementedError

    def _accumulate(self, lo, cur, y):
        if lo is not None:
            if (getattr(self, 'skip_channels_last', False) and lo.shape[1] % 4 == 0 and self.resample_filter.shape == (4, 4)
                    and _inference_on_gpu(lo, y) and self._filter_is_1331() and _resample_init()):
                return _resample_plugin.skip_upsample_add_cl(lo, y)
            f = self.resample_filter
            return _upfirdn_plugin().upfirdn2d_ex(lo, f, 2, 2, 1, 1, 2, 1, 2, 1, False, 4.0, add=y)
        return cur.add_(y) if cur is not None else y

    def _filter_is_1331(self):
        ok = getattr(self, '_f1331', None)
        if ok is None:
            ref = upfirdn2d.setup_filter([1, 3, 3, 1])
            ok = self._f1331 = bool(torch.equal(self.resample_filter.detach().cpu(), ref))
        return ok

    def forward(self, x, img, seg, ws, force_fp32=False, fused_modconv=None, block_noise=None, disable_rgb=False, **layer_kwargs):
        misc.assert_shape(ws, [None, self.num_conv + self.num_torgb, self.w_dim])
        resume_after_conv0 = bool(layer_kwargs.pop('_resume_after_conv0', False))
        x_unused = bool(layer_kwargs.pop('_x_unused', False))
        ws_list = ws.unbind(dim=1)
        w_iter = iter(ws_list)
        dtype = torch.float16 if self.use_fp16 and not force_fp32 else torch.float32
        memory_format = torch.channels_last if self.channels_last and not force_fp32 else torch.contiguous_format
        out_dtype = dtype
        if dtype == torch.float16 and ws.is_cuda and not torch.is_grad_enabled() and use_hip_modconv:
            dtype, memory_format = torch.float32, torch.contiguous_format
        if fused_modconv is None:
            with misc.suppress_tracer_warnings():
                fused_modconv = (not self.training) and (dtype == torch.float32 or int(ws.shape[0]) == 1)

        fused = fused_heads = None
        if self.in_channels == 0:
            x = self.const.to(dtype=dtype, memory_format=memory_format)
            x = x.unsqueeze(0).expand(ws.shape[0], *x.size())
            if not self.use_single_layer:
                layer_kwargs['input_noise'] = block_noise[:, 1:2] if block_noise is not None else None
                x = self.conv1(x, next(w_iter), fused_modconv=fused_modconv, **layer_kwargs)
        else:
            x = x.to(dtype=dtype, memory_format=memory_format)
            layer_kwargs['input_noise'] = block_noise[:, 0:1] if block_noise is not None else None
            if resume_after_conv0:
                next(w_iter)
            else:
                x = self.conv0(x, next(w_iter), fused_modconv=fused_modconv, **layer_kwargs)
            if not self.use_single_layer:
                layer_kwargs['input_noise'] = block_noise[:, 1:2] if block_noise is not None else None
                w1 = next(w_iter)
                if (self.is_last or self.architecture == 'skip') and not disable_rgb and dtype == torch.float32:
                    fused = _conv1_dual_head(self, x, w1, ws_list[self.num_conv], not x_unused, **layer_kwargs)
                if fused is not None:
                    x, fused_heads = fused
                else:
                    x = self.conv1(x, w1, fused_modconv=fused_modconv, **layer_kwargs)

        w_shared = next(w_iter) if (self.is_last or self.architecture == 'skip') else None
        ref = x if x is not None else fused_heads[0]
        img_lo = seg_lo = None
        heads_follow = (self.is_last or self.architecture == 'skip') and not disable_rgb
        if heads_follow and _inference_on_gpu(ref) and img is not None and seg is not None and img.size(-1) * 2 == ref.size(-1):
            img_lo, seg_lo, img, seg = img, seg, None, None
        else:
            img = self._merge_skip(img, ref)
            seg = self._merge_skip(seg, ref)
        if self.is_last or self.architecture == 'skip':
            if disable_rgb:
                img = seg = None
            else:
                heads = fused_heads if fused_heads is not None else _dual_head(x, self.torgb, self.toseg, w_shared)
                if heads is not None:
                    y, y_seg = heads
                else:
                    y = self.torgb(x, w_shared, fused_modconv=fused_modconv).to(dtype=torch.float32, memory_format=torch.contiguous_format)
                    y_seg = self.toseg(x, w_shared, fused_modconv=fused_modconv).to(dtype=torch.float32, memory_format=torch.contiguous_format)
                lo_both, y_both = _adjacent_views(img_lo, seg_lo), _adjacent_views(y, y_seg)
                if (lo_both is not None and y_both is not None and img is None and seg is None and not getattr(self, 'skip_channels_last', False)
                        and not self.is_last and not os.environ.get('IDE3D_NO_SKIP_MERGE')):
                    both = self._accumulate(lo_both, None, y_both)
                    img, seg = both[:, :y.shape[1]], both[:, y.shape[1]:]
                else:
                    img = self._accumulate(img_lo, img, y)
                    seg = self._accumulate(seg_lo, seg, y_seg)
        assert x is None or x.dtype == dtype
        if x is not None and out_dtype != dtype:
            x = x.to(out_dtype)
        assert img is None or img.dtype == torch.float32
        assert seg is None or seg.dtype == torch.float32
        return x, img, seg
```

### ide-3d_amd/training/video_render.py

```python

import math
import threading
import weakref
from typing import Iterable, Iterator, Sequence, Tuple

import numpy as np
import scipy.interpolate
import torch

from training import distributed_render as dr
from training import triplane
from training.volumetric_rendering import LookAtPoseSampler, device_const

INTRINSICS = ((4.2647, 0, 0.5), (0, 4.2647, 0.5), (0, 0, 1))


def sweep_pose(frame_idx: int, total_frames: int, lookat, radius: float = 2.7, yaw_range: float = 0.5, pitch_range: float = 0.25,
               device='cpu') -> torch.Tensor:
    t = 2 * math.pi * frame_idx / total_frames
    cam2world = LookAtPoseSampler.sample(math.pi / 2 - yaw_range * np.sin(t), math.pi / 2 - 0.05 + pitch_range * np.cos(t),
                                         lookat, radius=radius, device=device)
    intr = device_const([v for row in INTRINSICS for v in row], torch.float32, device).reshape(3, 3)
    return torch.cat([cam2world.reshape(-1, 16), intr.reshape(-1, 9)], 1)


def interpolate_ws(ws_keyframes: np.ndarray, w_frames: int, kind: str = 'cubic', wraps: int = 2) -> np.ndarray:
    k = ws_keyframes.shape[0]
    x = np.arange(-k * wraps, k * (wraps + 1))
    y = np.tile(ws_keyframes, [wraps * 2 + 1, 1, 1])
    interp = scipy.interpolate.interp1d(x, y, kind=kind, axis=0)
    return interp(np.arange(k * w_frames) / w_frames).astype(np.float32)


_plane_pool = weakref.WeakKeyDictionary()
_plane_pool_lock = threading.Lock()


def _checkout_plane_buffers(synthesis, planes):
    if not planes[0].is_cuda:
        return planes, None
    with _plane_pool_lock:
        pool = _plane_pool.setdefault(synthesis, [])
        ent = next((e for e in pool if not e[1] and all(b.shape == t.shape and b.stride() == t.stride() and b.device == t.device and b.dtype == t.dtype
                                                        for b, t in zip(e[0], planes))), None)
        if ent is None:
            ent = [tuple(torch.empty_like(t) for t in planes), False]
            pool.append(ent)
            del pool[:-8]
        ent[1] = True
    for b, t in zip(ent[0], planes):
        b.copy_(t)
    return ent[0], ent


def _release_plane_buffers(token):
    if token is not None:
        with _plane_pool_lock:
            token[1] = False


def layout_u8(frames: torch.Tensor, grid_w: int, grid_h: int) -> torch.Tensor:
    n, h, w, c = frames.shape
    assert n == grid_w * grid_h
    return frames.reshape(grid_h, grid_w, h, w, c).permute(0, 2, 1, 3, 4).reshape(grid_h * h, grid_w * w, c)


@torch.no_grad()
def gen_interp_frames(G, seeds: Sequence[int], shuffle_seed=None, w_frames: int = 60 * 4, kind: str = 'cubic',
                      grid_dims: Tuple[int, int] = (1, 1), num_keyframes=None, wraps: int = 2, psi: float = 1, truncation_cutoff=14,
                      cfg: str = 'FFHQ', image_mode: str = 'image_seg', device=torch.device('cuda'), noise_mode: str = 'const',
                      cache_static_planes: bool = True, **synthesis_kwargs) -> Iterator[torch.Tensor]:
    grid_w, grid_h = grid_dims
    cells = grid_w * grid_h
    if num_keyframes is None:
        if len(seeds) % cells != 0:
            raise ValueError('Number of input seeds must be divisible by grid W*H')
        num_keyframes = len(seeds) // cells
    if image_mode not in ('image', 'image_seg'):
        raise ValueError("image_mode must be 'image' or 'image_seg'")
    all_seeds = np.array([seeds[i % len(seeds)] for i in range(num_keyframes * cells)], dtype=np.int64)
    if shuffle_seed is not None:
        np.random.RandomState(seed=shuffle_seed).shuffle(all_seeds)
    lookat = torch.tensor([0, 0, 0.2] if cfg == 'FFHQ' else [0, 0, 0], dtype=torch.float32, device=device)

    zs = torch.from_numpy(np.stack([np.random.RandomState(int(s)).randn(G.z_dim) for s in all_seeds])).to(device).float()
    front = LookAtPoseSampler.sample(math.pi / 2, math.pi / 2, lookat, radius=2.7, device=device)
    c_front = torch.cat([front.reshape(-1, 16), device_const([v for row in INTRINSICS for v in row], torch.float32, device).reshape(-1, 9)], 1)
    ws = G.mapping(zs, c_front.repeat(len(zs), 1), truncation_psi=psi, truncation_cutoff=truncation_cutoff)
    ws = ws.reshape(grid_h, grid_w, num_keyframes, *ws.shape[1:]).cpu().numpy()
    total = num_keyframes * w_frames
    ws_frames = torch.from_numpy(np.stack([interpolate_ws(ws[yi][xi], w_frames, kind, wraps)
                                           for yi in range(grid_h) for xi in range(grid_w)])).to(device)
    static = cache_static_planes and num_keyframes == 1 and bool(torch.allclose(ws_frames, ws_frames[:, :1].expand_as(ws_frames), atol=1e-5))
    planes = token = None
    if static:
        planes, token = _checkout_plane_buffers(G.synthesis, G.synthesis.planes(ws_frames[:, 0], noise_mode=noise_mode))
    palette = dr.palette_tensor(G.synthesis.seg_channels, device)
    try:
        for frame_idx in range(total):
            c = sweep_pose(frame_idx, total, lookat, device=device).repeat(cells, 1)
            img, seg = G.synthesis(ws_frames[:, frame_idx], c=c, noise_mode=noise_mode, return_seg=True, cached_planes=planes, **synthesis_kwargs)
            if image_mode == 'image_seg':
                cell_frames = dr.frames_u8(img, seg, palette)
            else:
                cell_frames = (img.float() * 127.5 + 128).clamp(0, 255).to(torch.uint8).permute(0, 2, 3, 1).contiguous()
            yield layout_u8(cell_frames, grid_w, grid_h)
    finally:
        _release_plane_buffers(token)



def rgb_u8_to_yuv444(frame: torch.Tensor) -> torch.Tensor:
    assert frame.dtype == torch.uint8 and frame.ndim == 3 and frame.shape[2] == 3
    rgb = frame.to(torch.int32)
    r, g, b = rgb[..., 0], rgb[..., 1], rgb[..., 2]
    y = 16 + ((66 * r + 129 * g + 25 * b + 128) >> 8)
    cb = 128 + ((-38 * r - 74 * g + 112 * b + 128) >> 8)
    cr = 128 + ((112 * r - 94 * g - 18 * b + 128) >> 8)
    return torch.stack([y, cb, cr]).clamp_(0, 255).to(torch.uint8)


def write_y4m(frames: Iterable[torch.Tensor], path: str, fps: int = 60) -> int:
    count = 0
    with open(path, 'wb') as f:
        for frame in frames:
            if count == 0:
                h, w = int(frame.shape[0]), int(frame.shape[1])
                f.write(f'YUV4MPEG2 W{w} H{h} F{int(fps)}:1 Ip A1:1 C444\n'.encode('ascii'))
            assert tuple(frame.shape[:2]) == (h, w), 'all frames of a stream have one size'
            f.write(b'FRAME\n')
            f.write(rgb_u8_to_yuv444(frame).cpu().numpy().tobytes())
            count += 1
    return count


def read_y4m(path: str):
    with open(path, 'rb') as f:
        head = f.readline().decode('ascii').split()
        assert head[0] == 'YUV4MPEG2' and 'C444' in head
        info = {t[0]: t[1:] for t in head[1:]}
        w, h = int(info['W']), int(info['H'])
        frames = []
        while True:
            line = f.readline()
            if not line:
                break
            assert line.startswith(b'FRAME')
            frames.append(np.frombuffer(f.read(3 * h * w), dtype=np.uint8).reshape(3, h, w))
    return info, np.stack(frames) if frames else np.zeros((0, 3, h, w), np.uint8)
```

### include/ide3d_hip.h

```cpp
#ifndef IDE3D_HIP_H_
#define IDE3D_HIP_H_

#include <stdint.h>

#ifdef __cplusplus
extern "C" {
#endif


#define IDE3D_OK            0
#define IDE3D_EINVAL       (-1)
#define IDE3D_ENOKERNEL    (-2)
#define IDE3D_ELAUNCH      (-3)

#define IDE3D_F32  0
#define IDE3D_F16  1
#define IDE3D_BF16 2
#define IDE3D_F64  3

const char* ide3d_last_error(void);
int         ide3d_abi_version(void);
const char* ide3d_build_arch(void);
const char* ide3d_build_flags(void);
int         ide3d_exclusive_violations(void);
// ... 25 lines not shown
int ide3d_upfirdn2d(const ide3d_upfirdn2d_params* p, void* stream);

#define IDE3D_AMAX_SLOTS  32
#define IDE3D_AMAX_STRIDE 64
#define IDE3D_AMAX_FLOATS (IDE3D_AMAX_SLOTS * IDE3D_AMAX_STRIDE)

typedef struct ide3d_upfirdn2d_epilogue {
    const void*  add;
    int64_t      add_stride[4];
    const float* noise;
    float        noise_strength;
    const void*  bias;
    int32_t      fused_act;
    int32_t      act;
    float        alpha, act_gain, clamp;
    float*       y_amax;
} ide3d_upfirdn2d_epilogue;

int ide3d_upfirdn2d_ex(const ide3d_upfirdn2d_params* p, const ide3d_upfirdn2d_epilogue* ep, void* stream);

typedef struct ide3d_filtered_lrelu_params {
    const void*  x;
    void*        y;
    const void*  b;
    uint8_t*     s;
    const float* fu;
    const float* fd;
    int32_t dtype;
    int32_t n, c, in_h, in_w;
    int32_t out_h, out_w;
    int64_t x_stride[4];
    int64_t y_stride[4];
    int32_t fu_w, fu_h;
    int32_t fd_w, fd_h;
    int64_t fu_stride[2];
    int64_t fd_stride[2];
    int32_t up, down;
    int32_t pad_x0, pad_y0;
    int32_t s_w_bytes, s_h;
    int32_t s_ofs_x, s_ofs_y;
    int32_t sw_limit;
    int32_t sign_mode;
    int32_t flip;
    float   gain, slope, clamp;
} ide3d_filtered_lrelu_params;

int ide3d_filtered_lrelu(const ide3d_filtered_lrelu_params* p, void* stream);

int ide3d_filtered_lrelu_act(void* x, uint8_t* s, int dtype,
                             int32_t n, int32_t c, int32_t h, int32_t w,
                             const int64_t x_stride[4],
                             int32_t s_w, int32_t s_h, int32_t s_ofs_x, int32_t s_ofs_y,
                             float gain, float slope, float clamp, int sign_mode, void* stream);

int ide3d_triplane_sample(const float* planes, const int64_t plane_stride[4],
                          int32_t n, int32_t C, int32_t H, int32_t W,
                          const float* coords, int64_t m, float* out, void* stream);

int ide3d_triplane_sample_rays(const float* planes, const int64_t plane_stride[4],
                               int32_t n, int32_t C, int32_t H, int32_t W,
                               const float* coords, int64_t m, float* out,
                               int32_t rays_h, int32_t rays_w, int32_t steps, void* stream);

int ide3d_triplane_taps(int32_t H, int32_t W, const float* coords, int64_t n_times_m,
                        int32_t* taps, void* stream);

int ide3d_triplane_sample_backward(const float* grad_out, const float* planes,
                                   const int64_t plane_stride[4],
                                   int32_t n, int32_t C, int32_t H, int32_t W,
                                   const float* coords, int64_t m,
                                   float* grad_planes, const int64_t grad_plane_stride[4],
                                   float* grad_coords, void* stream);

int ide3d_composite(const float* rgb_sigma, const float* z_vals, const float* dir_norm,
                    const float* noise, int64_t rays, int32_t steps, int32_t ch,
                    int clamp_mode, int last_back, int white_back, float max_depth,
                    int fill_mode, float* rgb, float* depth, float* weights, void* stream);

int ide3d_sample_pdf(const float* bins, const float* weights, const float* u, int64_t u_ray_stride,
                     int64_t rays, int32_t k, int32_t n_importance, float eps, float* samples,
                     void* stream);

typedef struct ide3d_render_params {
    const float* rays_d_cam;
    const float* z_lin;
    const float* cam2world;
    const float* jitter;
    const float* sigma_noise;
    const float* tex_planes;
    const float* geo_planes;
    int64_t tex_stride[4];
    int64_t geo_stride[4];
    const float* geo_w0; const float* geo_b0; const float* geo_w1; const float* geo_b1;
    const float* tex_w0; const float* tex_b0; const float* tex_w1; const float* tex_b1;
    int32_t n, rays_per_img, steps;
    int32_t C, H, W;
    int32_t hidden, feat_ch, seg_ch;
    int32_t clamp_mode, last_back, white_back;
    float   max_depth;
    float*  out_feat;
    float*  out_depth;
    float*  out_wsum;
} ide3d_render_params;

int ide3d_render_rays(const ide3d_render_params* p, void* stream);

int ide3d_sample_voxel(const ide3d_render_params* p, const float* pts, int64_t m,
                       float* out, float* out_sigma, int sigma_only, void* stream);

typedef struct ide3d_lattice {
    int32_t n;
    float   voxel_size;
    float   corner[3];
    float   scale;
} ide3d_lattice;

int ide3d_lattice_points(const ide3d_lattice* lat, int64_t first, int64_t count, float* pts, void* stream);

int ide3d_density_lattice(const ide3d_render_params* p, const ide3d_lattice* lat, int64_t first, int64_t count,
                          float* out_sigma, void* stream);

typedef struct ide3d_modconv_params {
    const float* x; const float* w; const float* styles; const float* dcoefs;
    const float* noise; const float* bias; float* y;
    int32_t n, cin, cout, h, w_, k;
    float noise_strength;
    int32_t act; float alpha, gain, clamp;
    int32_t mode;
    int32_t weights_packed;
    float*  workspace;
    int64_t workspace_bytes;
    int64_t w_batch_stride;
    int32_t arith;
    const float* x_amax;
    float*       y_amax;
    int32_t      y_pitch;
} ide3d_modconv_params;

int64_t ide3d_modconv_workspace_bytes(int32_t n, int32_t cin, int32_t cout, int32_t h, int32_t w, int32_t k, int32_t mode,
                                      int32_t per_image_weights);
int ide3d_modconv2d(const ide3d_modconv_params* p, void* stream);

typedef struct ide3d_modconv_head_epilogue {
    const float* w;
    const float* bias;
    float*       y;
    int32_t      rows;
    float        clamp;
    int32_t      no_activation_output;
    float*       workspace;
    int64_t      workspace_bytes;
} ide3d_modconv_head_epilogue;
int ide3d_modconv2d_heads(const ide3d_modconv_params* p, const ide3d_modconv_head_epilogue* heads, void* stream);

enum { IDE3D_PLAN_FP32 = 0,
       IDE3D_PLAN_SPLIT = 1,
       IDE3D_PLAN_SPLIT_TEAMS = 2,
       IDE3D_PLAN_HEAD_SPLIT = 3,
       IDE3D_PLAN_HEAD_RESIDENT = 4,
       IDE3D_PLAN_HEAD_SMALL = 5 };
typedef struct ide3d_modconv_plan_info {
    int32_t kind;
    int32_t tile_h, tile_w;
    int32_t images_per_tile;
    int32_t rows;
    int32_t waves;
    int32_t parts, f16;
    int32_t split_k;
    int32_t strip;
    int32_t transposed_all_class;
    int32_t reserved;
    int64_t workgroups;
} ide3d_modconv_plan_info;
int ide3d_modconv_plan(const ide3d_modconv_params* p, ide3d_modconv_plan_info* out);

int     ide3d_set_conv_arithmetic(int32_t arith);
int32_t ide3d_get_conv_arithmetic(void);

int ide3d_style_demod(const float* w, int64_t w_stride, const float* affine_w, const float* affine_b, const float* wsq_t,
                      int32_t n, int32_t cin, int32_t cout, int32_t wdim, float affine_gain, float bias_gain,
                      float* styles, float* dcoefs, void* stream);

int ide3d_fold_heads(const float* w, int64_t w_stride, int32_t n, int32_t cin, int32_t wdim, float affine_gain,
                     const float* a0, const float* b0, const float* w0, int32_t cout0, float gain0,
                     const float* a1, const float* b1, const float* w1, int32_t cout1, float gain1,
                     float* out, void* stream);

#define IDE3D_STYLE_BATCH_MAX 24
typedef struct ide3d_style_job {
    const float* w; int64_t w_stride;
    const float* affine_w; const float* affine_b;
    const float* wsq_t;
    int32_t cin, cout;
    float affine_gain, bias_gain;
    float* styles; float* dcoefs;
} ide3d_style_job;
typedef struct ide3d_fold_job {
    const float* w; int64_t w_stride;
    int32_t cin; float affine_gain;
    const float *a0, *b0, *w0; int32_t cout0; float gain0;
    const float *a1, *b1, *w1; int32_t cout1; float gain1;
    float* out;
} ide3d_fold_job;
int ide3d_style_demod_batch(const ide3d_style_job* jobs, int32_t njobs, int32_t n, int32_t wdim, void* stream);
int ide3d_fold_heads_batch(const ide3d_fold_job* jobs, int32_t njobs, int32_t n, int32_t wdim, void* stream);

#define IDE3D_LOWRES_MAX_LAYERS 8
#define IDE3D_LOWRES_MAX_HEADS 4
typedef struct ide3d_lowres_layer {
    const float* weight;
    const float* styles;
    const float* dcoefs;
    const float* noise;
    const float* bias;
    float act_gain, clamp;
    int32_t up;
    int32_t head;
    int32_t weights_packed;
    int32_t reserved;
} ide3d_lowres_layer;
typedef struct ide3d_lowres_head {
    const float* w;
    const float* bias;
    float* skip;
    float clamp;
    int32_t O;
} ide3d_lowres_head;
typedef struct ide3d_lowres_params {
    const float* x0; int64_t x0_batch_stride;
    const float* fir;
    float* x_out;
    void* workspace; int64_t workspace_bytes;
    int32_t n, C, res0, nlayers, nheads;
    int32_t arith;
    int32_t persistent;
    int32_t reserved;
    ide3d_lowres_layer layers[IDE3D_LOWRES_MAX_LAYERS];
    ide3d_lowres_head heads[IDE3D_LOWRES_MAX_HEADS];
} ide3d_lowres_params;
int32_t ide3d_lowres_layers_supported(int32_t n, int32_t C, int32_t res0, const int32_t* ups, int32_t nlayers, int32_t arith);
int64_t ide3d_lowres_workspace_bytes(const ide3d_lowres_params* p);
int ide3d_lowres_group(const ide3d_lowres_params* p, void* stream);

typedef struct ide3d_mapping_params {
    const float* z; const float* c;
    const float* embed_w; const float* embed_b;
    const float* fc_w[16]; const float* fc_b[16];
    int32_t fc_out[16];
    const float* w_avg;
    float* ws;
    void* workspace; int64_t workspace_bytes;
    int32_t n, z_dim, c_dim, embed, layers, num_ws;
    float embed_weight_gain, embed_bias_gain, lr_multiplier, alpha, act_gain, truncation_psi;
    int32_t truncation_cutoff;
} ide3d_mapping_params;

int ide3d_mapping_workspace_bytes(void);
int ide3d_mapping_supported(void);
int ide3d_mapping(const ide3d_mapping_params* p, void* stream);

int ide3d_skip_upsample_add_cl(const float* lo, const int64_t lo_stride[4], const float* add, const int64_t add_stride[4],
                               int32_t n, int32_t c, int32_t h, int32_t w, float* out, void* stream);

int ide3d_bilinear_up2_split(const float* x, int32_t n, int32_t c, int32_t h, int32_t w,
                             float* const dst[3], const int32_t c_begin[3], const int32_t c_count[3], const int64_t* dst_batch_floats, void* stream);

int ide3d_frame_u8(const float* img, const float* seg, const uint8_t* palette,
                   int32_t n, int32_t classes, int32_t H, int32_t W, uint8_t* out, void* stream);

int ide3d_sphere_points(const float* theta, const float* pitch, int32_t n, float r, int32_t pitch_is_v,
                        float* pos, float* phi_out, void* stream);
int ide3d_cam2world(const float* forward, const float* origin, const float* lookat, int32_t lookat_stride, int32_t n,
                    float* out, void* stream);

#ifdef __cplusplus
}
#endif
#endif
```

Measured before the change: 910.8.

## Fuse skip-branch 2x bilinear upsample-add into the modconv heads epilogue

The fused conv1+toRGB/toSeg heads kernel now also loads the half-resolution img/seg skip patch into LDS. It upsamples the patch with the 1-3-3-1 filter, adds the head outputs and writes the merged skip image directly. This removes a separate upsample/add kernel and the round trip of the head outputs through memory. The cost is extra LDS traffic and synchronisation in the epilogue. Python plumbing, the plane pool and the graph cache now accept channels-last buffers.

```diff
diff --git a/ide-3d_amd/csrc/modconv.hip b/ide-3d_amd/csrc/modconv.hip
--- a/ide-3d_amd/csrc/modconv.hip
+++ b/ide-3d_amd/csrc/modconv.hip
@@ -602,8 +602,13 @@
     float clamp;
     int store_x;
     int bias_first;
+    const float* lo;
+    float* dst;
+    int64_t lo_s[4], dst_s[4];
+    int lo_h, lo_w;
 };
-template <int PH, int PW, int NWV, int MTW, int NTW, int BM, int MT, int PARTS, int SCRATCH>
+enum { HEAD_SKIP_NONE = 0, HEAD_SKIP_CL = 1, HEAD_SKIP_UP2 = 2 };
+template <int PH, int PW, int NWV, int MTW, int NTW, int BM, int MT, int PARTS, int SCRATCH, int SKIP = HEAD_SKIP_NONE>
 __device__ __forceinline__ void split_heads_finish(const ide3d_modconv_params& p, const HeadEpi& he, f32x16 (&acc)[1][MTW][NTW], float* smem,
                                                    int n0, int y0, int x0, int wm, int wn, int lp) {
     constexpr int NT = 64 * NWV, BN = PH * PW, TP = BN + 4, ROWS = MT * 32, CCH = BM / 16, A_UNITS = PARTS * 2 * ROWS;
@@ -704,6 +709,87 @@
         }
     }
     const float h_clamp = (he.clamp >= 0.f) ? he.clamp : __builtin_inff();
+    auto head_value = [&](float v, int row) {
+        if (he.bias_first) {
+            v = __builtin_amdgcn_fmed3f(v, -h_clamp, h_clamp);
+        } else {
+            v *= 1.f; v += 0.f; v += s_hb[row];
+            v = (v > 0.f) ? v : v * 1.f;
+            v = fminf(fmaxf(v, -h_clamp), h_clamp);
+        }
+        return v;
+    };
+    if constexpr (SKIP != HEAD_SKIP_NONE) {
+        constexpr int LH = PH / 2 + 2, LW = PW / 2 + 2, LP = ROWS + 4, NLO = (ROWS * LH * LW + NT - 1) / NT;
+        static_assert(LH * LW * LP <= BM * TP, "the skip patch must fit the activation tile (s_hb stays)");
+        __syncthreads();
+        float* const s_lo = smem;
+        const int m0 = y0 / 2 - 1, q0 = x0 / 2 - 1;
+        const float* __restrict__ lob = he.lo + (int64_t)n0 * he.lo_s[0];
+        float lv[NLO];
+#pragma unroll
+        for (int i = 0; i < NLO; ++i) {
+            const int e = tid + i * NT, lx = e % LW, ly = (e / LW) % LH, r = e / (LW * LH);
+            const int yy = m0 + ly, xx = q0 + lx;
+            lv[i] = 0.f;
+            if (r < he.rows && yy >= 0 && yy < he.lo_h && xx >= 0 && xx < he.lo_w)
+                lv[i] = lob[r * he.lo_s[1] + yy * he.lo_s[2] + xx * he.lo_s[3]];
+        }
+#pragma unroll
+        for (int i = 0; i < NLO; ++i) {
+            const int e = tid + i * NT, lx = e % LW, ly = (e / LW) % LH, r = e / (LW * LH);
+            if (r < ROWS) s_lo[(ly * LW + lx) * LP + r] = lv[i];
+        }
+        __syncthreads();
+        typedef float f32x4a __attribute__((ext_vector_type(4)));
+        const bool cl = he.dst_s[1] == 1;
+#pragma unroll
+        for (int t = 0; t < NTH; ++t) {
+            const int pix = (pg * NTH + t) * 32 + l32;
+            const int py = pix / PW, px = pix % PW, gy = y0 + py, gx = x0 + px;
+            const int ly = (py >> 1) + (gy & 1), lx = (px >> 1) + (gx & 1);
+            const float wy0 = (gy & 1) ? 0.75f : 0.25f, wy1 = 1.0f - wy0;
+            const float wx0 = (gx & 1) ? 0.75f : 0.25f, wx1 = 1.0f - wx0;
+            const float ay0 = (gy & 1) ? 3.f : 1.f, ay1 = (gy & 1) ? 1.f : 3.f, ax0 = (gx & 1) ? 3.f : 1.f, ax1 = (gx & 1) ? 1.f : 3.f;
+            const float g00 = ay0 * ax0 * 0.0625f, g01 = ay0 * ax1 * 0.0625f, g10 = ay1 * ax0 * 0.0625f, g11 = ay1 * ax1 * 0.0625f;
+            const float* const t00 = s_lo + (ly * LW + lx) * LP;
+            float* const o = he.dst + (int64_t)n0 * he.dst_s[0] + (int64_t)gy * he.dst_s[2] + (int64_t)gx * he.dst_s[3];
+#pragma unroll
+            for (int m = 0; m < MTH; ++m)
+#pragma unroll
+                for (int g = 0; g < 4; ++g) {
+                    const int row0 = (rg * MTH + m) * 32 + 8 * g + 4 * half;
+                    if (row0 >= he.rows) continue;
+                    const f32x4a a = *reinterpret_cast<const f32x4a*>(t00 + row0);
+                    const f32x4a b = *reinterpret_cast<const f32x4a*>(t00 + LP + row0);
+                    const f32x4a c = *reinterpret_cast<const f32x4a*>(t00 + LW * LP + row0);
+                    const f32x4a d = *reinterpret_cast<const f32x4a*>(t00 + (LW + 1) * LP + row0);
+                    f32x4a out;
+#pragma unroll
+                    for (int k = 0; k < 4; ++k) {
+                        float v;
+                        if constexpr (SKIP == HEAD_SKIP_CL) {
+                            v = __builtin_fmaf(wy0, __builtin_fmaf(wx0, a[k], wx1 * b[k]), wy1 * __builtin_fmaf(wx0, c[k], wx1 * d[k]));
+                        } else {
+                            v = __builtin_fmaf(a[k], g00, 0.f);
+                            v = __builtin_fmaf(b[k], g01, v);
+                            v = __builtin_fmaf(c[k], g10, v);
+                            v = __builtin_fmaf(d[k], g11, v);
+                        }
+                        out[k] = v + head_value(hacc[m][t][4 * g + k], row0 + k);
+                    }
+                    if (cl) {
+                        *reinterpret_cast<f32x4a*>(o + row0) = out;
+                    } else {
+#pragma unroll
+                        for (int k = 0; k < 4; ++k)
+                            if (row0 + k < he.rows) o[(int64_t)(row0 + k) * he.dst_s[1]] = out[k];
+                    }
+                }
+        }
+        __syncthreads();
+        return;
+    }
 #pragma unroll
     for (int t = 0; t < NTH; ++t) {
         const int pix = (pg * NTH + t) * 32 + l32;
@@ -715,21 +801,13 @@
             for (int r = 0; r < 16; ++r) {
                 const int row = (rg * MTH + m) * 32 + 8 * (r >> 2) + 4 * half + (r & 3);
                 if (row >= he.rows) continue;
-                float v = hacc[m][t][r];
-                if (he.bias_first) {
-                    v = __builtin_amdgcn_fmed3f(v, -h_clamp, h_clamp);
-                } else {
-                    v *= 1.f; v += 0.f; v += s_hb[row];
-                    v = (v > 0.f) ? v : v * 1.f;
-                    v = fminf(fmaxf(v, -h_clamp), h_clamp);
-                }
-                o[(int64_t)row * hw] = v;
+                o[(int64_t)row * hw] = head_value(hacc[m][t][r], row);
             }
     }
     __syncthreads();
 }
 
-template <int MODE, int BIG, int PH, int PARTS, int WBUF, int NWV, int F16, int TEAMS = 1, int PAR = -1, int HEAD_MT = 0>
+template <int MODE, int BIG, int PH, int PARTS, int WBUF, int NWV, int F16, int TEAMS = 1, int PAR = -1, int HEAD_MT = 0, int HEAD_SKIP = HEAD_SKIP_NONE>
 __device__ __forceinline__ void modconv_split_tile(const ide3d_modconv_params& p, const u32x4* __restrict__ wp, float* __restrict__ partial,
                                                    const ConvGeom& g, unsigned char* smem, int mb, int tl, int grp, int split, int tiles_x,
                                                    const float* __restrict__ row_unscale, float* wg_scratch = nullptr, const HeadEpi* he = nullptr) {
@@ -943,7 +1021,7 @@
 #endif
     if constexpr (HEAD_MT > 0) {
         static_assert(MODE == MODE_CONV3 && TEAMS == 1 && !F16 && K::NCLS == 1, "fused heads: 3x3 split-bf16 layers");
-        split_heads_finish<PH, PW, K::NWV, K::MTW, K::NTW, K::BM, HEAD_MT, PARTS, K::LDS_BYTES / 4>(p, *he, acc, reinterpret_cast<float*>(smem), n0, y0, x0, wm, wn, lp);
+        split_heads_finish<PH, PW, K::NWV, K::MTW, K::NTW, K::BM, HEAD_MT, PARTS, K::LDS_BYTES / 4, HEAD_SKIP>(p, *he, acc, reinterpret_cast<float*>(smem), n0, y0, x0, wm, wn, lp);
     } else
     modconv_finish<MODE, 1, PH, PW, K::NWV, K::NCLS, K::MTW, K::NTW, K::BM, K::LDS_BYTES / 4, PAR>(p, partial, g, acc, reinterpret_cast<float*>(smem), mb, n0, y0, x0, split, 0, wm, wn, lp,
                                                                                                 F16 ? row_unscale : nullptr, xus, (TEAMS == 2) ? tid : -1, wg_scratch);
@@ -1424,14 +1502,14 @@
     modconv_split_tile<MODE, BIG, PH, PARTS, WBUF, NWV, F16>(p, wp, partial, g, sp_smem, b.mb, b.tile, b.grp, b.split, g.tiles_x[0], row_unscale);
 }
 
-template <int BIG, int PH, int HEAD_MT>
+template <int BIG, int PH, int HEAD_MT, int SKIP = HEAD_SKIP_NONE>
 __global__ void __launch_bounds__(512, 2)
 modconv_split_heads_kernel(ide3d_modconv_params p, const u32x4* __restrict__ wp, ConvGeom g, HeadEpi he) {
     using K = SpCfg<MODE_CONV3, BIG, PH, 3, 2, 8>;
     if constexpr (kSpExclusive) asm volatile("" ::: "v255");
     __shared__ __attribute__((aligned(16))) unsigned char sp_smem[K::LDS_BYTES];
     const BlockId b = decode_block(g);
-    modconv_split_tile<MODE_CONV3, BIG, PH, 3, 2, 8, 0, 1, -1, HEAD_MT>(p, wp, nullptr, g, sp_smem, b.mb, b.tile, b.grp, b.split, g.tiles_x[0], nullptr, nullptr, &he);
+    modconv_split_tile<MODE_CONV3, BIG, PH, 3, 2, 8, 0, 1, -1, HEAD_MT, SKIP>(p, wp, nullptr, g, sp_smem, b.mb, b.tile, b.grp, b.split, g.tiles_x[0], nullptr, nullptr, &he);
 }
 
 template <int BIG, int PH, int PARTS, int F16 = 0>
@@ -2006,18 +2084,29 @@
     return IDE3D_OK;
 }
 
-extern "C" int ide3d_modconv2d_heads(const ide3d_modconv_params* pp, const ide3d_modconv_head_epilogue* hp, void* stream) {
+static int modconv2d_heads_impl(const ide3d_modconv_params* pp, const ide3d_modconv_head_epilogue* hp, const ide3d_modconv_skip_epilogue* sp,
+                                void* stream) {
     using namespace ide3d;
     IDE3D_CHECK_ARG(pp != nullptr && hp != nullptr, "modconv2d_heads: null params");
     const ide3d_modconv_params& p = *pp;
     const ide3d_modconv_head_epilogue& h = *hp;
-    IDE3D_CHECK_ARG(p.x && p.w && p.workspace && (p.y || h.no_activation_output) && h.w && h.y && h.workspace, "modconv2d_heads: null tensor / workspace pointer");
+    IDE3D_CHECK_ARG(p.x && p.w && p.workspace && (p.y || h.no_activation_output) && h.w && (h.y || sp) && h.workspace, "modconv2d_heads: null tensor / workspace pointer");
+    IDE3D_CHECK_ARG(!sp || (sp->lo && sp->y), "modconv2d_heads_skip: null lo / y");
     int rc = check_modconv(p);
     if (rc) return rc;
     IDE3D_CHECK_ARG(p.act == 1 || p.act == 3, "modconv2d_heads: act must be linear (1) or lrelu (3)");
     IDE3D_CHECK_ARG(h.rows > 0, "modconv2d_heads: bad head rows");
     auto no_kernel = [](const char* why) { set_error("modconv2d_heads: %s", why); return IDE3D_ENOKERNEL; };
     if (knob_live("IDE3D_MODCONV_NO_HEAD_FUSION")) return no_kernel("IDE3D_MODCONV_NO_HEAD_FUSION is set");
+    if (sp) {
+        if (knob_live("IDE3D_MODCONV_NO_SKIP_FUSION")) return no_kernel("IDE3D_MODCONV_NO_SKIP_FUSION is set");
+        if (sp->filter != IDE3D_SKIP_1331_CL && sp->filter != IDE3D_SKIP_1331_UP2) return no_kernel("no fused form for this skip filter");
+        if (sp->lo_h * 2 != p.h || sp->lo_w * 2 != p.w_) return no_kernel("the skip image is not exactly half the map");
+        const int64_t* ys = sp->y_stride;
+        if (ys[1] == 1 && (h.rows % 4 || (reinterpret_cast<uintptr_t>(sp->y) & 15) || (ys[0] & 3) || (ys[2] & 3) || (ys[3] & 3)))
+            return no_kernel("channels-last skip output: rows, pointer or strides not 16-byte aligned");
+        if (reinterpret_cast<uintptr_t>(sp->lo) & 3 || reinterpret_cast<uintptr_t>(sp->y) & 3) return no_kernel("misaligned skip pointer");
+    }
     if (p.k != 3 || p.mode != 0 || p.w_batch_stride != 0 || p.y_amax || p.y_pitch != 0) return no_kernel("not a shared-weight 3x3 layer without side outputs");
     int arith = resolve_arith(p.arith);
     if (arith == 16 && !p.x_amax) arith = 6;
@@ -2046,14 +2135,36 @@
     HeadEpi e;
     e.w = hw_packed; e.bias = h.bias; e.y = h.y; e.rows = h.rows; e.clamp = h.clamp; e.store_x = !h.no_activation_output;
     e.bias_first = head_resident_applies(q) ? 1 : 0;
+    e.lo = nullptr; e.dst = nullptr; e.lo_h = e.lo_w = 0;
+    for (int i = 0; i < 4; ++i) e.lo_s[i] = e.dst_s[i] = 0;
+    const int skip = sp ? sp->filter : HEAD_SKIP_NONE;
+    if (sp) {
+        e.lo = sp->lo; e.dst = sp->y; e.lo_h = sp->lo_h; e.lo_w = sp->lo_w;
+        for (int i = 0; i < 4; ++i) { e.lo_s[i] = sp->lo_stride[i]; e.dst_s[i] = sp->y_stride[i]; }
+    }
     const ConvGeom& g = pl.g;
     const unsigned nblocks = (unsigned)((int64_t)g.mblocks * g.tile_base[4] * g.img_groups * g.split_k);
     const u32x4* wu = reinterpret_cast<const u32x4*>(p.workspace);
-    if (tile32) IDE3D_EXCL_LAUNCH((modconv_split_heads_kernel<2, 32, 1>), dim3(nblocks), 512, 0, st, p, wu, g, e);
-    else if (mt == 1) IDE3D_EXCL_LAUNCH((modconv_split_heads_kernel<1, 16, 1>), dim3(nblocks), 512, 0, st, p, wu, g, e);
-    else IDE3D_EXCL_LAUNCH((modconv_split_heads_kernel<1, 16, 6>), dim3(nblocks), 512, 0, st, p, wu, g, e);
-    IDE3D_CHECK_LAUNCH("modconv2d_heads");
+#define IDE3D_HEADS_LAUNCH(S)                                                                                                    \
+    if (tile32) IDE3D_EXCL_LAUNCH((modconv_split_heads_kernel<2, 32, 1, S>), dim3(nblocks), 512, 0, st, p, wu, g, e);          \
+    else if (mt == 1) IDE3D_EXCL_LAUNCH((modconv_split_heads_kernel<1, 16, 1, S>), dim3(nblocks), 512, 0, st, p, wu, g, e);    \
+    else IDE3D_EXCL_LAUNCH((modconv_split_heads_kernel<1, 16, 6, S>), dim3(nblocks), 512, 0, st, p, wu, g, e);
+    if (skip == HEAD_SKIP_CL) { IDE3D_HEADS_LAUNCH(HEAD_SKIP_CL) }
+    else if (skip == HEAD_SKIP_UP2) { IDE3D_HEADS_LAUNCH(HEAD_SKIP_UP2) }
+    else { IDE3D_HEADS_LAUNCH(HEAD_SKIP_NONE) }
+#undef IDE3D_HEADS_LAUNCH
+    IDE3D_CHECK_LAUNCH(sp ? "modconv2d_heads_skip" : "modconv2d_heads");
     return IDE3D_OK;
+}
+
+extern "C" int ide3d_modconv2d_heads(const ide3d_modconv_params* pp, const ide3d_modconv_head_epilogue* hp, void* stream) {
+    return modconv2d_heads_impl(pp, hp, nullptr, stream);
+}
+
+extern "C" int ide3d_modconv2d_heads_skip(const ide3d_modconv_params* pp, const ide3d_modconv_head_epilogue* hp, const ide3d_modconv_skip_epilogue* sp,
+                                          void* stream) {
+    if (sp == nullptr) { ide3d::set_error("modconv2d_heads_skip: null skip epilogue"); return IDE3D_EINVAL; }
+    return modconv2d_heads_impl(pp, hp, sp, stream);
 }
 
 extern "C" int ide3d_modconv_plan(const ide3d_modconv_params* pp, ide3d_modconv_plan_info* out) {
diff --git a/ide-3d_amd/torch_utils/hip_plugin.py b/ide-3d_amd/torch_utils/hip_plugin.py
--- a/ide-3d_amd/torch_utils/hip_plugin.py
+++ b/ide-3d_amd/torch_utils/hip_plugin.py
@@ -124,6 +124,17 @@
         ('rows', ctypes.c_int32), ('clamp', ctypes.c_float), ('no_activation_output', ctypes.c_int32),
         ('workspace', ctypes.c_void_p), ('workspace_bytes', ctypes.c_int64),
     ]
+
+
+class _ModconvSkipEpilogue(ctypes.Structure):
+    _fields_ = [
+        ('lo', ctypes.c_void_p), ('lo_stride', ctypes.c_int64 * 4),
+        ('y', ctypes.c_void_p), ('y_stride', ctypes.c_int64 * 4),
+        ('lo_h', ctypes.c_int32), ('lo_w', ctypes.c_int32), ('filter', ctypes.c_int32), ('reserved', ctypes.c_int32),
+    ]
+
+
+SKIP_FILTERS = {'1331_cl': 1, '1331_up2': 2}
 
 
 class _ModconvPlanInfo(ctypes.Structure):
@@ -263,6 +274,7 @@
             'ide3d_density_lattice': [ctypes.POINTER(_RenderParams), ctypes.POINTER(_Lattice), i64, i64, vp, vp],
             'ide3d_modconv2d': [ctypes.POINTER(_ModconvParams), vp],
             'ide3d_modconv2d_heads': [ctypes.POINTER(_ModconvParams), ctypes.POINTER(_ModconvHeadEpilogue), vp],
+            'ide3d_modconv2d_heads_skip': [ctypes.POINTER(_ModconvParams), ctypes.POINTER(_ModconvHeadEpilogue), ctypes.POINTER(_ModconvSkipEpilogue), vp],
             'ide3d_modconv_plan': [ctypes.POINTER(_ModconvParams), ctypes.POINTER(_ModconvPlanInfo)],
             'ide3d_modconv_workspace_bytes': [i32, i32, i32, i32, i32, i32, i32, i32],
             'ide3d_set_conv_arithmetic': [i32],
@@ -296,7 +308,7 @@
     'ide3d_filtered_lrelu', 'ide3d_filtered_lrelu_act', 'ide3d_triplane_sample', 'ide3d_triplane_sample_rays', 'ide3d_triplane_taps',
     'ide3d_triplane_sample_backward', 'ide3d_composite', 'ide3d_sample_pdf', 'ide3d_render_rays', 'ide3d_sample_voxel',
     'ide3d_lattice_points', 'ide3d_density_lattice',
-    'ide3d_modconv2d', 'ide3d_modconv2d_heads', 'ide3d_modconv_workspace_bytes', 'ide3d_modconv_plan', 'ide3d_set_conv_arithmetic', 'ide3d_get_conv_arithmetic', 'ide3d_frame_u8', 'ide3d_sphere_points', 'ide3d_cam2world', 'ide3d_style_demod', 'ide3d_fold_heads',
+    'ide3d_modconv2d', 'ide3d_modconv2d_heads', 'ide3d_modconv2d_heads_skip', 'ide3d_modconv_workspace_bytes', 'ide3d_modconv_plan', 'ide3d_set_conv_arithmetic', 'ide3d_get_conv_arithmetic', 'ide3d_frame_u8', 'ide3d_sphere_points', 'ide3d_cam2world', 'ide3d_style_demod', 'ide3d_fold_heads',
     'ide3d_style_demod_batch', 'ide3d_fold_heads_batch',
     'ide3d_skip_upsample_add_cl', 'ide3d_bilinear_up2_split', 'ide3d_mapping', 'ide3d_mapping_workspace_bytes', 'ide3d_mapping_supported',
     'ide3d_lowres_layers_supported', 'ide3d_lowres_workspace_bytes', 'ide3d_lowres_group',
@@ -944,7 +956,7 @@
 
     @staticmethod
     def modconv2d_heads(x, w, styles, dcoefs, noise, noise_strength, bias, act, alpha, gain, clamp, head_w, head_bias, head_clamp,
-                        want_x=True, arith=0):
+                        want_x=True, arith=0, skip=None):
         for t in (x, w, head_w):
             _require(t.is_cuda and t.dtype == torch.float32 and t.is_contiguous(), 'modconv2d_heads: contiguous float32 CUDA tensors required')
         n, cin, h, wd = x.shape
@@ -961,8 +973,30 @@
         knob_off = 'IDE3D_MODCONV_NO_HEAD_FUSION' in os.environ
         if knob_off or shape_key in ModconvPlugin._heads_declined:
             return None
+        if skip is not None:
+            lo, filt = skip
+            _require(filt in SKIP_FILTERS, f'modconv2d_heads: skip filter must be one of {sorted(SKIP_FILTERS)}')
+            _require(lo.is_cuda and lo.dtype == torch.float32 and lo.device == x.device and lo.ndim == 4 and lo.shape[:2] == (n, rows),
+                     'modconv2d_heads: skip lo must be float32 [n, rows, h / 2, w / 2] on the device of x')
+            if 'IDE3D_MODCONV_NO_SKIP_FUSION' not in os.environ:
+                out = ModconvPlugin._heads_launch(lib, x, w, styles, dcoefs, noise, noise_strength, bias, act, alpha, gain, clamp, head_w,
+                                                  head_bias, head_clamp, want_x, arith, lo, SKIP_FILTERS[filt])
+                if out is not None:
+                    return out[0], out[1], True
+            out = ModconvPlugin._heads_launch(lib, x, w, styles, dcoefs, noise, noise_strength, bias, act, alpha, gain, clamp, head_w,
+                                              head_bias, head_clamp, want_x, arith)
+            return None if out is None else (out[0], out[1], False)
+        return ModconvPlugin._heads_launch(lib, x, w, styles, dcoefs, noise, noise_strength, bias, act, alpha, gain, clamp, head_w,
+                                           head_bias, head_clamp, want_x, arith)
+
+    @staticmethod
+    def _heads_launch(lib, x, w, styles, dcoefs, noise, noise_strength, bias, act, alpha, gain, clamp, head_w, head_bias, head_clamp,
+                      want_x, arith, lo=None, filt=0):
+        n, cin, h, wd = x.shape
+        cout, rows = w.shape[0], head_w.shape[1]
         y = torch.empty([n, cout, h, wd], dtype=torch.float32, device=x.device) if want_x else None
-        heads = torch.empty([n, rows, h, wd], dtype=torch.float32, device=x.device)
+        heads = torch.empty([n, rows, h, wd], dtype=torch.float32, device=x.device,
+                            memory_format=torch.channels_last if filt == SKIP_FILTERS['1331_cl'] else torch.contiguous_format)
         p, ent, keep = ModconvPlugin._params(lib, x, w, y, styles, dcoefs, noise, noise_strength, bias, act, alpha, gain, clamp, 0, arith, None, None)
         hent = ModconvPlugin._workspace(lib, heads, head_w, n, cout, rows, h, wd, 1, 0, True, arith)
         e = _ModconvHeadEpilogue()
@@ -972,12 +1006,22 @@
             _require(head_bias.is_cuda and head_bias.dtype == torch.float32 and head_bias.numel() == rows, 'modconv2d_heads: head_bias must be float32 [rows] on GPU')
             e.bias = head_bias.data_ptr()
         e.workspace, e.workspace_bytes = hent[0].data_ptr(), hent[0].numel() * 4
-        with _dev_guard(x.device):
-            rc = lib.ide3d_modconv2d_heads(ctypes.byref(p), ctypes.byref(e), _stream(x))
-        if rc == -2:
-            ModconvPlugin._heads_declined.add(shape_key)
-            return None
-        _check(rc, 'modconv2d_heads')
+        if lo is not None:
+            s = _ModconvSkipEpilogue()
+            s.lo, s.lo_stride, s.y, s.y_stride = lo.data_ptr(), _i64x4(lo.stride()), heads.data_ptr(), _i64x4(heads.stride())
+            s.lo_h, s.lo_w, s.filter = lo.shape[2], lo.shape[3], int(filt)
+            with _dev_guard(x.device):
+                rc = lib.ide3d_modconv2d_heads_skip(ctypes.byref(p), ctypes.byref(e), ctypes.byref(s), _stream(x))
+            if rc == -2:
+                return None
+            _check(rc, 'modconv2d_heads_skip')
+        else:
+            with _dev_guard(x.device):
+                rc = lib.ide3d_modconv2d_heads(ctypes.byref(p), ctypes.byref(e), _stream(x))
+            if rc == -2:
+                ModconvPlugin._heads_declined.add((n, cin, cout, h, wd, rows, arith))
+                return None
+            _check(rc, 'modconv2d_heads')
         ent[1], ent[2] = w._version, weakref.ref(w)
         return y, heads
 
diff --git a/ide-3d_amd/training/graph_cache.py b/ide-3d_amd/training/graph_cache.py
--- a/ide-3d_amd/training/graph_cache.py
+++ b/ide-3d_amd/training/graph_cache.py
@@ -119,7 +119,8 @@
         if not torch.is_tensor(t):
             return t
         base = t._base
-        if (base is not None and base.ndim >= 2 and base.is_contiguous() and t.ndim == base.ndim and t.stride() == base.stride()
+        dense = base is not None and (base.is_contiguous() or (base.ndim == 4 and base.is_contiguous(memory_format=torch.channels_last)))
+        if (dense and base.ndim >= 2 and t.ndim == base.ndim and t.stride() == base.stride()
                 and t.shape[0] == base.shape[0] and t.shape[2:] == base.shape[2:]):
             nb = memo.get(id(base))
             if nb is None:
diff --git a/ide-3d_amd/training/networks.py b/ide-3d_amd/training/networks.py
--- a/ide-3d_amd/training/networks.py
+++ b/ide-3d_amd/training/networks.py
@@ -421,7 +421,7 @@
     return y[:, :co], y[:, co:]
 
 
-def _conv1_dual_head(block, x, w1, w_shared, want_x, noise_mode='random', gain=1, input_noise=None, **unused):
+def _conv1_dual_head(block, x, w1, w_shared, want_x, noise_mode='random', gain=1, input_noise=None, skip=None, **unused):
     c1, tr, ts = block.conv1, block.torgb, block.toseg
     if not (use_hip_modconv and type(c1) is SynthesisLayer and c1.up == 1 and c1.padding == 1 and c1.weight.shape[2:] == (3, 3)
             and c1.activation in ('linear', 'lrelu') and tr.weight.shape[2] == 1 and tr.conv_clamp == ts.conv_clamp
@@ -450,13 +450,15 @@
     xc = x.contiguous()
     out = _modconv_plugin.modconv2d_heads(xc, c1.weight.contiguous(), styles.contiguous(), dcoefs, noise, 1.0, bias,
                                           spec.cuda_idx, spec.def_alpha, act_gain, -1.0 if act_clamp is None else act_clamp,
-                                          wcat, hbias, hclamp, want_x=want_x)
+                                          wcat, hbias, hclamp, want_x=want_x, skip=skip)
     if out is None:
         x = _modconv_bias_act(x, c1.weight, styles, True, noise, 1.0, bias, c1.activation, act_gain, act_clamp, dcoefs=dcoefs)
-        return x, _dual_head(x, tr, ts, w_shared, wcat=wcat)
-    x, y = out
+        return x, _dual_head(x, tr, ts, w_shared, wcat=wcat), None
+    x, y = out[:2]
+    if skip is not None and out[2]:
+        return x, None, y
     co = tr.weight.shape[0]
-    return x, (y[:, :co], y[:, co:])
+    return x, (y[:, :co], y[:, co:]), None
 
 
 _lowres_plugin = None
@@ -898,6 +900,18 @@
             return _upfirdn_plugin().upfirdn2d_ex(lo, f, 2, 2, 1, 1, 2, 1, 2, 1, False, 4.0, add=y)
         return cur.add_(y) if cur is not None else y
 
+    def _skip_in_heads(self, x, img, seg):
+        if img is None or seg is None or img.size(-1) * 2 != x.size(-1) or not _inference_on_gpu(img, seg):
+            return None
+        lo = _adjacent_views(img, seg)
+        if lo is None or self.resample_filter.shape != (4, 4) or not self._filter_is_1331():
+            return None
+        if getattr(self, 'skip_channels_last', False):
+            return (lo, '1331_cl') if img.shape[1] % 4 == 0 and seg.shape[1] % 4 == 0 else None
+        if self.is_last or os.environ.get('IDE3D_NO_SKIP_MERGE'):
+            return None
+        return lo, '1331_up2'
+
     def _filter_is_1331(self):
         ok = getattr(self, '_f1331', None)
         if ok is None:
@@ -920,7 +934,7 @@
             with misc.suppress_tracer_warnings():
                 fused_modconv = (not self.training) and (dtype == torch.float32 or int(ws.shape[0]) == 1)
 
-        fused = fused_heads = None
+        fused = fused_heads = fused_skip = None
         if self.in_channels == 0:
             x = self.const.to(dtype=dtype, memory_format=memory_format)
             x = x.unsqueeze(0).expand(ws.shape[0], *x.size())
@@ -938,22 +952,26 @@
                 layer_kwargs['input_noise'] = block_noise[:, 1:2] if block_noise is not None else None
                 w1 = next(w_iter)
                 if (self.is_last or self.architecture == 'skip') and not disable_rgb and dtype == torch.float32:
-                    fused = _conv1_dual_head(self, x, w1, ws_list[self.num_conv], not x_unused, **layer_kwargs)
+                    fused = _conv1_dual_head(self, x, w1, ws_list[self.num_conv], not x_unused, skip=self._skip_in_heads(x, img, seg),
+                                             **layer_kwargs)
                 if fused is not None:
-                    x, fused_heads = fused
+                    x, fused_heads, fused_skip = fused
                 else:
                     x = self.conv1(x, w1, fused_modconv=fused_modconv, **layer_kwargs)
 
         w_shared = next(w_iter) if (self.is_last or self.architecture == 'skip') else None
-        ref = x if x is not None else fused_heads[0]
         img_lo = seg_lo = None
-        heads_follow = (self.is_last or self.architecture == 'skip') and not disable_rgb
-        if heads_follow and _inference_on_gpu(ref) and img is not None and seg is not None and img.size(-1) * 2 == ref.size(-1):
-            img_lo, seg_lo, img, seg = img, seg, None, None
+        if fused_skip is not None:
+            img, seg = fused_skip[:, :img.shape[1]], fused_skip[:, img.shape[1]:]
         else:
-            img = self._merge_skip(img, ref)
-            seg = self._merge_skip(seg, ref)
-        if self.is_last or self.architecture == 'skip':
+            ref = x if x is not None else fused_heads[0]
+            heads_follow = (self.is_last or self.architecture == 'skip') and not disable_rgb
+            if heads_follow and _inference_on_gpu(ref) and img is not None and seg is not None and img.size(-1) * 2 == ref.size(-1):
+                img_lo, seg_lo, img, seg = img, seg, None, None
+            else:
+                img = self._merge_skip(img, ref)
+                seg = self._merge_skip(seg, ref)
+        if (self.is_last or self.architecture == 'skip') and fused_skip is None:
             if disable_rgb:
                 img = seg = None
             else:
diff --git a/ide-3d_amd/training/video_render.py b/ide-3d_amd/training/video_render.py
--- a/ide-3d_amd/training/video_render.py
+++ b/ide-3d_amd/training/video_render.py
@@ -41,10 +41,11 @@
         return planes, None
     with _plane_pool_lock:
         pool = _plane_pool.setdefault(synthesis, [])
-        ent = next((e for e in pool if not e[1] and all(b.shape == t.shape and b.stride() == t.stride() and b.device == t.device and b.dtype == t.dtype
-                                                        for b, t in zip(e[0], planes))), None)
+        fmt = lambda t: torch.channels_last if t.ndim == 4 and t.stride(1) == 1 else torch.contiguous_format
+        ent = next((e for e in pool if not e[1] and all(b.shape == t.shape and b.is_contiguous(memory_format=fmt(t)) and b.device == t.device
+                                                        and b.dtype == t.dtype for b, t in zip(e[0], planes))), None)
         if ent is None:
-            ent = [tuple(torch.empty_like(t) for t in planes), False]
+            ent = [tuple(torch.empty_like(t, memory_format=fmt(t)) for t in planes), False]
             pool.append(ent)
             del pool[:-8]
         ent[1] = True
diff --git a/include/ide3d_hip.h b/include/ide3d_hip.h
--- a/include/ide3d_hip.h
+++ b/include/ide3d_hip.h
@@ -201,6 +201,20 @@
     int64_t      workspace_bytes;
 } ide3d_modconv_head_epilogue;
 int ide3d_modconv2d_heads(const ide3d_modconv_params* p, const ide3d_modconv_head_epilogue* heads, void* stream);
+
+enum { IDE3D_SKIP_1331_CL = 1, IDE3D_SKIP_1331_UP2 = 2 };
+typedef struct ide3d_modconv_skip_epilogue {
+    const float* lo;
+    int64_t      lo_stride[4];
+    float*       y;
+    int64_t      y_stride[4];
+    int32_t      lo_h;
+    int32_t      lo_w;
+    int32_t      filter;
+    int32_t      reserved;
+} ide3d_modconv_skip_epilogue;
+int ide3d_modconv2d_heads_skip(const ide3d_modconv_params* p, const ide3d_modconv_head_epilogue* heads, const ide3d_modconv_skip_epilogue* skip,
+                               void* stream);
 
 enum { IDE3D_PLAN_FP32 = 0,
        IDE3D_PLAN_SPLIT = 1,
```

After: 922.6, median of 6. 1.3% higher.
